# THUDM/GCC

Hardware: AMD Instinct MI355X
Metric: sampled-subgraphs/sec (higher is better)
Workload: dtype f32

## Files before the change

gcc_amd/_cabi.py:

```python
from __future__ import annotations

import ctypes
import os

_HERE = os.path.dirname(os.path.abspath(__file__))
LIB_PATH = os.path.join(_HERE, "csrc", "libgcc_amd.so")
HEADER_PATH = os.path.join(os.path.dirname(_HERE), "include", "gcc_amd.h")

c_i32p = ctypes.POINTER(ctypes.c_int32)
c_f32p = ctypes.POINTER(ctypes.c_float)
c_f64p = ctypes.POINTER(ctypes.c_double)

STATUS_SCRATCH_OVERFLOW = 1
STATUS_NODE_OVERFLOW = 2
STATUS_EDGE_OVERFLOW = 4


class GccGraph(ctypes.Structure):
    _fields_ = [
        ("row_ptr", ctypes.c_void_p),
        ("col_idx", ctypes.c_void_p),
        ("seed_cdf", ctypes.c_void_p),
        ("ltab", ctypes.c_void_p),
        ("num_nodes", ctypes.c_int64),
# ... 150 lines not shown


CLS_HEAD_MAX_CLASSES = 64
CLS_HEAD_MAX_DIM = 256

ABI_VERSION = 3
GRAPH_CONTRACT_CHECKED = 1

GAT_MAX_LAYERS = 8
GAT_MAX_S2S_LAYERS = 8


class GccGatWeights(ctypes.Structure):
    _fields_ = [
        ("num_layers", ctypes.c_int32), ("hidden", ctypes.c_int32), ("heads", ctypes.c_int32), ("out_dim", ctypes.c_int32),
        ("pos_dim", ctypes.c_int32), ("deg_emb_dim", ctypes.c_int32), ("max_degree", ctypes.c_int32),
        ("s2s_iters", ctypes.c_int32), ("s2s_layers", ctypes.c_int32), ("normalize", ctypes.c_int32),
        ("norm_eps", ctypes.c_float),
        ("degree_embedding", _VP),
        ("fc", _VP * GAT_MAX_LAYERS), ("attn_l", _VP * GAT_MAX_LAYERS), ("attn_r", _VP * GAT_MAX_LAYERS),
        ("w_ih", _VP * GAT_MAX_S2S_LAYERS), ("w_hh", _VP * GAT_MAX_S2S_LAYERS),
        ("b_ih", _VP * GAT_MAX_S2S_LAYERS), ("b_hh", _VP * GAT_MAX_S2S_LAYERS),
        ("ro0_w", _VP), ("ro0_b", _VP), ("ro2_w", _VP), ("ro2_b", _VP),
    ]


class GccGatGrads(ctypes.Structure):
    _fields_ = [
        ("degree_embedding", _VP),
        ("fc", _VP * GAT_MAX_LAYERS), ("attn_l", _VP * GAT_MAX_LAYERS), ("attn_r", _VP * GAT_MAX_LAYERS),
        ("w_ih", _VP * GAT_MAX_S2S_LAYERS), ("w_hh", _VP * GAT_MAX_S2S_LAYERS),
        ("b_ih", _VP * GAT_MAX_S2S_LAYERS), ("b_hh", _VP * GAT_MAX_S2S_LAYERS),
        ("ro0_w", _VP), ("ro0_b", _VP), ("ro2_w", _VP), ("ro2_b", _VP),
    ]


class GccGatPass(ctypes.Structure):
    _fields_ = [
        ("node_off", _VP), ("row_ptr", _VP), ("col_idx", _VP), ("seed_local", _VP), ("pos", _VP),
        ("batch_size", ctypes.c_int32), ("node_cap", ctypes.c_int32), ("edge_multiplicity", ctypes.c_int32),
        ("reserved_", ctypes.c_int32),
        ("saved", _VP), ("out", _VP),
    ]


SIGNATURES = {
    "gcc_abi_version": (ctypes.c_int32, []),
    "gcc_last_error": (ctypes.c_char_p, []),
    "gcc_stream_create_cu_mask": (ctypes.c_int32, [ctypes.c_void_p, ctypes.c_int32, ctypes.POINTER(ctypes.c_void_p)]),
    "gcc_stream_destroy": (ctypes.c_int32, [ctypes.c_void_p]),
    "gcc_prof_create": (ctypes.c_void_p, [ctypes.c_int32]),
    "gcc_prof_destroy": (None, [ctypes.c_void_p]),
    "gcc_prof_elapsed_ms": (ctypes.c_int32, [ctypes.c_void_p, ctypes.c_int32, ctypes.c_int32, c_f32p]),
    "gcc_sampler_workspace_bytes": (ctypes.c_int64, [ctypes.POINTER(GccGraph), ctypes.c_int32, ctypes.c_int64]),
    "gcc_sampler_workspace_bytes_multi": (ctypes.c_int64, [ctypes.POINTER(GccGraph), ctypes.c_int32, ctypes.c_int32, ctypes.c_int64]),
    "gcc_sample_multi": (ctypes.c_int32, [
        ctypes.POINTER(GccGraph), ctypes.POINTER(GccSampleParams), ctypes.c_int32, ctypes.c_int64, ctypes.POINTER(GccBatchOut),
        ctypes.c_void_p, ctypes.c_int64, ctypes.c_int64, ctypes.c_void_p, ctypes.c_void_p]),
    "gcc_sample_batch": (ctypes.c_int32, [
        ctypes.POINTER(GccGraph), ctypes.POINTER(GccSampleParams), ctypes.POINTER(GccBatchOut),
        ctypes.POINTER(GccBatchOut), ctypes.c_void_p, ctypes.c_int64, ctypes.c_int64, ctypes.c_void_p,
        ctypes.c_void_p]),
    "gcc_posemb_workspace_bytes": (ctypes.c_int64, [ctypes.c_int32, ctypes.c_int64, ctypes.c_int32]),
    "gcc_posemb_debug_ticks": (None, [ctypes.c_void_p]),
    "gcc_posemb_set_fork": (None, [ctypes.c_int32]),
    "gcc_sampler_debug_ticks": (None, [ctypes.c_void_p]),
    "gcc_sampler_debug_grids": (None, [ctypes.c_int32, ctypes.c_int32, ctypes.c_int32]),
    "gcc_debug_load": (ctypes.c_int32, [ctypes.c_int32, ctypes.c_int32, ctypes.c_int32, ctypes.c_int32, ctypes.c_int64, ctypes.c_int32,
                                        ctypes.c_void_p, ctypes.c_int64, ctypes.c_void_p, ctypes.c_void_p]),
    "gcc_gin_debug_ticks": (None, [ctypes.c_void_p]),
    "gcc_ginw_debug_ticks": (None, [ctypes.c_void_p]),
    "gcc_posemb_multi_workspace_bytes": (ctypes.c_int64, [ctypes.c_int32, ctypes.c_int32, ctypes.c_int64, ctypes.c_int32]),
    "gcc_posemb_multi": (ctypes.c_int32, [ctypes.POINTER(GccPosembView), ctypes.c_int32, ctypes.c_int32, ctypes.c_int64,
                                          ctypes.c_int32, ctypes.c_uint64, ctypes.c_void_p, ctypes.c_int64, ctypes.c_void_p,
                                          ctypes.c_void_p, ctypes.c_void_p]),
    "gcc_posemb_multi_gated": (ctypes.c_int32, [ctypes.POINTER(GccPosembView), ctypes.c_int32, ctypes.c_int32, ctypes.c_int64,
                                          ctypes.c_int32, ctypes.c_uint64, ctypes.c_void_p, ctypes.c_int64, ctypes.c_void_p,
                                          ctypes.c_void_p, ctypes.c_void_p, ctypes.c_void_p, ctypes.c_void_p]),
    "gcc_posemb": (ctypes.c_int32, [ctypes.POINTER(GccBatchOut), ctypes.c_int32, ctypes.c_int32, ctypes.c_void_p,
                                    ctypes.c_void_p, ctypes.c_void_p, ctypes.c_uint64, ctypes.c_void_p, ctypes.c_int64, ctypes.c_void_p,
                                    ctypes.c_void_p, ctypes.c_void_p]),
    "gcc_gin_forward": (ctypes.c_int32, [ctypes.POINTER(GccGinPass), ctypes.c_int32, ctypes.c_void_p,
                                         ctypes.c_void_p]),
    "gcc_gin_backward_workspace_bytes": (ctypes.c_int64, [ctypes.c_int64, ctypes.c_int32, ctypes.c_int32]),
    "gcc_gin_backward": (ctypes.c_int32, [ctypes.POINTER(GccGinPass), ctypes.c_void_p, ctypes.POINTER(GccGinGrads),
                                          ctypes.c_int32, ctypes.c_void_p, ctypes.c_int64, ctypes.c_int64,
                                          ctypes.c_void_p, ctypes.c_void_p]),
    "gcc_ginx_workspace_bytes": (ctypes.c_int64, [ctypes.c_int64, ctypes.c_int32, ctypes.c_int32, ctypes.c_int32, ctypes.c_int32, ctypes.c_int32]),
    "gcc_ginx_forward": (ctypes.c_int32, [ctypes.POINTER(GccGinxPass), ctypes.c_void_p]),
    "gcc_ginx_backward": (ctypes.c_int32, [ctypes.POINTER(GccGinxPass), ctypes.c_void_p, ctypes.POINTER(GccGinGrads), ctypes.c_void_p]),
    "gcc_ncex_forward": (ctypes.c_int32, [ctypes.c_void_p, ctypes.c_void_p, ctypes.c_void_p, ctypes.c_int32, ctypes.c_int32, ctypes.c_int32,
                                          ctypes.c_float, ctypes.c_int32] + [ctypes.c_void_p] * 8),
    "gcc_queue_enqueue_x": (ctypes.c_int32, [ctypes.c_void_p, ctypes.c_int32, ctypes.c_int32, ctypes.c_void_p, ctypes.c_int32, ctypes.c_int32,
                                             ctypes.c_void_p]),
    "gcc_ginw_forward": (ctypes.c_int32, [ctypes.POINTER(GccGinwArgs), ctypes.c_void_p, ctypes.c_void_p, ctypes.c_void_p]),
    "gcc_ginw_pack_weights": (ctypes.c_int32, [ctypes.c_void_p, ctypes.c_void_p, ctypes.c_int32, ctypes.c_void_p]),
    "gcc_nce_workspace_bytes": (ctypes.c_int64, [ctypes.c_int32, ctypes.c_int32]),
    "gcc_nce_forward": (ctypes.c_int32, [ctypes.POINTER(GccNceArgs), ctypes.c_void_p, ctypes.c_int64,
                                         ctypes.c_void_p, ctypes.c_void_p]),
    "gcc_nce_backward": (ctypes.c_int32, [ctypes.POINTER(GccNceArgs), ctypes.c_void_p, ctypes.c_int32,
                                          ctypes.c_void_p, ctypes.c_void_p, ctypes.c_int64, ctypes.c_void_p,
                                          ctypes.c_void_p]),
    "gcc_queue_enqueue": (ctypes.c_int32, [ctypes.c_void_p, ctypes.c_int32, ctypes.c_void_p, ctypes.c_int32,
                                           ctypes.c_int32, ctypes.c_void_p, ctypes.c_void_p]),
    "gcc_adam_step": (ctypes.c_int32, [ctypes.c_void_p, ctypes.c_void_p, ctypes.c_void_p, ctypes.c_void_p,
                                       ctypes.c_int64, ctypes.c_float, ctypes.c_float, ctypes.c_float, ctypes.c_float,
                                       ctypes.c_float, ctypes.c_int32, ctypes.c_float, ctypes.c_float, ctypes.c_void_p,
                                       ctypes.c_void_p, ctypes.c_void_p]),
    "gcc_adam_ema_step": (ctypes.c_int32, [ctypes.c_void_p, ctypes.c_void_p, ctypes.c_void_p, ctypes.c_void_p,
                                           ctypes.c_int64, ctypes.c_float, ctypes.c_float, ctypes.c_float, ctypes.c_float,
                                           ctypes.c_float, ctypes.c_int32, ctypes.c_float, ctypes.c_float, ctypes.c_void_p,
                                           ctypes.c_void_p, ctypes.c_void_p, ctypes.c_int64, ctypes.c_float,
                                           ctypes.POINTER(GccStepMetersArgs), ctypes.c_void_p]),
    "gcc_adam_ema_step_scalars": (ctypes.c_int32, [ctypes.c_void_p, ctypes.c_void_p, ctypes.c_void_p, ctypes.c_void_p,
                                                   ctypes.c_int64, ctypes.c_float, ctypes.c_float, ctypes.c_float,
                                                   ctypes.c_float, ctypes.c_float, ctypes.c_float, ctypes.c_void_p,
                                                   ctypes.c_void_p, ctypes.c_void_p, ctypes.c_int64, ctypes.c_float,
                                                   ctypes.POINTER(GccStepMetersArgs), ctypes.c_void_p, ctypes.c_void_p]),
    "gcc_queue_enqueue_scalars": (ctypes.c_int32, [ctypes.c_void_p, ctypes.c_int32, ctypes.c_void_p, ctypes.c_int32,
                                                   ctypes.c_void_p, ctypes.c_void_p]),
    "gcc_ginw_scratch_bytes": (ctypes.c_int64, [ctypes.c_int64, ctypes.c_int32]),
    "gcc_gin_eval_debug_ticks": (None, [ctypes.c_void_p]),
    "gcc_gin_eval_fused": (ctypes.c_int32, [ctypes.POINTER(GccGinPass), ctypes.c_int32, ctypes.c_void_p, ctypes.c_void_p]),
    "gcc_step_scalars_fill": (None, [ctypes.c_void_p, ctypes.c_float, ctypes.c_float, ctypes.c_float, ctypes.c_int32,
                                      ctypes.c_int32, ctypes.c_uint64]),
    "gcc_step_scalars_fetch": (ctypes.c_int32, [ctypes.c_void_p, ctypes.c_void_p, ctypes.c_int32, ctypes.c_void_p, ctypes.c_void_p]),
    "gcc_step_scalars_set": (ctypes.c_int32, [ctypes.c_void_p, ctypes.c_float, ctypes.c_float, ctypes.c_float, ctypes.c_int32,
                                              ctypes.c_int32, ctypes.c_uint64, ctypes.c_void_p]),
    "gcc_step_meters": (ctypes.c_int32, [ctypes.c_void_p] * 8 + [ctypes.c_int32, ctypes.c_void_p]),
    "gcc_ema_update": (ctypes.c_int32, [ctypes.c_void_p, ctypes.c_void_p, ctypes.c_int64, ctypes.c_float,
                                        ctypes.c_void_p]),
    "gcc_gat_saved_floats": (ctypes.c_int64, [ctypes.POINTER(GccGatWeights), ctypes.c_int32, ctypes.c_int32]),
    "gcc_gat_forward": (ctypes.c_int32, [ctypes.POINTER(GccGatPass), ctypes.POINTER(GccGatWeights), ctypes.c_void_p]),
    "gcc_gat_backward_workspace_bytes": (ctypes.c_int64, [ctypes.POINTER(GccGatWeights), ctypes.c_int32, ctypes.c_int32]),
    "gcc_gat_backward": (ctypes.c_int32, [ctypes.POINTER(GccGatPass), ctypes.POINTER(GccGatWeights), ctypes.c_void_p,
                                          ctypes.POINTER(GccGatGrads), ctypes.c_int32, ctypes.c_void_p, ctypes.c_int64,
                                          ctypes.c_void_p]),
    "gcc_cls_head_train": (ctypes.c_int32, [ctypes.POINTER(GccClsHeadArgs), ctypes.c_void_p]),
    "gcc_cls_head_eval": (ctypes.c_int32, [ctypes.POINTER(GccClsHeadArgs), ctypes.c_void_p]),
    "gcc_adam_clipvalue_step": (ctypes.c_int32, [ctypes.c_void_p, ctypes.c_void_p, ctypes.c_void_p, ctypes.c_void_p,
                                                 ctypes.c_int64, ctypes.c_float, ctypes.c_float, ctypes.c_float, ctypes.c_float,
                                                 ctypes.c_float, ctypes.c_int32, ctypes.c_float, ctypes.c_float, ctypes.c_void_p]),
}
PENDING = set()


def declare(lib: ctypes.CDLL) -> ctypes.CDLL:
    for name, (res, args) in SIGNATURES.items():
        fn = getattr(lib, name)
        fn.restype = res
        fn.argtypes = args
    return lib


_lib = None


def load() -> ctypes.CDLL:
    global _lib
    if _lib is None:
        if not os.path.exists(LIB_PATH):
            raise RuntimeError(
                f"{LIB_PATH} is missing: build it with `python -c 'import __graft_entry__ as g; g.build()'` "
                "(hipcc --offload-arch=gfx950).  gcc_amd has no CPU fallback.")
        import torch

        lib = declare(ctypes.CDLL(LIB_PATH))
        got = lib.gcc_abi_version()
        if got != ABI_VERSION:
            raise RuntimeError(f"{LIB_PATH} reports C-ABI version {got}, this binding was written for {ABI_VERSION}: "
                               "rebuild the library (python -c 'import __graft_entry__ as g; g.build()')")
        _lib = lib
    return _lib


def check(rc: int, what: str) -> None:
    if rc != 0:
        raise RuntimeError(f"{what} failed ({rc}): {load().gcc_last_error().decode()}")


def dev_ptr(t, dtype=None) -> int:
    import torch

    if t is None:
        return 0
    if not isinstance(t, torch.Tensor) or not t.is_cuda:
        raise RuntimeError("gcc_amd kernels take device (HIP) tensors only; there is no CPU path")
    if dtype is not None and t.dtype != dtype:
        raise TypeError(f"expected {dtype}, got {t.dtype}")
    if not t.is_contiguous():
        raise ValueError("tensor must be contiguous")
    return t.data_ptr()
```

gcc_amd/contrast.py:

```python
from __future__ import annotations

import ctypes
import math

import torch
from torch import nn

from . import _cabi

D = 64


class NceEngine:

    def __init__(self, lib=None, ptr=None, dtype="f32"):
        self.lib = lib if lib is not None else _cabi.load()
        self.ptr = ptr if ptr is not None else _cabi.dev_ptr
        self._ws = {}
        self.dtype = dtype

    def _workspace(self, B, K, device):
        nbytes = self.lib.gcc_nce_workspace_bytes(B, K)
        key = (nbytes, str(device))
        if key not in self._ws:
            self._ws[key] = torch.empty(nbytes, dtype=torch.uint8, device=device)
        return self._ws[key], nbytes

    def _args(self, q, k, mem, inv_T, pos_mode, patch, patch_index, outs, dense):
        ptr = self.ptr
        a = _cabi.GccNceArgs()
        a.q, a.k, a.mem = ptr(q), ptr(k) if k is not None else None, ptr(mem)
        a.patch = ptr(patch) if patch is not None else None
        a.patch_index = int(patch_index)
        a.patch_rows = int(patch.shape[0]) if patch is not None else 0
        a.B, a.K, a.pos_mode, a.inv_T = q.shape[0], mem.shape[0], pos_mode, inv_T
        a.lse, a.pos, a.loss, a.prob = ptr(outs["lse"]), ptr(outs["pos"]), ptr(outs["loss"]), ptr(outs["prob"])
        a.out_dense = ptr(dense) if dense is not None else None
        a.dtype = {"f32": 0, "bf16": 1}[self.dtype]
        return a

    def forward(self, q, k, mem, T, pos_mode, dense=False, lse_rows=None, patch=None, patch_index=0, stream=None,
                prof=None):
        B, K = q.shape[0], mem.shape[0]
        f32 = dict(dtype=torch.float32, device=q.device)
        outs = dict(lse=torch.empty(lse_rows or B, **f32), pos=torch.empty(B, **f32), loss=torch.empty(1, **f32),
                    prob=torch.empty(1, **f32))
        out = torch.empty(B, K + (1 if pos_mode == 0 else 0), **f32) if dense else None
        ws, nbytes = self._workspace(B, K, q.device)
        a = self._args(q, k, mem, 1.0 / T, pos_mode, patch, patch_index, outs, out)
        rc = self.lib.gcc_nce_forward(ctypes.byref(a), self.ptr(ws), nbytes, prof.handle if prof else None, stream)
        if rc != 0:
            raise RuntimeError(f"gcc_nce_forward failed ({rc}): {self.lib.gcc_last_error().decode()}")
        outs["out"] = out
        return outs

    def backward(self, q, k, mem, T, pos_mode, outs, dloss, patch=None, patch_index=0, by_mem_row=False,
                 stream=None, prof=None):
        B, K = q.shape[0], mem.shape[0]
        dq = torch.empty_like(q)
        ws, nbytes = self._workspace(B, K, q.device)
        a = self._args(q, k, mem, 1.0 / T, pos_mode, patch, patch_index, outs, None)
        dloss = dloss.reshape(1).to(torch.float32).contiguous()
        rc = self.lib.gcc_nce_backward(ctypes.byref(a), self.ptr(dloss), int(by_mem_row), self.ptr(dq), self.ptr(ws),
                                       nbytes, prof.handle if prof else None, stream)
        if rc != 0:
            raise RuntimeError(f"gcc_nce_backward failed ({rc}): {self.lib.gcc_last_error().decode()}")
        return dq

    def set_scalars(self, scalars, lr, betas, adam_step, enqueue_index, dropout_seed, stream=None):
        rc = self.lib.gcc_step_scalars_set(self.ptr(scalars), float(lr), float(betas[0]), float(betas[1]), int(adam_step),
                                           int(enqueue_index), int(dropout_seed) & 0xFFFFFFFFFFFFFFFF, stream)
        if rc != 0:
            raise RuntimeError(f"gcc_step_scalars_set failed ({rc}): {self.lib.gcc_last_error().decode()}")

    def fill_scalars(self, ring, slot, lr, betas, adam_step, enqueue_index, dropout_seed):
        self.lib.gcc_step_scalars_fill(ring.data_ptr() + 24 * int(slot), float(lr), float(betas[0]), float(betas[1]),
                                       int(adam_step), int(enqueue_index), int(dropout_seed) & 0xFFFFFFFFFFFFFFFF)

    def fetch_scalars(self, scalars, ring, ring_len, counter, stream=None):
        rc = self.lib.gcc_step_scalars_fetch(self.ptr(scalars), ring.data_ptr(), int(ring_len), self.ptr(counter), stream)
        if rc != 0:
            raise RuntimeError(f"gcc_step_scalars_fetch failed ({rc}): {self.lib.gcc_last_error().decode()}")

    def enqueue(self, mem, keys, index, save=True, stream=None, scalars=None):
        if scalars is not None:
            rc = self.lib.gcc_queue_enqueue_scalars(self.ptr(mem), mem.shape[0], self.ptr(keys), keys.shape[0],
                                                    self.ptr(scalars), stream)
            if rc != 0:
                raise RuntimeError(f"gcc_queue_enqueue_scalars failed ({rc}): {self.lib.gcc_last_error().decode()}")
            return None
        saved = torch.empty_like(keys) if save else None
        rc = self.lib.gcc_queue_enqueue(self.ptr(mem), mem.shape[0], self.ptr(keys), keys.shape[0], int(index),
                                        self.ptr(saved) if saved is not None else None, stream)
        if rc != 0:
            raise RuntimeError(f"gcc_queue_enqueue failed ({rc}): {self.lib.gcc_last_error().decode()}")
        return saved

    def adam(self, param, grad, exp_avg, exp_avg_sq, lr, betas, eps, weight_decay, step, max_norm, grad_norm,
             scratch, stream=None, grad_scale=1.0):
        rc = self.lib.gcc_adam_step(self.ptr(param), self.ptr(grad), self.ptr(exp_avg), self.ptr(exp_avg_sq),
                                    param.numel(), float(lr), float(betas[0]), float(betas[1]), float(eps),
                                    float(weight_decay), int(step), float(max_norm), float(grad_scale), self.ptr(grad_norm),
                                    self.ptr(scratch), stream)
        if rc != 0:
            raise RuntimeError(f"gcc_adam_step failed ({rc}): {self.lib.gcc_last_error().decode()}")

    def adam_ema(self, param, grad, exp_avg, exp_avg_sq, lr, betas, eps, weight_decay, step, max_norm, grad_norm,
                 scratch, stream=None, grad_scale=1.0, ema=None, ema_src=None, ema_m=0.0, meters=None, scalars=None):
        ma = None
        if meters is not None:
            acc, mx, loss, prob, q, k = meters
            ma = _cabi.GccStepMetersArgs(self.ptr(acc), self.ptr(mx), self.ptr(loss), self.ptr(prob), self.ptr(q.node_off),
                                         self.ptr(q.edge_off), self.ptr(k.node_off), int(q.batch_size))
        if ema is not None and (ema_src is None or ema_src.data_ptr() != param.data_ptr() or ema.numel() != ema_src.numel()):
            raise ValueError("adam_ema: param must be a prefix of ema_src, and ema the same size as ema_src")
        if scalars is not None:
            rc = self.lib.gcc_adam_ema_step_scalars(
                self.ptr(param), self.ptr(grad), self.ptr(exp_avg), self.ptr(exp_avg_sq), param.numel(), float(betas[0]),
                float(betas[1]), float(eps), float(weight_decay), float(max_norm), float(grad_scale), self.ptr(grad_norm),
                self.ptr(scratch), self.ptr(ema) if ema is not None else None, ema.numel() if ema is not None else 0,
                float(ema_m), ctypes.byref(ma) if ma is not None else None, self.ptr(scalars), stream)
            if rc != 0:
                raise RuntimeError(f"gcc_adam_ema_step_scalars failed ({rc}): {self.lib.gcc_last_error().decode()}")
            return
        rc = self.lib.gcc_adam_ema_step(self.ptr(param), self.ptr(grad), self.ptr(exp_avg), self.ptr(exp_avg_sq),
                                        param.numel(), float(lr), float(betas[0]), float(betas[1]), float(eps),
                                        float(weight_decay), int(step), float(max_norm), float(grad_scale),
                                        self.ptr(grad_norm), self.ptr(scratch),
                                        self.ptr(ema) if ema is not None else None, ema.numel() if ema is not None else 0,
                                        float(ema_m), ctypes.byref(ma) if ma is not None else None, stream)
        if rc != 0:
            raise RuntimeError(f"gcc_adam_ema_step failed ({rc}): {self.lib.gcc_last_error().decode()}")

    def meters(self, acc, mx, loss, prob, grad_norm, q, k, stream=None):
        rc = self.lib.gcc_step_meters(self.ptr(acc), self.ptr(mx), self.ptr(loss), self.ptr(prob), self.ptr(grad_norm),
                                      self.ptr(q.node_off), self.ptr(q.edge_off), self.ptr(k.node_off),
                                      int(q.batch_size), stream)
        if rc != 0:
            raise RuntimeError(f"gcc_step_meters failed ({rc}): {self.lib.gcc_last_error().decode()}")

    def ema(self, ema, p, m, stream=None):
        rc = self.lib.gcc_ema_update(self.ptr(ema), self.ptr(p), ema.numel(), float(m), stream)
        if rc != 0:
            raise RuntimeError(f"gcc_ema_update failed ({rc}): {self.lib.gcc_last_error().decode()}")


def _stream(t):
    return torch.cuda.current_stream(t.device).cuda_stream if t.is_cuda else None


class _MoCoLoss(torch.autograd.Function):

    @staticmethod
    def forward(ctx, q, k, module, outs, patch, patch_index):
        ctx.module, ctx.outs, ctx.patch, ctx.patch_index = module, outs, patch, patch_index
        ctx.save_for_backward(q, k)
        return outs["loss"].reshape(())

    @staticmethod
    def backward(ctx, dloss):
        q, k = ctx.saved_tensors
        m = ctx.module
        dq = m.engine().backward(q, k, m.kernel_memory(), m.T, 0, ctx.outs, dloss, patch=ctx.patch,
                                 patch_index=ctx.patch_index, stream=_stream(q))
        return dq, None, None, None, None, None


class _NSLoss(torch.autograd.Function):

    @staticmethod
    def forward(ctx, feat_q, feat_k, T, eng):
        fq, fk = feat_q.contiguous(), feat_k.contiguous()
        outs = eng.forward(fk, None, fq, T, 1, stream=_stream(fq))
        ctx.eng, ctx.T, ctx.outs = eng, T, outs
        ctx.save_for_backward(fq, fk)
        ctx.mark_non_differentiable(outs["prob"])
        return outs["loss"].reshape(()), outs["prob"].reshape(())

    @staticmethod
    def backward(ctx, dloss, _dprob):
        fq, fk = ctx.saved_tensors
        eng, T, outs = ctx.eng, ctx.T, ctx.outs
        dk = eng.backward(fk, None, fq, T, 1, outs, dloss, stream=_stream(fq))
        dq = eng.backward(fq, None, fk, T, 1, outs, dloss, by_mem_row=True, stream=_stream(fq))
        return dq, dk, None, None


class WideNceEngine:

    def __init__(self, lib=None, ptr=None):
        self.lib = lib if lib is not None else _cabi.load()
        self.ptr = ptr if ptr is not None else _cabi.dev_ptr

    def forward(self, rows, k, mem, T, mode, stream=None):
        B, D = rows.shape
        K = mem.shape[0]
        f32 = dict(dtype=torch.float32, device=rows.device)
        ncols = K + 1 if mode == 0 else K
# ... 173 lines not shown
```

gcc_amd/csrc/encoder.hip:

```cpp
#include "encoder_common.h"

namespace {

struct FeatArgs {
    const int32_t *node_off, *row_ptr, *graph_id, *seed_local;
    const float *pos, *emb;
    float *x0;
    float4 *zero_a, *zero_b;
    int64_t zero_a16, zero_b16;
    int32_t B, pos_dim, emb_dim, max_degree, mult;
    int32_t cap;
};
struct FeatLaunch { FeatArgs p[kMaxPass]; };

__global__ __launch_bounds__(kThreads) void gin_feat_kernel(FeatLaunch L)
{
    TRAIN_STEP_WAVE_PRIORITY();
    const FeatArgs &a = L.p[blockIdx.y];
    const int tid = (int)threadIdx.x, t = tid & 15, gi = tid >> 4;
    constexpr int kR = kTile / 16;
    int vv[kR], r0[kR], r1[kR], gv[kR];
    float pv[kR][4];
    auto request = [&](int tile0) {
#pragma unroll
        for (int i = 0; i < kR; ++i) {
            vv[i] = cap_row(tile0 + gi + 16 * i, a.cap);
            r0[i] = a.row_ptr[vv[i]];
            r1[i] = a.row_ptr[vv[i] + 1];
            gv[i] = a.graph_id[vv[i]];
#pragma unroll
            for (int e = 0; e < 4; ++e)
                pv[i][e] = a.pos_dim > 0 ? a.pos[(int64_t)vv[i] * a.pos_dim + min(4 * t + e, a.pos_dim - 1)] : 0.f;
        }
    };
    const int tf = first_tile();
    request(tf * kTile);
    const int N = a.node_off[a.B];
    SCHED_FENCE();
    {
        const float4 z4 = make_float4(0.f, 0.f, 0.f, 0.f);
        const int64_t stride = (int64_t)gridDim.x * kThreads;
        for (int64_t i = (int64_t)blockIdx.x * kThreads + tid; i < a.zero_a16; i += stride) a.zero_a[i] = z4;
        for (int64_t i = (int64_t)blockIdx.x * kThreads + tid; i < a.zero_b16; i += stride) a.zero_b[i] = z4;
    }
    for (TileWalk tw(N); tw.ti < tw.tend; tw.ti += tw.step) {
        const int tile0 = tw.ti * kTile;
        const int nrows = min(kTile, N - tile0);
        if (tw.ti != tf) request(tile0);
        int first[kR], sl[kR];
        float ev[kR][4];
        const int dtot = a.pos_dim + a.emb_dim;
#pragma unroll
        for (int i = 0; i < kR; ++i) {
            const int deg = (r1[i] - r0[i]) * a.mult;
            const int dcl = max(0, deg < a.max_degree ? deg : a.max_degree);
            const int g = min(max(gv[i], 0), a.B - 1);
            first[i] = a.node_off[g];
            sl[i] = a.seed_local ? a.seed_local[g] : 0;
#pragma unroll
            for (int e = 0; e < 4; ++e) {
                const int c = 4 * t + e;
                ev[i][e] = a.emb[(int64_t)dcl * a.emb_dim + (c >= a.pos_dim && c < dtot ? c - a.pos_dim : 0)];
            }
        }
#pragma unroll
        for (int i = 0; i < kR; ++i) {
            if (gi + 16 * i >= nrows) continue;
            const bool is_seed = vv[i] == first[i] + sl[i];
            F4 x;
#pragma unroll
            for (int e = 0; e < 4; ++e) {
                const int c = 4 * t + e;
                at(x, e) = c < a.pos_dim ? pv[i][e] : c < dtot ? ev[i][e] : (c == dtot && is_seed ? 1.f : 0.f);
            }
            st4(a.x0 + (int64_t)vv[i] * H + 4 * t, x);
        }
    }
}

struct InArgs {
    const int32_t *node_off, *row_ptr, *col_idx, *graph_id;
    const float *src;
    BnDev bnb, bnc;
    const float *w0, *b0;
    float *agg;
    float *z1;
    double *stats_a;
    double *pooled;
    int32_t B, first, kdim, training;
    float eps, nbr_weight;
    int32_t cap;
};
struct InLaunch { InArgs p[kMaxPass]; long long *ticks; };
#ifndef GIN_IN_LDS_W
#define GIN_IN_LDS_W 1
#endif
#ifndef GIN_DBG_SKIP
#define GIN_DBG_SKIP 0
#endif
static long long *g_gin_ticks = nullptr;
constexpr int kTickWgs = 2048, kTickPhases = 16;
#define TICK_ADD(kind, ph, v) atomicAdd((unsigned long long *)&L.ticks[((kind) * kTickPhases + (ph)) * kTickWgs + (int)blockIdx.y * 1024 + (int)blockIdx.x], (unsigned long long)(v))
#define GIN_TICK(ph) do { if (L.ticks && tid == 0) { const long long now_ = device_ticks(); TICK_ADD(a.first ? 0 : 1, ph, now_ - tick_); tick_ = now_; } } while (0)

#ifndef GIN_IN_PER_CU
#define GIN_IN_PER_CU 3
#endif
#ifndef GIN_GATHER_J
#define GIN_GATHER_J 8
#endif
__global__ __launch_bounds__(kThreads, GIN_IN_PER_CU) void gin_in_kernel(InLaunch L)
{
    TRAIN_STEP_WAVE_PRIORITY();
    __shared__ float T[kTile * kLdt];
    __shared__ __attribute__((aligned(16))) float part[32 * H];
    __shared__ float red[4 * 2 * H];
    __shared__ int prow[32];
    __shared__ int rpl[kTile + 1], gidl[kTile];
    const InArgs &a = L.p[blockIdx.y];
    const int tid = (int)threadIdx.x, t = tid & 15, gi = tid >> 4, lane = lane_id(), wv = tid >> 6;
    int N;
    __shared__ float tabb[2 * H], tabc[2 * H];
#if GIN_IN_LDS_W
    __shared__ float Wl[H * kLdt];
    __shared__ __attribute__((aligned(16))) float bl[H];
#endif
    Aff4 ab, ac;
    long long tick_ = L.ticks ? device_ticks() : 0;
    const float *src = a.src;
    auto load = [&](int u) -> F4 { return ld4(src + (int64_t)u * H + 4 * t); };
    const int tf = first_tile();
    int rp_own, gid_own;
    F4 own[kTile / 16];
    auto request = [&](int tile0) {
        rp_own = a.row_ptr[min(tile0 + min(tid, kTile), a.cap)];
        gid_own = a.graph_id[cap_row(tile0 + (tid & (kTile - 1)), a.cap)];
#pragma unroll
        for (int i = 0; i < kTile / 16; ++i) own[i] = load(cap_row(tile0 + gi + 16 * i, a.cap));
    };
    {
#if GIN_IN_LDS_W
        const WStage wst = stage_weights_request(a.w0, a.kdim);
        const float b_own = a.b0 ? a.b0[tid & (H - 1)] : 0.f;
#endif
        if (!a.first) {
            const BnReq rb = bn_request(a.bnb), rc = bn_request(a.bnc);
            request(tf * kTile);
            N = a.node_off[a.B];
            SCHED_FENCE();
            if (no_tiles(N)) return;
            bn_table_finish(tabb, rb, (double)N, a.eps, a.training, (double *)part);
            bn_table_finish(tabc, rc, (double)N, a.eps, a.training, (double *)part);
        } else {
            request(tf * kTile);
            N = ((const volatile int32_t *)a.node_off)[a.B];
            if (no_tiles(N)) return;
        }
#if GIN_IN_LDS_W
        stage_weights_store(Wl, wst, a.kdim);
// ... 295 lines not shown
            for (int e = 0; e < 4; ++e) pd[c][e] = prow[16 * c + e];
        SCHED_FENCE();
#pragma unroll
        for (int c = 0; c < 4; ++c) {
            const F4 x = {(float)pd[c][0], (float)pd[c][1], (float)pd[c][2], (float)pd[c][3]}, z = {0.f, 0.f, 0.f, 0.f};
            xb[c] = valid ? x : z;
        }
        f32x4 acc[4];
        mfma_rows16(xb, wf, acc);
#pragma unroll
        for (int cb = 0; cb < 4; ++cb) {
            const int ch = 16 * cb + 4 * q;
            const F4 bias = bias4[cb];
            const F4 m = valid ? drop_mul4(drop, i, b, ch) : bias;
            score[cb].x += (acc[cb][0] + bias.x) * m.x;
            score[cb].y += (acc[cb][1] + bias.y) * m.y;
            score[cb].z += (acc[cb][2] + bias.z) * m.z;
            score[cb].w += (acc[cb][3] + bias.w) * m.w;
        }
    }
#pragma unroll
    for (int cb = 0; cb < 4; ++cb) st4(&part[wv][j][16 * cb + 4 * q], score[cb]);
    __syncthreads();
    if (wv == 0) {
        float ss = 0.f;
#pragma unroll
        for (int cb = 0; cb < 4; ++cb) {
            F4 t = ld4(&part[0][j][16 * cb + 4 * q]);
            for (int w2 = 1; w2 < 4; ++w2) t = add4(t, ld4(&part[w2][j][16 * cb + 4 * q]));
            score[cb] = t;
            ss += t.x * t.x + t.y * t.y + t.z * t.z + t.w * t.w;
        }
        ss += wave_shfl_xor(ss, 16);
        ss += wave_shfl_xor(ss, 32);
        const float inv = a.normalize ? 1.0f / fmaxf(sqrtf(ss), a.norm_eps) : 1.0f;
        if (valid) {
#pragma unroll
            for (int cb = 0; cb < 4; ++cb) {
                const int ch = 16 * cb + 4 * q;
                st4(a.score + (int64_t)b * H + ch, score[cb]);
                F4 o = {score[cb].x * inv, score[cb].y * inv, score[cb].z * inv, score[cb].w * inv};
                st4(a.feat + (int64_t)b * H + ch, o);
            }
        }
    }
    if (bn_work) {
        const int n_nodes = a.node_off[a.B];
        double *scratch = (double *)&part[0][0][0];
        for (int k = (int)blockIdx.x; k < 3 * a.nlayers; k += (int)gridDim.x) {
            __syncthreads();
            const BnDev &bn = a.bn[k];
            float rm = rm0, rv = rv0;
            if (k == (int)blockIdx.x) {
                scratch[tid] = rep_sum(rq);
                __syncthreads();
            } else {
                replica_sums128(bn.stats, 2 * H, scratch);
                rm = bn.running_mean[tid & (H - 1)];
                rv = bn.running_var[tid & (H - 1)];
            }
            if (tid < H) {
                const int c = tid;
                const double n = (double)n_nodes;
                const double s1 = scratch[c] + scratch[128 + c], s2 = scratch[H + c] + scratch[128 + H + c];
                if (a.totals) { a.totals[(int64_t)k * 2 * H + c] = s1; a.totals[(int64_t)k * 2 * H + H + c] = s2; }
                if (a.update_running) {
                    const double mean = s1 / n;
                    double var = s2 / n - mean * mean;
                    if (var < 0.0) var = 0.0;
                    const double unb = n > 1.0 ? var * n / (n - 1.0) : var;
                    bn.running_mean[c] = (float)((1.0 - a.momentum) * (double)rm + a.momentum * mean);
                    bn.running_var[c] = (float)((1.0 - a.momentum) * (double)rv + a.momentum * unb);
                    if (c == 0 && bn.nbt) bn.nbt[0] += 1;
                }
            }
        }
    }
}

}

extern "C" void gcc_gin_debug_ticks(long long *device_ticks64) { g_gin_ticks = device_ticks64; }

extern "C" int32_t gcc_gin_forward(const gcc_gin_pass *passes, int32_t npass, gcc_prof *prof, void *stream)
{
    if (!passes || npass < 1 || npass > kMaxPass) {
        snprintf(g_err, kErrLen, "gcc_gin_forward: npass must be 1..%d", kMaxPass);
        return -1;
    }
    const int Lg = passes[0].w.num_gin_layers;
    int maxB = 0;
    for (int i = 0; i < npass; ++i) {
        const gcc_gin_pass &p = passes[i];
        const int din = p.w.pos_dim + p.w.deg_emb_dim + 1;
        if (p.w.num_gin_layers != Lg || Lg < 1 || Lg > GCC_GIN_MAX_LAYERS || din > H || p.batch_size < 1) {
            snprintf(g_err, kErrLen, "gcc_gin_forward: unsupported shape (layers=%d d_in=%d B=%d)",
                     p.w.num_gin_layers, din, p.batch_size);
            return -2;
        }
        if (p.node_cap < 1 || p.node_cap > 0x7fffffff) {
            snprintf(g_err, kErrLen, "gcc_gin_forward: gcc_gin_pass.node_cap = %lld (the row capacity of the pass's buffers is required)",
                     (long long)p.node_cap);
            return -2;
        }
        maxB = p.batch_size > maxB ? p.batch_size : maxB;
    }
    hipStream_t s = (hipStream_t)stream;
    prof_mark(prof, 0, s);
    int64_t rows_max = 0;
    for (int i = 0; i < npass; ++i) {
        const gcc_gin_pass &p = passes[i];
        const int64_t r = p.rows_hint > 0 && p.rows_hint < p.node_cap ? p.rows_hint : p.node_cap;
        rows_max = r > rows_max ? r : rows_max;
    }
    const dim3 grid(tile_grid(rows_max), npass), block(kThreads);
    {
        FeatLaunch L;
        for (int i = 0; i < npass; ++i) {
            const gcc_gin_pass &p = passes[i];
            L.p[i] = {p.node_off, p.row_ptr, p.graph_id, p.seed_local, p.pos, p.w.degree_embedding, p.x0,
                      (float4 *)p.stats, (float4 *)p.pooled, (int64_t)Lg * 3 * kRep * 2 * H * (int64_t)sizeof(double) / 16,
                      (int64_t)(Lg + 1) * p.batch_size * H * (int64_t)sizeof(double) / 16,
                      p.batch_size, p.w.pos_dim, p.w.deg_emb_dim, p.w.max_degree, p.edge_multiplicity > 1 ? p.edge_multiplicity : 1,
                      (int32_t)p.node_cap};
        }
        hipLaunchKernelGGL(gin_feat_kernel, grid, block, 0, s, L);
    }
    for (int l = 0; l < Lg; ++l) {
        {
            InLaunch L;
            for (int i = 0; i < npass; ++i) {
                const gcc_gin_pass &p = passes[i];
                InArgs a;
                a.node_off = p.node_off; a.row_ptr = p.row_ptr; a.col_idx = p.col_idx; a.graph_id = p.graph_id;
                a.src = l == 0 ? p.x0 : p.z2[l - 1];
                a.bnb = l == 0 ? BnDev() : bn_of(p, p.w.bn_b[l - 1], l - 1, 1, false);
                a.bnc = l == 0 ? BnDev() : bn_of(p, p.w.bn_c[l - 1], l - 1, 2, false);
                a.w0 = p.w.lin0_w[l]; a.b0 = p.w.lin0_b[l];
                a.agg = p.agg[l]; a.z1 = p.z1[l];
                a.stats_a = stats_of(p, l, 0);
                a.pooled = p.pooled + (int64_t)l * p.batch_size * H;
                a.B = p.batch_size; a.first = l == 0;
                a.kdim = l == 0 ? p.w.pos_dim + p.w.deg_emb_dim + 1 : hidden_of(p.w);
                a.training = p.training; a.eps = p.w.bn_eps;
                a.nbr_weight = p.edge_multiplicity > 1 ? (float)p.edge_multiplicity : 1.0f;
                a.cap = (int32_t)p.node_cap;
                L.p[i] = a;
            }
            L.ticks = g_gin_ticks;
            hipLaunchKernelGGL(gin_in_kernel, grid, block, 0, s, L);
        }
        {
            MidLaunch L;
            for (int i = 0; i < npass; ++i) {
                const gcc_gin_pass &p = passes[i];
                L.p[i] = {p.node_off, p.z1[l], bn_of(p, p.w.bn_a[l], l, 0, false), p.w.lin1_w[l], p.w.lin1_b[l],
                          p.z2[l], stats_of(p, l, 1), p.batch_size, p.training,
                          p.w.bn_eps, hidden_of(p.w), (int32_t)p.node_cap};
            }
            L.ticks = g_gin_ticks;
            hipLaunchKernelGGL(gin_mid_kernel, grid, block, 0, s, L);
        }
        {
            StatLaunch L;
            bool need = false;
            for (int i = 0; i < npass; ++i) {
                const gcc_gin_pass &p = passes[i];
                L.p[i] = {p.node_off, p.z2[l], bn_of(p, p.w.bn_b[l], l, 1, false), stats_of(p, l, 2), p.batch_size, p.training, p.w.bn_eps,
                          (int32_t)p.node_cap};
                need = need || p.training;
            }
            if (need) hipLaunchKernelGGL(gin_stat_kernel, grid, block, 0, s, L);
        }
    }
    {
        PoolLaunch L;
        for (int i = 0; i < npass; ++i) {
            const gcc_gin_pass &p = passes[i];
            L.p[i] = {p.node_off, p.graph_id, p.z2[Lg - 1], bn_of(p, p.w.bn_b[Lg - 1], Lg - 1, 1, false),
                      bn_of(p, p.w.bn_c[Lg - 1], Lg - 1, 2, false), p.pooled + (int64_t)Lg * p.batch_size * H,
                      p.batch_size, p.training, p.w.bn_eps, (int32_t)p.node_cap};
        }
        hipLaunchKernelGGL(gin_pool_kernel, grid, block, 0, s, L);
    }
    {
        ReadLaunch L;
        for (int i = 0; i < npass; ++i) {
            const gcc_gin_pass &p = passes[i];
            ReadArgs a;
            a.node_off = p.node_off; a.pooled = p.pooled;
            for (int k = 0; k <= Lg; ++k) { a.pred_w[k] = p.w.pred_w[k]; a.pred_b[k] = p.w.pred_b[k]; }
            a.drop = drop_cfg(p); a.score = p.score; a.feat = p.feat;
            for (int l = 0; l < Lg; ++l) {
                a.bn[3 * l + 0] = bn_of(p, p.w.bn_a[l], l, 0, false);
                a.bn[3 * l + 1] = bn_of(p, p.w.bn_b[l], l, 1, false);
                a.bn[3 * l + 2] = bn_of(p, p.w.bn_c[l], l, 2, false);
            }
            a.totals = p.training ? p.bn_totals : nullptr;
            a.B = p.batch_size; a.nlayers = Lg; a.kdim0 = p.w.pos_dim + p.w.deg_emb_dim + 1; a.hid = hidden_of(p.w);
            a.normalize = p.normalize; a.update_running = p.training && p.update_running_stats;
            a.norm_eps = p.w.norm_eps; a.momentum = p.w.bn_momentum;
            L.p[i] = a;
        }
        hipLaunchKernelGGL(gin_readout_kernel, dim3((maxB + 15) / 16, npass), block, 0, s, L);
    }
    prof_mark(prof, 1, s);
    hipError_t e = hipGetLastError();
    if (e != hipSuccess) {
        snprintf(g_err, kErrLen, "gcc_gin_forward: launch failed: %s", hipGetErrorString(e));
        return -10;
    }
    return 0;
}
```

gcc_amd/csrc/encoder_bwd.hip:

```cpp
#include "encoder_common.h"

namespace {

constexpr int kWgChunks = 64;

struct BnCol { float mean, rstd, gamma, beta; };
__device__ __forceinline__ BnCol bn_col(const BnDev &bn, int c, double s1, double s2, double n, float eps)
{
    const double mean = s1 / n;
    double var = s2 / n - mean * mean;
    if (var < 0.0) var = 0.0;
    BnCol r;
    r.mean = (float)mean;
    r.rstd = (float)(1.0 / sqrt(var + (double)eps));
    r.gamma = bn.weight[c];
    r.beta = bn.bias[c];
    return r;
}

enum { RS = 0, RM = 1, PS = 2, PH = 3, K1 = 4, K2 = 5, K3 = 6, kCoefRows = 7 };

__device__ __forceinline__ void fill_coefs(float *C , const BnDev &bn, const double *bst, double n,
                                           float eps, double *scratch)
{
// ... 641 lines not shown
    SCHED_FENCE();
    const int N = jb.rows_fixed > 0 ? jb.rows_fixed : Nn;
    TileWalk tw(N);
    if (tid < H) {
        float sc = 1.f, sh = 0.f;
        if (fast) {
            const double mean = cr.s1 / (double)Nn;
            double var = cr.s2 / (double)Nn - mean * mean;
            if (var < 0.0) var = 0.0;
            const double rstd = 1.0 / sqrt(var + (double)a.eps);
            sc = (float)((double)cr.gamma * rstd);
            sh = (float)((double)cr.beta - mean * (double)cr.gamma * rstd);
        } else if (act) {
            bn_scale_shift(jb.bn, tid, (double)Nn, a.eps, 1, sc, sh);
        }
        Cx[tid] = sc;
        Cx[H + tid] = sh;
    }
    __syncthreads();
    float xs[4], xh[4];
#pragma unroll
    for (int kb = 0; kb < 4; ++kb) { xs[kb] = Cx[16 * kb + j]; xh[kb] = Cx[H + 16 * kb + j]; }
    for (; tw.ti < tw.tend; tw.ti += tw.step) {
        const int tile0 = tw.ti * kTile;
        float an[4][4], xn[4][4];
        const bool more = tw.ti + tw.step < tw.tend;
        if (more) fetch((tw.ti + tw.step) * kTile, an, xn);
        mask_tile(tile0, N, av, xv);
#pragma unroll
        for (int s = 0; s < 4; ++s) {
            const int row = tile0 + 16 * wv + 4 * s + q;
            float bv[4];
#pragma unroll
            for (int k = 0; k < 4; ++k) {
                bsum[k] += av[s][k];
                bv[k] = act ? (row < N ? fmaxf(fmaf(xv[s][k], xs[k], xh[k]), 0.f) : 0.f) : xv[s][k];
            }
#pragma unroll
            for (int ob = 0; ob < 4; ++ob)
#pragma unroll
                for (int kb = 0; kb < 4; ++kb) acc[ob][kb] = mfma_16x16x4_f32(av[s][ob], bv[kb], acc[ob][kb]);
        }
        if (more) {
#pragma unroll
            for (int s = 0; s < 4; ++s)
#pragma unroll
                for (int k = 0; k < 4; ++k) { av[s][k] = an[s][k]; xv[s][k] = xn[s][k]; }
        }
    }
    for (int w = 0; w < 4; ++w) {
        if (wv == w) {
#pragma unroll
            for (int ob = 0; ob < 4; ++ob)
#pragma unroll
                for (int kb = 0; kb < 4; ++kb)
#pragma unroll
                    for (int r = 0; r < 4; ++r) {
                        const int o = 16 * ob + 4 * q + r, k = 16 * kb + j;
                        S[o * H + k] = (w == 0 ? 0.f : S[o * H + k]) + acc[ob][kb][r];
                    }
        }
        __syncthreads();
    }
    float *slab = a.slabs + ((int64_t)jid * kWgChunks + blockIdx.x) * H * H;
    for (int i = tid; i < H * H; i += kThreads) slab[i] = S[i];
#pragma unroll
    for (int k = 0; k < 4; ++k) {
        bsum[k] += wave_shfl_xor(bsum[k], 16);
        bsum[k] += wave_shfl_xor(bsum[k], 32);
        if (q == 0) Sb[wv * H + 16 * k + j] = bsum[k];
    }
    __syncthreads();
    if (tid < H)
        a.bias_slabs[((int64_t)jid * kWgChunks + blockIdx.x) * H + tid] =
            (Sb[tid] + Sb[H + tid]) + (Sb[2 * H + tid] + Sb[3 * H + tid]);
}

struct FinalArgs {
    const float *slabs, *bias_slabs;
    const double *bst;
    const float *demb_parts;
    gcc_gin_grads g;
    int32_t B, L, kdim0, emb_rows, emb_dim, accumulate, hid;
};

__device__ __forceinline__ void put(float *dst, float v, int acc)
{
    if (dst) *dst = acc ? *dst + v : v;
}

__global__ __launch_bounds__(kThreads) void gin_grad_final_kernel(FinalArgs a)
{
    TRAIN_STEP_WAVE_PRIORITY();
    const int64_t gid = (int64_t)blockIdx.x * kThreads + threadIdx.x;
    const int L = a.L;
    int64_t base = 0;
    const int njobs = 3 * L + 1;
    const int64_t n1 = (int64_t)njobs * H * H;
    if (gid < n1) {
        const int y = (int)(gid / (H * H)), idx = (int)(gid % (H * H));
        const int o = idx / H, k = idx % H;
        float s = 0.f;
        for (int c = 0; c < kWgChunks; ++c) s += a.slabs[((int64_t)y * kWgChunks + c) * H * H + idx];
        int kd = H;
        float *dst;
        if (y < 2 * L) {
            const int l = y >> 1, which = y & 1;
            kd = (which == 0 && l == 0) ? a.kdim0 : a.hid;
            dst = which ? a.g.lin1_w[l] : a.g.lin0_w[l];
        } else {
            const int i = y - 2 * L;
            kd = i == 0 ? a.kdim0 : a.hid;
            dst = a.g.pred_w[i];
        }
        if (k < kd && dst) put(dst + (int64_t)o * kd + k, s, a.accumulate);
        return;
    }
    base += n1;
    const int64_t n3 = (int64_t)(L + 1) * H;
    if (gid < base + n3) {
        const int64_t r = gid - base;
        const int i = (int)(r / H), o = (int)(r % H);
        float s = 0.f;
        for (int c = 0; c < kWgChunks; ++c) s += a.bias_slabs[((int64_t)(2 * L + i) * kWgChunks + c) * H + o];
        if (a.g.pred_b[i]) put(a.g.pred_b[i] + o, s, a.accumulate);
        return;
    }
    base += n3;
    const int64_t n4 = (int64_t)L * 3 * 3 * H;
    if (gid < base + n4) {
        const int64_t r = gid - base;
        const int c = (int)(r % H), slot = (int)((r / H) % 3), which = (int)((r / (3 * H)) % 3), l = (int)(r / (9 * H));
        double acc = 0.0;
        const double *src = a.bst + ((int64_t)l * 3 + which) * kRep * 3 * H + slot * H + c;
#pragma unroll
        for (int rep = 0; rep < kRep; rep += 8) {
            double v8[8];
#pragma unroll
            for (int u = 0; u < 8; ++u) v8[u] = src[(int64_t)(rep + u) * 3 * H];
            acc += ((v8[0] + v8[1]) + (v8[2] + v8[3])) + ((v8[4] + v8[5]) + (v8[6] + v8[7]));
        }
        const float v = (float)acc;
        float *dst = nullptr;
        if (which == 0) dst = slot == 0 ? a.g.bn_a_b[l] : slot == 1 ? a.g.bn_a_w[l] : a.g.lin0_b[l];
        else if (which == 1) dst = slot == 0 ? a.g.bn_b_b[l] : slot == 1 ? a.g.bn_b_w[l] : a.g.lin1_b[l];
        else dst = slot == 0 ? a.g.bn_c_b[l] : slot == 1 ? a.g.bn_c_w[l] : nullptr;
        if (dst) put(dst + c, v, a.accumulate);
        return;
    }
    base += n4;
    base = (base + 63) & ~(int64_t)63;
    const int64_t n5 = (int64_t)a.emb_rows * a.emb_dim;
    if (gid >= base) {
        static_assert(kEmbBlocks % 64 == 0, "8 threads x batches of 8 partials");
        const int64_t q = gid - base, r = q >> 3;
        const int part = (int)(q & 7);
        float s = 0.f;
        if (r < n5) {
            const float *src = a.demb_parts + (int64_t)part * (kEmbBlocks / 8) * n5 + r;
            for (int k = 0; k < kEmbBlocks / 8; k += 8) {
                float v[8];
#pragma unroll
                for (int u = 0; u < 8; ++u) v[u] = src[(int64_t)(k + u) * n5];
                s += ((v[0] + v[1]) + (v[2] + v[3])) + ((v[4] + v[5]) + (v[6] + v[7]));
            }
        }
        s += wave_shfl_xor(s, 1);
        s += wave_shfl_xor(s, 2);
        s += wave_shfl_xor(s, 4);
        if (part == 0 && r < n5 && a.g.degree_embedding) put(a.g.degree_embedding + r, s, a.accumulate);
    }
}

struct BwdWork {
    float *U, *V, *Wt, *D;
    float *dz1[GCC_GIN_MAX_LAYERS], *dz2[GCC_GIN_MAX_LAYERS];
    float *G, *dpooled, *slabs, *bias_slabs;
    double *bst;
    float *demb_parts;
    int64_t off_zero, zero_bytes, total;
};

inline BwdWork bwd_layout(char *base, int64_t node_cap, int32_t B, int32_t L, int32_t emb_elems)
{
    BwdWork w;
    auto al = [](int64_t x) { return (x + 255) & ~(int64_t)255; };
    int64_t o = 0;
    auto take = [&](int64_t bytes) { int64_t at = o; o = al(o + bytes); return base ? base + at : (char *)nullptr; };
    const int64_t act = node_cap * H * (int64_t)sizeof(float);
    w.U = (float *)take(act); w.V = (float *)take(act); w.Wt = (float *)take(act); w.D = (float *)take(act);
    for (int l = 0; l < GCC_GIN_MAX_LAYERS; ++l) {
        w.dz1[l] = l < L ? (float *)take(act) : nullptr;
        w.dz2[l] = l < L ? (float *)take(act) : nullptr;
    }
    w.G = (float *)take((int64_t)(L + 1) * B * H * sizeof(float));
    w.dpooled = (float *)take((int64_t)(L + 1) * B * H * sizeof(float));
    w.slabs = (float *)take((int64_t)(3 * L + 1) * kWgChunks * H * H * sizeof(float));
    w.bias_slabs = (float *)take((int64_t)(3 * L + 1) * kWgChunks * H * sizeof(float));
    w.demb_parts = (float *)take((int64_t)kEmbBlocks * emb_elems * sizeof(float));
    w.off_zero = o;
    w.bst = (double *)take((int64_t)L * 9 * kRep * H * sizeof(double));
    w.zero_bytes = o - w.off_zero;
    w.total = o;
    return w;
}

}

extern "C" int64_t gcc_gin_backward_workspace_bytes(int64_t node_cap, int32_t batch_size, int32_t num_gin_layers)
{
    if (node_cap <= 0 || batch_size <= 0 || num_gin_layers < 1 || num_gin_layers > GCC_GIN_MAX_LAYERS) {
        snprintf(g_err, kErrLen, "gcc_gin_backward_workspace_bytes: bad argument");
        return -1;
    }
    return bwd_layout(nullptr, node_cap, batch_size, num_gin_layers, kEmbMaxElems).total;
}

extern "C" int32_t gcc_gin_backward(const gcc_gin_pass *pass, const float *dfeat, const gcc_gin_grads *grads,
                                    int32_t accumulate, void *workspace, int64_t workspace_bytes,
                                    int64_t node_cap, gcc_prof *prof, void *stream)
{
    if (!pass || !dfeat || !grads || !workspace) {
        snprintf(g_err, kErrLen, "gcc_gin_backward: null argument");
        return -1;
    }
    const gcc_gin_pass &p = *pass;
    if (p.edge_multiplicity > 1) {
        snprintf(g_err, kErrLen, "gcc_gin_backward: edge_multiplicity %d (inference-only feature)", p.edge_multiplicity);
        return -2;
    }
    const int L = p.w.num_gin_layers, B = p.batch_size;
    const int kdim0 = p.w.pos_dim + p.w.deg_emb_dim + 1;
    const int emb_elems = (p.w.max_degree + 1) * p.w.deg_emb_dim;
    if (!p.training || L < 1 || L > GCC_GIN_MAX_LAYERS || emb_elems > kEmbMaxElems) {
        snprintf(g_err, kErrLen, "gcc_gin_backward: needs a training-mode pass (layers=%d)", L);
        return -2;
    }
    for (int l = 0; l < L; ++l)
        if (!p.agg[l]) { snprintf(g_err, kErrLen, "gcc_gin_backward: agg[%d] was not saved", l); return -2; }
    const BwdWork w = bwd_layout((char *)workspace, node_cap, B, L, kEmbMaxElems);
    if (workspace_bytes < w.total) {
        snprintf(g_err, kErrLen, "gcc_gin_backward: workspace %lld < %lld bytes", (long long)workspace_bytes,
                 (long long)w.total);
        return -3;
    }
    if (node_cap < 1 || node_cap > 0x7fffffff || (p.node_cap > 0 && p.node_cap != node_cap)) {
        snprintf(g_err, kErrLen, "gcc_gin_backward: node_cap %lld (the pass says %lld)", (long long)node_cap, (long long)p.node_cap);
        return -2;
    }
    const int32_t cap = (int32_t)node_cap;
    hipStream_t s = (hipStream_t)stream;
    prof_mark(prof, 0, s);
    const dim3 grid(tile_grid(p.rows_hint > 0 && p.rows_hint < node_cap ? p.rows_hint : node_cap)), block(kThreads);
    auto bst = [&](int l, int which) { return w.bst + ((int64_t)l * 3 + which) * kRep * 3 * H; };
    {
        ReadBwdArgs a;
        a.dfeat = dfeat; a.score = p.score; a.feat = p.feat; a.drop = drop_cfg(p);
        for (int i = 0; i <= L; ++i) a.pred_w[i] = p.w.pred_w[i];
        a.G = w.G; a.dpooled = w.dpooled; a.B = B; a.nlayers = L; a.kdim0 = kdim0; a.normalize = p.normalize; a.hid = hidden_of(p.w);
        a.norm_eps = p.w.norm_eps;
        a.zero = (float4 *)((char *)workspace + w.off_zero); a.zero16 = w.zero_bytes / 16; a.nread = ((B + 15) / 16 * (L + 1) + 3) / 4;
        hipLaunchKernelGGL(gin_bwd_readout_kernel, dim3(a.nread + 64), block, 0, s, a);
    }
    for (int l = L - 1; l >= 0; --l) {
        const BnDev bna = bn_of(p, p.w.bn_a[l], l, 0);
        const BnDev bnb = bn_of(p, p.w.bn_b[l], l, 1);
        const BnDev bnc = bn_of(p, p.w.bn_c[l], l, 2);
        {
            BwdCArgs a = {p.node_off, p.row_ptr, p.col_idx, p.graph_id, l == L - 1 ? nullptr : w.D,
                          w.dpooled + (int64_t)(l + 1) * B * H, p.z2[l], bnb, bnc, w.U, bst(l, 2), B, p.w.bn_eps, cap};
            hipLaunchKernelGGL(gin_bwd_c_kernel, grid, block, 0, s, a);
        }
        {
            BwdBArgs a = {p.node_off, w.U, p.z2[l], bnb, bnc, bst(l, 2), w.V, bst(l, 1), B, p.w.bn_eps, cap};
            hipLaunchKernelGGL(gin_bwd_b_kernel, grid, block, 0, s, a);
        }
        {
            BwdLinArgs a = {p.node_off, w.V, p.z2[l], bnb, bst(l, 1), bst(l, 1) + 2 * H, p.w.lin1_w[l], hidden_of(p.w),
                            w.dz2[l], w.Wt, p.z1[l], bna, bst(l, 0), B, p.w.bn_eps, cap};
            hipLaunchKernelGGL((gin_bwd_lin_kernel<true>), grid, block, 0, s, a);
        }
        {
            BwdLinArgs a = {p.node_off, w.Wt, p.z1[l], bna, bst(l, 0), bst(l, 0) + 2 * H, p.w.lin0_w[l],
                            l == 0 ? kdim0 : hidden_of(p.w), w.dz1[l], w.D, nullptr, BnDev(), nullptr, B, p.w.bn_eps, cap};
            hipLaunchKernelGGL((gin_bwd_lin_kernel<false>), grid, block, 0, s, a);
        }
    }
    {
        EmbArgs a = {p.node_off, p.row_ptr, p.col_idx, p.graph_id, w.D, w.dpooled, w.demb_parts, B, p.w.pos_dim,
                     p.w.deg_emb_dim, p.w.max_degree, cap};
        hipLaunchKernelGGL(gin_bwd_emb_kernel, dim3(kEmbBlocks), block, 0, s, a);
    }
    {
        WgradArgs a;
        a.node_off = p.node_off; a.slabs = w.slabs; a.bias_slabs = w.bias_slabs; a.B = B; a.eps = p.w.bn_eps; a.cap = cap;
        for (int l = 0; l < L; ++l) {
            a.job[2 * l + 0] = {w.dz1[l], p.agg[l], nullptr, BnDev(), 0};
            a.job[2 * l + 1] = {w.dz2[l], p.z1[l], nullptr, bn_of(p, p.w.bn_a[l], l, 0), 0};
        }
        for (int i = 0; i <= L; ++i)
            a.job[2 * L + i] = {w.G + (int64_t)i * B * H, nullptr, p.pooled + (int64_t)i * B * H, BnDev(), B};
        hipLaunchKernelGGL(gin_wgrad_kernel, dim3(kWgChunks, 3 * L + 1), block, 0, s, a);
    }
    {
        FinalArgs a;
        a.slabs = w.slabs; a.bias_slabs = w.bias_slabs; a.bst = w.bst; a.demb_parts = w.demb_parts; a.g = *grads;
        a.B = B; a.L = L; a.kdim0 = kdim0; a.emb_rows = p.w.max_degree + 1; a.emb_dim = p.w.deg_emb_dim; a.hid = hidden_of(p.w);
        a.accumulate = accumulate;
        const int64_t upto4 = (int64_t)(3 * L + 1) * H * H + (int64_t)(L + 1) * H + (int64_t)L * 9 * H;
        const int64_t total = ((upto4 + 63) & ~(int64_t)63) + (((int64_t)a.emb_rows * a.emb_dim * 8 + 63) & ~(int64_t)63);
        hipLaunchKernelGGL(gin_grad_final_kernel, dim3((unsigned)((total + kThreads - 1) / kThreads)), block, 0, s, a);
    }
    prof_mark(prof, 1, s);
    hipError_t e = hipGetLastError();
    if (e != hipSuccess) {
        snprintf(g_err, kErrLen, "gcc_gin_backward: launch failed: %s", hipGetErrorString(e));
        return -10;
    }
    return 0;
}
```

gcc_amd/csrc/nce.hip:

```cpp
#include "host_common.h"

#include <math.h>

namespace {

constexpr int D = GCC_NCE_DIM;
constexpr int kLd = 72;
constexpr int kChunk = 64;
constexpr int kThreads = 256;
constexpr int kQPerBlock = 64;

struct F4 { float x, y, z, w; };
__device__ __forceinline__ F4 ld4(const float *p)
{
    const float4 v = *reinterpret_cast<const float4 *>(p);
    F4 r = {v.x, v.y, v.z, v.w};
    return r;
}
__device__ __forceinline__ void st4(float *p, F4 v) { *reinterpret_cast<float4 *>(p) = make_float4(v.x, v.y, v.z, v.w); }

struct NceDev {
    const float *q, *k, *mem, *patch;
    int32_t patch_index, patch_rows, B, K, pos_mode;
    int32_t bf16;
// ... 112 lines not shown
    for (int c0 = row_beg; c0 < row_end; c0 += kChunk) {
#pragma unroll
        for (int i = 0; i < 4; ++i) {
            const int idx = tid + kThreads * i, row = idx >> 4, c4 = (idx & 15) * 4;
            st4(&Ms[row * kLd + c4], finish_mem4(a, nxt[i], c0 + row));
        }
        __syncthreads();
        if (c0 + kChunk < row_end) request(c0 + kChunk);
        for (int t = 0; t < 4; ++t) {
            if (c0 + 16 * t >= row_end) break;
            f32x4 acc = {0.f, 0.f, 0.f, 0.f};
            if (kBf16 && !kBwd) {
#pragma unroll
                for (int sl = 0; sl < 2; ++sl) {
                    const F4 lo = ld4(&Ms[(16 * t + j) * kLd + 32 * sl + 8 * q]), hi = ld4(&Ms[(16 * t + j) * kLd + 32 * sl + 8 * q + 4]);
                    u32x4 mb;
                    mb[0] = pack_bf16(lo.x, lo.y); mb[1] = pack_bf16(lo.z, lo.w);
                    mb[2] = pack_bf16(hi.x, hi.y); mb[3] = pack_bf16(hi.z, hi.w);
                    acc = mfma_16x16x32_bf16(mb, qb[sl], acc);
                }
            } else {
#pragma unroll
                for (int c = 0; c < 4; ++c) {
                    const F4 mf = ld4(&Ms[(16 * t + j) * kLd + 16 * c + 4 * q]);
                    acc = mfma_16x16x4_f32(mf.x, qf[c].x, acc);
                    acc = mfma_16x16x4_f32(mf.y, qf[c].y, acc);
                    acc = mfma_16x16x4_f32(mf.z, qf[c].z, acc);
                    acc = mfma_16x16x4_f32(mf.w, qf[c].w, acc);
                }
            }
            const int row0 = c0 + 16 * t + 4 * q;
            float lv[4];
#pragma unroll
            for (int r = 0; r < 4; ++r) {
                const float l = acc[r] * a.inv_T;
                const bool valid = row0 + r < row_end;
                if (!kBwd && a.out_dense && qvalid && valid) a.out_dense[(int64_t)qj * ld_out + off_out + row0 + r] = l;
                lv[r] = valid ? l : -INFINITY;
            }
            if (!kBwd) {
                const float tmax = fmaxf(fmaxf(lv[0], lv[1]), fmaxf(lv[2], lv[3]));
                if (tmax > -INFINITY) {
                    const float mn = fmaxf(m, tmax);
                    ssum = ssum * expf(m - mn) + expf(lv[0] - mn) + expf(lv[1] - mn) + expf(lv[2] - mn) + expf(lv[3] - mn);
                    m = mn;
                }
            } else {
                float lse_r[4] = {my_lse, my_lse, my_lse, my_lse};
                if (a.by_mem_row) {
#pragma unroll
                    for (int r = 0; r < 4; ++r) lse_r[r] = a.lse[min(row0 + r, a.K - 1)];
                }
#pragma unroll
                for (int r = 0; r < 4; ++r) {
                    float p = 0.f;
                    if (qvalid && lv[r] > -INFINITY) p = expf(lv[r] - lse_r[r]);
#pragma unroll
                    for (int db = 0; db < 4; ++db)
                        acc2[db] = mfma_16x16x4_f32(Ms[(16 * t + 4 * q + r) * kLd + 16 * db + j], p, acc2[db]);
                }
            }
        }
        __syncthreads();
    }
    if (!kBwd) {
#pragma unroll
        for (int d = 16; d <= 32; d <<= 1) {
            const float m2 = wave_shfl_xor(m, d), s2 = wave_shfl_xor(ssum, d);
            const float mn = fmaxf(m, m2);
            ssum = mn > -INFINITY ? ssum * expf(m - mn) + s2 * expf(m2 - mn) : 0.f;
            m = mn;
        }
        if (q == 0 && qvalid) {
            a.pm[(int64_t)s * a.B + qj] = m;
            a.ps[(int64_t)s * a.B + qj] = ssum;
        }
    } else if (qvalid) {
#pragma unroll
        for (int db = 0; db < 4; ++db) {
            F4 o = {acc2[db][0], acc2[db][1], acc2[db][2], acc2[db][3]};
            st4(a.slabs + ((int64_t)s * a.B + qj) * D + 16 * db + 4 * q, o);
        }
    }
}

__global__ __launch_bounds__(kThreads) void nce_combine_kernel(NceDev a)
{
    TRAIN_STEP_WAVE_PRIORITY();
    __shared__ double red[8];
    __shared__ int last;
    const int tid = (int)threadIdx.x, lane = lane_id(), wv = tid >> 6;
    const int ld_out = a.K + (a.pos_mode == 0 ? 1 : 0);
    const int b = (int)blockIdx.x * (kThreads >> 6) + wv;
    if (b < a.B) {
        const float *other = a.pos_mode == 0 ? a.k : a.mem;
        float qv = a.q[(int64_t)b * D + lane], ov = other[(int64_t)b * D + lane];
        const int s0 = min(lane, a.S - 1);
        const float pm0r = a.pm[(int64_t)s0 * a.B + b], ps0r = a.ps[(int64_t)s0 * a.B + b];
        const float pm0 = lane < a.S ? pm0r : -INFINITY;
        if (a.bf16) { qv = rnd_bf16(qv); ov = rnd_bf16(ov); }
        const float pos = wave_sum(qv * ov) * a.inv_T;
        float m = pm0;
        for (int s = lane + 64; s < a.S; s += 64) m = fmaxf(m, a.pm[(int64_t)s * a.B + b]);
        m = wave_max(m);
        if (a.pos_mode == 0) m = fmaxf(m, pos);
        float sum = pm0 > -INFINITY ? ps0r * expf(pm0 - m) : 0.f;
        for (int s = lane + 64; s < a.S; s += 64) {
            const float pmv = a.pm[(int64_t)s * a.B + b], psv = a.ps[(int64_t)s * a.B + b];
            if (pmv > -INFINITY) sum += psv * expf(pmv - m);
        }
        sum = wave_sum(sum);
        if (a.pos_mode == 0) sum += expf(pos - m);
        const float lse = m + logf(sum);
        if (lane == 0) {
            a.lse[b] = lse;
            a.pos[b] = pos;
            if (a.pos_mode == 0 && a.out_dense) a.out_dense[(int64_t)b * ld_out] = pos;
        }
    }
    device_fence();
    __syncthreads();
    if (tid == 0) last = atomicAdd(a.ticket, 1) == (int)gridDim.x - 1;
    __syncthreads();
    if (!last) return;
    device_fence();
    double lsum = 0.0, psum = 0.0;
    for (int i = tid; i < a.B; i += kThreads) {
        const float lse = load_fresh(a.lse + i), pos = load_fresh(a.pos + i);
        lsum += (double)(lse - pos);
        psum += (double)pos;
    }
    lsum = wave_sum(lsum);
    psum = wave_sum(psum);
    if (lane == 0) { red[wv] = lsum; red[4 + wv] = psum; }
    __syncthreads();
    if (tid == 0) {
        a.loss[0] = (float)((red[0] + red[1] + red[2] + red[3]) / (double)a.B);
        a.prob[0] = (float)((red[4] + red[5] + red[6] + red[7]) / (double)a.B);
        *a.ticket = 0;
    }
}

#ifndef NCE_DQ_BATCH
#define NCE_DQ_BATCH 16
#endif
__global__ __launch_bounds__(kThreads) void nce_dq_kernel(NceDev a)
{
    TRAIN_STEP_WAVE_PRIORITY();
    const int gid = (int)blockIdx.x * kThreads + (int)threadIdx.x;
    const int b = gid >> 4, c4 = (gid & 15) * 4;
    if (b >= a.B) return;
    const float dl = a.dloss[0];
    const float posb = a.pos_mode == 0 ? a.pos[b] : 0.f, lseb = a.pos_mode == 0 ? a.lse[b] : 0.f;
    const F4 other = rnd4(ld4((a.pos_mode == 0 ? a.k : a.mem) + (int64_t)b * D + c4), a.bf16 != 0);
    F4 s = {0.f, 0.f, 0.f, 0.f};
    const float *sp = a.slabs + (int64_t)b * D + c4;
    const int64_t st = (int64_t)a.B * D;
    for (int sl = 0; sl < a.S; sl += NCE_DQ_BATCH) {
        F4 v[NCE_DQ_BATCH];
#pragma unroll
        for (int u = 0; u < NCE_DQ_BATCH; ++u) v[u] = ld4(sp + (int64_t)min(sl + u, a.S - 1) * st);
#pragma unroll
        for (int u = 0; u < NCE_DQ_BATCH; ++u)
            if (sl + u < a.S) { s.x += v[u].x; s.y += v[u].y; s.z += v[u].z; s.w += v[u].w; }
    }
    const int nrows = a.by_mem_row ? a.K : a.B;
    const float coef = dl * a.inv_T / (float)nrows;
    F4 o;
    if (a.pos_mode == 0) {
        const float pp = expf(posb - lseb) - 1.f;
        o.x = coef * (s.x + pp * other.x); o.y = coef * (s.y + pp * other.y);
        o.z = coef * (s.z + pp * other.z); o.w = coef * (s.w + pp * other.w);
    } else {
        o.x = coef * (s.x - other.x); o.y = coef * (s.y - other.y); o.z = coef * (s.z - other.z); o.w = coef * (s.w - other.w);
    }
    st4(a.dq + (int64_t)b * D + c4, o);
}

__global__ __launch_bounds__(kThreads) void queue_enqueue_kernel(float *mem, int K, const float *keys, int nkeys,
                                                                 int index, float *saved, const gcc_step_scalars *sc)
{
    TRAIN_STEP_WAVE_PRIORITY();
    if (sc) index = sc->enqueue_index % K;
    const int gid = (int)blockIdx.x * kThreads + (int)threadIdx.x;
    const int i = gid >> 4, c4 = (gid & 15) * 4;
    if (i >= nkeys) return;
    const int row = (index + i) % K;
    if (saved) st4(saved + (int64_t)i * D + c4, ld4(mem + (int64_t)row * D + c4));
    st4(mem + (int64_t)row * D + c4, ld4(keys + (int64_t)i * D + c4));
}

__global__ __launch_bounds__(kThreads) void ema_kernel(float *ema, const float *p, int64_t n, float m)
{
    TRAIN_STEP_WAVE_PRIORITY();
    const int64_t stride = (int64_t)gridDim.x * kThreads;
    for (int64_t i = (int64_t)blockIdx.x * kThreads + threadIdx.x; i < n; i += stride)
        ema[i] = ema[i] * m + (1.f - m) * p[i];
}

constexpr int kNormBlocks = 32;
__global__ __launch_bounds__(kThreads) void gradnorm_kernel(const float *g, int64_t n, double *scratch)
{
    TRAIN_STEP_WAVE_PRIORITY();
    static_assert(kNormBlocks <= 64, "the last workgroup adds the partials up with one wave");
    __shared__ double red[kThreads / 64];
    __shared__ int last;
    const int tid = (int)threadIdx.x;
    double s = 0.0;
    const int64_t stride = (int64_t)gridDim.x * kThreads;
    for (int64_t base = (int64_t)blockIdx.x * kThreads + tid; base < n; base += 8 * stride) {
        float x[8];
#pragma unroll
        for (int u = 0; u < 8; ++u) { const int64_t i = base + u * stride; x[u] = g[i < n ? i : n - 1]; }
#pragma unroll
        for (int u = 0; u < 8; ++u) if (base + u * stride < n) s += (double)x[u] * (double)x[u];
    }
    s = wave_sum(s);
    if ((tid & 63) == 0) red[tid >> 6] = s;
    __syncthreads();
    if (tid == 0) {
        double t = 0.0;
        for (int i = 0; i < kThreads / 64; ++i) t += red[i];
        scratch[2 + blockIdx.x] = t;
        device_fence();
        last = atomicAdd((int *)(scratch + 1), 1) == (int)gridDim.x - 1;
    }
    __syncthreads();
    if (last && tid < 64) {
        device_fence();
        const double v = tid < (int)gridDim.x ? load_fresh_f64(scratch + 2 + tid) : 0.0;
        const double tot = wave_sum(v);
        if (tid == 0) {
            scratch[0] = tot;
            *(int *)(scratch + 1) = 0;
        }
    }
}

struct AdamExtras {
    float *ema; int64_t n_ema; float ema_m;
    const gcc_step_scalars *sc;
    double *acc; int32_t *mx; const float *loss, *prob; const int32_t *node_off_q, *edge_off_q, *node_off_k; int32_t B;
};

__global__ __launch_bounds__(kThreads) void adam_kernel(float *p, float *g, float *m, float *v, int64_t n, float lr,
                                                        float b1, float b2, float eps, float wd, float bc1,
                                                        float bc2_sqrt, float max_norm, float grad_scale,
                                                        const double *sumsq, float *grad_norm, AdamExtras x)
{
    TRAIN_STEP_WAVE_PRIORITY();
    const double ss = sumsq[0];
    if (x.sc) { lr = x.sc->lr; bc1 = x.sc->bias_corr1; bc2_sqrt = x.sc->bias_corr2_sqrt; }
    const int64_t stride = (int64_t)gridDim.x * kThreads, i0 = (int64_t)blockIdx.x * kThreads + threadIdx.x;
    const int64_t ic = i0 < n ? i0 : n - 1;
    float g0 = g[ic], p0 = p[ic], m0 = m[ic], v0 = v[ic];
    const float e0 = x.ema ? x.ema[i0 < x.n_ema ? i0 : x.n_ema - 1] : 0.f;
    const float norm = grad_scale * (float)sqrt(ss);
    float coef = 1.f;
    if (max_norm > 0.f) {
        coef = max_norm / (norm + 1e-6f);
        coef = coef > 1.f ? 1.f : coef;
    }
    if (blockIdx.x == 0 && threadIdx.x == 0) {
        grad_norm[0] = norm;
        if (x.acc) {
            const int32_t nq = x.node_off_q[x.B], nk = x.node_off_k[x.B], eq = x.edge_off_q[x.B];
            x.acc[0] += (double)x.loss[0];
            x.acc[1] += (double)x.prob[0];
            x.acc[2] += (double)norm;
            x.acc[3] += (double)nq + (double)nk;
            x.acc[4] += 1.0;
            x.mx[0] = nq > x.mx[0] ? nq : x.mx[0];
            x.mx[1] = eq > x.mx[1] ? eq : x.mx[1];
        }
    }
    coef *= grad_scale;
    const int64_t nmax = x.ema && x.n_ema > n ? x.n_ema : n;
    for (int64_t i = i0; i < nmax; i += stride) {
        float pi, ei = 0.f;
        if (i != i0) {
            const int64_t j = i < n ? i : n - 1;
            g0 = g[j]; p0 = p[j]; m0 = m[j]; v0 = v[j];
            if (x.ema) ei = x.ema[i < x.n_ema ? i : x.n_ema - 1];
        } else {
            ei = e0;
        }
        if (i < n) {
            const float gc = g0 * coef;
            g[i] = gc;
            const float gi = fmaf(wd, p0, gc);
            const float mi = fmaf(b1, m0, (1.f - b1) * gi);
            const float vi = fmaf(b2, v0, (1.f - b2) * gi * gi);
            m[i] = mi;
            v[i] = vi;
            const float denom = sqrtf(vi) / bc2_sqrt + eps;
            pi = p0 - (lr / bc1) * (mi / denom);
            p[i] = pi;
        } else {
            pi = p[i];
        }
        if (x.ema && i < x.n_ema) x.ema[i] = ei * x.ema_m + (1.f - x.ema_m) * pi;
    }
}

__global__ void step_meters_kernel(double *acc, int32_t *mx, const float *loss, const float *prob, const float *gnorm,
                                   const int32_t *node_off_q, const int32_t *edge_off_q, const int32_t *node_off_k,
                                   int32_t B)
{
    TRAIN_STEP_WAVE_PRIORITY();
    if (threadIdx.x != 0 || blockIdx.x != 0) return;
    const int32_t nq = node_off_q[B], nk = node_off_k[B], eq = edge_off_q[B];
    acc[0] += (double)loss[0];
    acc[1] += (double)prob[0];
    acc[2] += (double)gnorm[0];
    acc[3] += (double)nq + (double)nk;
    acc[4] += 1.0;
    mx[0] = nq > mx[0] ? nq : mx[0];
    mx[1] = eq > mx[1] ? eq : mx[1];
}

inline int fill_dev(const gcc_nce_args *a, void *workspace, int64_t workspace_bytes, NceDev &d, Plan &pl)
{
    if (!a || !a->q || !a->mem || a->B < 1 || a->K < 1 || (a->pos_mode == 0 && !a->k) ||
        (a->pos_mode == 1 && a->K < a->B) || !a->lse || !a->pos) {
        snprintf(g_err, kErrLen, "gcc_nce: bad argument");
        return -1;
    }
    pl = make_plan(a->B, a->K);
    if (!workspace || workspace_bytes < pl.total) {
        snprintf(g_err, kErrLen, "gcc_nce: workspace %lld < %lld bytes", (long long)workspace_bytes, (long long)pl.total);
        return -3;
    }
    d.q = a->q; d.k = a->k; d.mem = a->mem; d.patch = a->patch;
    d.patch_index = a->patch_index; d.patch_rows = a->patch ? a->patch_rows : 0;
    d.B = a->B; d.K = a->K; d.pos_mode = a->pos_mode; d.inv_T = a->inv_T;
    d.bf16 = a->dtype == GCC_NCE_BF16 ? 1 : 0;
    d.lse = a->lse; d.pos = a->pos; d.loss = a->loss; d.prob = a->prob; d.out_dense = a->out_dense;
    d.S = pl.S; d.R = pl.R;
    char *base = (char *)workspace;
    d.pm = (float *)(base + pl.off_pm); d.ps = (float *)(base + pl.off_ps); d.slabs = (float *)(base + pl.off_slabs);
    d.ticket = (int32_t *)(base + pl.off_ticket);
    d.dloss = nullptr; d.by_mem_row = 0; d.dq = nullptr;
    return 0;
}

}

extern "C" {

int64_t gcc_nce_workspace_bytes(int32_t B, int32_t K)
{
    if (B < 1 || K < 1) { snprintf(g_err, kErrLen, "gcc_nce_workspace_bytes: bad argument"); return -1; }
    return make_plan(B, K).total;
}

int32_t gcc_nce_forward(const gcc_nce_args *a, void *workspace, int64_t workspace_bytes, gcc_prof *prof, void *stream)
{
    NceDev d;
    Plan pl;
    int rc = fill_dev(a, workspace, workspace_bytes, d, pl);
    if (rc) return rc;
    if (!a->loss || !a->prob) { snprintf(g_err, kErrLen, "gcc_nce_forward: loss/prob are required"); return -1; }
    hipStream_t s = (hipStream_t)stream;
    prof_mark(prof, 0, s);
    if (d.bf16) hipLaunchKernelGGL((nce_slice_kernel<false, true>), dim3(pl.S, pl.QB), dim3(kThreads), 0, s, d);
    else hipLaunchKernelGGL((nce_slice_kernel<false, false>), dim3(pl.S, pl.QB), dim3(kThreads), 0, s, d);
    hipLaunchKernelGGL(nce_combine_kernel, dim3((d.B + (kThreads >> 6) - 1) / (kThreads >> 6)), dim3(kThreads), 0, s, d);
    prof_mark(prof, 1, s);
    hipError_t e = hipGetLastError();
    if (e != hipSuccess) { snprintf(g_err, kErrLen, "gcc_nce_forward: %s", hipGetErrorString(e)); return -10; }
    return 0;
}

int32_t gcc_nce_backward(const gcc_nce_args *a, const float *dloss, int32_t by_mem_row, float *dq, void *workspace,
                         int64_t workspace_bytes, gcc_prof *prof, void *stream)
{
    NceDev d;
    Plan pl;
    int rc = fill_dev(a, workspace, workspace_bytes, d, pl);
    if (rc) return rc;
    if (!dloss || !dq || (by_mem_row && a->pos_mode != 1)) {
        snprintf(g_err, kErrLen, "gcc_nce_backward: bad argument");
        return -1;
    }
    d.dloss = dloss; d.by_mem_row = by_mem_row; d.dq = dq;
    hipStream_t s = (hipStream_t)stream;
    prof_mark(prof, 0, s);
    if (d.bf16) hipLaunchKernelGGL((nce_slice_kernel<true, true>), dim3(pl.S, pl.QB), dim3(kThreads), 0, s, d);
    else hipLaunchKernelGGL((nce_slice_kernel<true, false>), dim3(pl.S, pl.QB), dim3(kThreads), 0, s, d);
    hipLaunchKernelGGL(nce_dq_kernel, dim3((a->B * 16 + kThreads - 1) / kThreads), dim3(kThreads), 0, s, d);
    prof_mark(prof, 1, s);
    hipError_t e = hipGetLastError();
    if (e != hipSuccess) { snprintf(g_err, kErrLen, "gcc_nce_backward: %s", hipGetErrorString(e)); return -10; }
    return 0;
}

int32_t gcc_queue_enqueue(float *mem, int32_t K, const float *keys, int32_t nkeys, int32_t index, float *saved,
                          void *stream)
{
    if (!mem || !keys || K < 1 || nkeys < 1 || nkeys > K || index < 0 || index >= K) {
        snprintf(g_err, kErrLen, "gcc_queue_enqueue: bad argument (K=%d n=%d index=%d)", K, nkeys, index);
        return -1;
    }
    hipLaunchKernelGGL(queue_enqueue_kernel, dim3((nkeys * 16 + kThreads - 1) / kThreads), dim3(kThreads), 0,
                       (hipStream_t)stream, mem, K, keys, nkeys, index, saved, (const gcc_step_scalars *)nullptr);
    return hipGetLastError() == hipSuccess ? 0 : -10;
}

int32_t gcc_queue_enqueue_scalars(float *mem, int32_t K, const float *keys, int32_t nkeys, const gcc_step_scalars *scalars,
                                  void *stream)
{
    if (!mem || !keys || !scalars || K < 1 || nkeys < 1 || nkeys > K) {
        snprintf(g_err, kErrLen, "gcc_queue_enqueue_scalars: bad argument (K=%d n=%d)", K, nkeys);
        return -1;
    }
    hipLaunchKernelGGL(queue_enqueue_kernel, dim3((nkeys * 16 + kThreads - 1) / kThreads), dim3(kThreads), 0,
                       (hipStream_t)stream, mem, K, keys, nkeys, 0, (float *)nullptr, scalars);
    return hipGetLastError() == hipSuccess ? 0 : -10;
}

__global__ void step_scalars_kernel(gcc_step_scalars *dev, gcc_step_scalars v) { *dev = v; }

__global__ void step_scalars_fetch_kernel(gcc_step_scalars *dev, const gcc_step_scalars *ring, int ring_len,
                                          unsigned long long *counter)
{
    const unsigned long long n = *counter;
    const uint32_t *src = (const uint32_t *)(ring + (n % (unsigned long long)ring_len));
    uint32_t *dst = (uint32_t *)dev;
#pragma unroll
    for (int i = 0; i < (int)(sizeof(gcc_step_scalars) / 4); ++i) dst[i] = load_system_u32(src + i);
    *counter = n + 1;
}

static void fill_scalars(gcc_step_scalars &v, float lr, float beta1, float beta2, int32_t adam_step, int32_t enqueue_index,
                         uint64_t dropout_seed)
{
    v.lr = lr;
    v.bias_corr1 = 1.0f - powf(beta1, (float)adam_step);
    v.bias_corr2_sqrt = sqrtf(1.0f - powf(beta2, (float)adam_step));
    v.enqueue_index = enqueue_index;
    v.dropout_seed = dropout_seed;
}

void gcc_step_scalars_fill(gcc_step_scalars *host_entry, float lr, float beta1, float beta2, int32_t adam_step,
                           int32_t enqueue_index, uint64_t dropout_seed)
{
    gcc_step_scalars v;
    fill_scalars(v, lr, beta1, beta2, adam_step, enqueue_index, dropout_seed);
    memcpy(host_entry, &v, sizeof(v));
    __atomic_thread_fence(__ATOMIC_RELEASE);
}

int32_t gcc_step_scalars_fetch(gcc_step_scalars *dev, const gcc_step_scalars *ring, int32_t ring_len,
                               unsigned long long *counter, void *stream)
{
    if (!dev || !ring || !counter || ring_len < 1) {
        snprintf(g_err, kErrLen, "gcc_step_scalars_fetch: bad argument");
        return -1;
    }
    hipLaunchKernelGGL(step_scalars_fetch_kernel, dim3(1), dim3(1), 0, (hipStream_t)stream, dev, ring, (int)ring_len, counter);
    return hipGetLastError() == hipSuccess ? 0 : -10;
}

int32_t gcc_step_scalars_set(gcc_step_scalars *dev, float lr, float beta1, float beta2, int32_t adam_step,
                             int32_t enqueue_index, uint64_t dropout_seed, void *stream)
{
    if (!dev || adam_step < 1 || enqueue_index < 0) {
        snprintf(g_err, kErrLen, "gcc_step_scalars_set: bad argument");
        return -1;
    }
    gcc_step_scalars v;
    fill_scalars(v, lr, beta1, beta2, adam_step, enqueue_index, dropout_seed);
    hipLaunchKernelGGL(step_scalars_kernel, dim3(1), dim3(1), 0, (hipStream_t)stream, dev, v);
    return hipGetLastError() == hipSuccess ? 0 : -10;
}

int32_t gcc_adam_step(float *param, float *grad, float *exp_avg, float *exp_avg_sq, int64_t n, float lr,
                      float beta1, float beta2, float eps, float weight_decay, int32_t step, float max_norm,
                      float grad_scale, float *grad_norm, double *scratch, void *stream)
{
    if (!param || !grad || !exp_avg || !exp_avg_sq || !grad_norm || !scratch || n < 1 || step < 1 || !(grad_scale > 0.f)) {
        snprintf(g_err, kErrLen, "gcc_adam_step: bad argument");
        return -1;
    }
    hipStream_t s = (hipStream_t)stream;
    const float bc1 = 1.0f - powf(beta1, (float)step);
    const float bc2_sqrt = sqrtf(1.0f - powf(beta2, (float)step));
    hipLaunchKernelGGL(gradnorm_kernel, dim3(kNormBlocks), dim3(kThreads), 0, s, (const float *)grad, n, scratch);
    int blocks = (int)((n + kThreads - 1) / kThreads);
    if (blocks > 512) blocks = 512;
    const AdamExtras none = {};
    hipLaunchKernelGGL(adam_kernel, dim3(blocks), dim3(kThreads), 0, s, param, grad, exp_avg, exp_avg_sq, n, lr, beta1,
                       beta2, eps, weight_decay, bc1, bc2_sqrt, max_norm, grad_scale, (const double *)scratch, grad_norm, none);
    return hipGetLastError() == hipSuccess ? 0 : -10;
}

static int32_t adam_ema_launch(const char *who, float *param, float *grad, float *exp_avg, float *exp_avg_sq, int64_t n, float lr,
                               float beta1, float beta2, float eps, float weight_decay, int32_t step, float max_norm,
                               float grad_scale, float *grad_norm, double *scratch, float *ema, int64_t n_ema, float ema_m,
                               const gcc_step_meters_args *meters, const gcc_step_scalars *scalars, void *stream)
{
    if (!param || !grad || !exp_avg || !exp_avg_sq || !grad_norm || !scratch || n < 1 || (!scalars && step < 1) || !(grad_scale > 0.f) ||
        (ema && n_ema < n) ||
        (meters && (!meters->acc || !meters->mx || !meters->loss || !meters->prob || !meters->node_off_q ||
                    !meters->edge_off_q || !meters->node_off_k || meters->batch_size < 1))) {
        snprintf(g_err, kErrLen, "%s: bad argument", who);
        return -1;
    }
    hipStream_t s = (hipStream_t)stream;
    const float bc1 = scalars ? 1.f : 1.0f - powf(beta1, (float)step);
    const float bc2_sqrt = scalars ? 1.f : sqrtf(1.0f - powf(beta2, (float)step));
    hipLaunchKernelGGL(gradnorm_kernel, dim3(kNormBlocks), dim3(kThreads), 0, s, (const float *)grad, n, scratch);
    AdamExtras x = {};
    x.sc = scalars;
    if (ema) { x.ema = ema; x.n_ema = n_ema; x.ema_m = ema_m; }
    if (meters) {
        x.acc = meters->acc; x.mx = meters->mx; x.loss = meters->loss; x.prob = meters->prob;
        x.node_off_q = meters->node_off_q; x.edge_off_q = meters->edge_off_q; x.node_off_k = meters->node_off_k;
        x.B = meters->batch_size;
    }
    const int64_t nmax = ema ? n_ema : n;
    int blocks = (int)((nmax + kThreads - 1) / kThreads);
    if (blocks > 512) blocks = 512;
    hipLaunchKernelGGL(adam_kernel, dim3(blocks), dim3(kThreads), 0, s, param, grad, exp_avg, exp_avg_sq, n, lr, beta1,
                       beta2, eps, weight_decay, bc1, bc2_sqrt, max_norm, grad_scale, (const double *)scratch, grad_norm, x);
    return hipGetLastError() == hipSuccess ? 0 : -10;
}

int32_t gcc_adam_ema_step(float *param, float *grad, float *exp_avg, float *exp_avg_sq, int64_t n, float lr,
                          float beta1, float beta2, float eps, float weight_decay, int32_t step, float max_norm,
                          float grad_scale, float *grad_norm, double *scratch, float *ema, int64_t n_ema, float ema_m,
                          const gcc_step_meters_args *meters, void *stream)
{
    return adam_ema_launch("gcc_adam_ema_step", param, grad, exp_avg, exp_avg_sq, n, lr, beta1, beta2, eps, weight_decay, step,
                           max_norm, grad_scale, grad_norm, scratch, ema, n_ema, ema_m, meters, nullptr, stream);
}

int32_t gcc_adam_ema_step_scalars(float *param, float *grad, float *exp_avg, float *exp_avg_sq, int64_t n,
                                  float beta1, float beta2, float eps, float weight_decay, float max_norm,
                                  float grad_scale, float *grad_norm, double *scratch, float *ema, int64_t n_ema, float ema_m,
                                  const gcc_step_meters_args *meters, const gcc_step_scalars *scalars, void *stream)
{
    if (!scalars) { snprintf(g_err, kErrLen, "gcc_adam_ema_step_scalars: scalars is NULL"); return -1; }
    return adam_ema_launch("gcc_adam_ema_step_scalars", param, grad, exp_avg, exp_avg_sq, n, 0.f, beta1, beta2, eps, weight_decay,
                           0, max_norm, grad_scale, grad_norm, scratch, ema, n_ema, ema_m, meters, scalars, stream);
}

int32_t gcc_step_meters(double *acc, int32_t *mx, const float *loss, const float *prob, const float *grad_norm,
                        const int32_t *node_off_q, const int32_t *edge_off_q, const int32_t *node_off_k,
                        int32_t batch_size, void *stream)
{
    if (!acc || !mx || !loss || !prob || !grad_norm || !node_off_q || !edge_off_q || !node_off_k || batch_size < 1) {
        snprintf(g_err, kErrLen, "gcc_step_meters: bad argument");
        return -1;
    }
    hipLaunchKernelGGL(step_meters_kernel, dim3(1), dim3(64), 0, (hipStream_t)stream, acc, mx, loss, prob, grad_norm,
                       node_off_q, edge_off_q, node_off_k, batch_size);
    return hipGetLastError() == hipSuccess ? 0 : -10;
}

int32_t gcc_ema_update(float *ema, const float *p, int64_t n, float m, void *stream)
{
    if (!ema || !p || n < 1) { snprintf(g_err, kErrLen, "gcc_ema_update: bad argument"); return -1; }
    int blocks = (int)((n + kThreads - 1) / kThreads);
    if (blocks > 1024) blocks = 1024;
    hipLaunchKernelGGL(ema_kernel, dim3(blocks), dim3(kThreads), 0, (hipStream_t)stream, ema, p, n, m);
    return hipGetLastError() == hipSuccess ? 0 : -10;
}

}
```

gcc_amd/encoder.py:

```python
from __future__ import annotations

import ctypes

import torch
import torch.nn as nn

from . import _cabi

H = _cabi.GIN_HIDDEN
STATS_REPLICAS = 16
STALE_SLOT_MSG = ("backward of a GraphEncoder forward whose activations were overwritten: at most two forward passes that need "
                  "a backward (grad enabled, training mode) may be pending per encoder -- run backward before a third one; passes "
                  "under torch.no_grad() or in eval mode keep a workspace of their own and may run at any time")


class _MLP(nn.Module):
    def __init__(self, d_in, d_hid, d_out):
        super().__init__()
        self.linears = nn.ModuleList([nn.Linear(d_in, d_hid), nn.Linear(d_hid, d_out)])
        self.batch_norms = nn.ModuleList([nn.BatchNorm1d(d_hid)])


class _ApplyNodeFunc(nn.Module):
    def __init__(self, mlp, d):
# ... 181 lines not shown
            raise RuntimeError(f"gcc_gat_backward_workspace_bytes failed ({nbytes}): {self.lib.gcc_last_error().decode()}")
        ws = torch.empty(nbytes, dtype=torch.uint8, device=dout.device)
        grads = _fill_struct(_cabi.GccGatGrads(), [(n, i, t) for (n, i, _), t in zip(gat_params(enc), targets)], self.ptr)
        dout = dout.contiguous()
        rc = self.lib.gcc_gat_backward(ctypes.byref(p), ctypes.byref(w), self.ptr(dout), ctypes.byref(grads), int(accumulate),
                                       self.ptr(ws), nbytes, stream)
        if rc != 0:
            raise RuntimeError(f"gcc_gat_backward failed ({rc}): {self.lib.gcc_last_error().decode()}")
        return targets


class GinEngine:

    def __init__(self, lib=None, ptr=None):
        self.lib = lib if lib is not None else _cabi.load()
        self.ptr = ptr if ptr is not None else _cabi.dev_ptr
        self._bufs = {}
        self._gen = {}
        self.rows_hint = None

    def hint_rows(self, n, margin=1.10):
        want = int(n * margin) + 64
        if self.rows_hint is None or want > self.rows_hint:
            self.rows_hint = want

    def _buffers(self, key, node_cap, B, L, device):
        k = (key, node_cap, B, L, str(device))
        if k not in self._bufs:
            f32 = dict(dtype=torch.float32, device=device)
            self._bufs[k] = dict(
                x0=torch.zeros(node_cap, H, **f32),
                agg=[torch.zeros(node_cap, H, **f32) for _ in range(L)],
                z1=[torch.zeros(node_cap, H, **f32) for _ in range(L)],
                z2=[torch.zeros(node_cap, H, **f32) for _ in range(L)],
                stats=torch.zeros(L, 3, STATS_REPLICAS, 2, H, dtype=torch.float64, device=device),
                bn_totals=torch.zeros(L * 3 * 2 * H, dtype=torch.float64, device=device),
                pooled=torch.zeros(L + 1, B, H, dtype=torch.float64, device=device),
                score=torch.zeros(B, H, **f32), feat=torch.zeros(B, H, **f32))
        return self._bufs[k]

    def make_pass(self, enc, g, training, keep=None, slot=0, dropout_seed=None, scalars=None, backward=True):
        ptr = self.ptr
        L = len(enc.gnn.ginlayers)
        enc.ensure_padded()
        node_cap = g.parent_nid.numel() if hasattr(g, "parent_nid") else g.graph_id.numel()
        buf = self._buffers(slot, node_cap, g.batch_size, L, g.node_off.device)
        p = _cabi.GccGinPass()
        p.node_off, p.row_ptr, p.col_idx, p.graph_id = ptr(g.node_off), ptr(g.row_ptr), ptr(g.col_idx), ptr(g.graph_id)
        if g.pos_undirected is None:
            raise RuntimeError("the batch has no pos_undirected (run the positional embedding first)")
        p.pos = ptr(g.pos_undirected)
        p.batch_size = g.batch_size
        p.training = int(training)
        p.update_running_stats = int(training)
        p.normalize = int(enc.norm)
        p.dropout_keep = ptr(keep) if keep is not None else None
        p.dropout_philox = int(keep is None and dropout_seed is not None)
        p.dropout_seed = int(dropout_seed or 0) & 0xFFFFFFFFFFFFFFFF
        p.w = fill_weights(enc, ptr)
        p.x0 = ptr(buf["x0"])
        for i in range(L):
            p.agg[i], p.z1[i], p.z2[i] = (ptr(buf["agg"][i]) if backward else None), ptr(buf["z1"][i]), ptr(buf["z2"][i])
        p.stats, p.pooled, p.score, p.feat = ptr(buf["stats"]), ptr(buf["pooled"]), ptr(buf["score"]), ptr(buf["feat"])
        p.edge_multiplicity = int(getattr(g, "edge_multiplicity", 1))
        p.bn_totals = ptr(buf["bn_totals"]) if training else None
        seed_local = getattr(g, "seed_local", None)
        p.seed_local = ptr(seed_local) if seed_local is not None else None
        p.scalars = ptr(scalars) if scalars is not None else None
        p.node_cap = node_cap
        if self.rows_hint is None:
            self.hint_rows(int(g.node_off[g.batch_size].item()))
        p.rows_hint = int(self.rows_hint or 0)
        key = (slot, node_cap, g.batch_size, L, str(g.node_off.device))
        self._gen[key] = self._gen.get(key, 0) + 1
        buf = dict(buf)
        buf["_keepalive"] = (g, keep, enc)
        buf["_slot"] = (key, self._gen[key])
        return p, buf

    def slot_is_current(self, buf):
        key, gen = buf["_slot"]
        return self._gen.get(key) == gen

    def forward(self, passes, stream=None, prof=None):
        arr = (_cabi.GccGinPass * len(passes))(*passes)
        rc = self.lib.gcc_gin_forward(arr, len(passes), prof.handle if prof is not None else None, stream)
        if rc != 0:
            raise RuntimeError(f"gcc_gin_forward failed ({rc}): {self.lib.gcc_last_error().decode()}")


    def eval_fused(self, passes, mean_out=None, stream=None):
        arr = (_cabi.GccGinPass * len(passes))(*passes)
        rc = self.lib.gcc_gin_eval_fused(arr, len(passes), self.ptr(mean_out) if mean_out is not None else None, stream)
        if rc != 0:
            raise RuntimeError(f"gcc_gin_eval_fused failed ({rc}): {self.lib.gcc_last_error().decode()}")

    def backward(self, enc, p, buf, dfeat, targets=None, accumulate=False, stream=None, prof=None):
        ptr = self.ptr
        L = len(enc.gnn.ginlayers)
        g = buf["_keepalive"][0]
        node_cap = g.parent_nid.numel() if hasattr(g, "parent_nid") else g.graph_id.numel()
        nbytes = self.lib.gcc_gin_backward_workspace_bytes(node_cap, p.batch_size, L)
        key = ("bwd", nbytes, str(dfeat.device))
        if key not in self._bufs:
            self._bufs[key] = torch.empty(nbytes, dtype=torch.uint8, device=dfeat.device)
        ws = self._bufs[key]
        grads = _cabi.GccGinGrads()
        plist = grad_params(enc)
        if targets is None:
            targets = []
            for _, _, param in plist:
                if param.grad is None or (enc.is_padded() and not getattr(param.grad, "_gcc_padded", False)):
                    param.grad = enc.padded_zeros_like(param)
                targets.append(param.grad)
        for (name, idx, _), tgt in zip(plist, targets):
            if idx is None:
                setattr(grads, name, ptr(tgt))
            else:
                getattr(grads, name)[idx] = ptr(tgt)
        dfeat = dfeat.contiguous()
        rc = self.lib.gcc_gin_backward(ctypes.byref(p), ptr(dfeat), ctypes.byref(grads), int(accumulate),
                                       ptr(ws), nbytes, node_cap, prof.handle if prof is not None else None, stream)
        if rc != 0:
            raise RuntimeError(f"gcc_gin_backward failed ({rc}): {self.lib.gcc_last_error().decode()}")
        return targets


class GraphEncoder(nn.Module):

    def __init__(self, positional_embedding_size=32, max_node_freq=8, max_edge_freq=8, max_degree=128,
                 freq_embedding_size=32, degree_embedding_size=32, output_dim=32, node_hidden_dim=32,
                 edge_hidden_dim=32, num_layers=6, num_heads=4, num_step_set2set=6, num_layer_set2set=3,
                 norm=False, gnn_model="mpnn", degree_input=False, lstm_as_gate=False):
        super().__init__()
        if gnn_model not in ("gin", "gat"):
            raise NotImplementedError(f"gnn_model={gnn_model!r}: gcc_amd runs the \"gin\" (train.py:77 default) and \"gat\" "
                                      "backbones (\"mpnn\" does not run in the reference: graph_encoder.py:188 feeds "
                                      "e_feat=None to NNConv)")
        if not degree_input:
            raise NotImplementedError("train.py:617 always passes degree_input=True")
        if node_hidden_dim < 1 or output_dim < 1:
            raise ValueError(f"hidden / output size must be positive (got {node_hidden_dim} / {output_dim})")
        node_input_dim = positional_embedding_size + degree_embedding_size + 1
        if gnn_model == "gat":
            self._init_gat(positional_embedding_size, max_node_freq, max_edge_freq, max_degree, degree_embedding_size,
                           output_dim, node_hidden_dim, num_layers, num_heads, num_step_set2set, num_layer_set2set, norm)
            return
        self.wide = node_hidden_dim > H or output_dim > H or node_input_dim > H
        if num_layers - 1 > _cabi.GIN_MAX_LAYERS:
            raise NotImplementedError("too many GIN layers")
        self.gnn = _UnsupervisedGIN(num_layers, node_input_dim, node_hidden_dim, output_dim, final_dropout=0.5)
        self.gnn_model = gnn_model
        self.max_node_freq, self.max_edge_freq = max_node_freq, max_edge_freq
        self.max_degree = max_degree
        self.degree_input = degree_input
        self.positional_embedding_size = positional_embedding_size
        self.degree_embedding_size = degree_embedding_size
        self.degree_embedding = nn.Embedding(max_degree + 1, degree_embedding_size)
        self.set2set = _Set2Set(node_hidden_dim, num_layer_set2set)
        self.lin_readout = nn.Sequential(nn.Linear(2 * node_hidden_dim, node_hidden_dim), nn.ReLU(),
                                         nn.Linear(node_hidden_dim, output_dim))
        self.norm = norm
        self.hidden, self.output_dim = int(node_hidden_dim), int(output_dim)
        self._pad_ptrs = {}
        self.fused_eval = True
        self._engine = None
        self._wide_engine = None
        self._slot = id(self)
        self._calls = 0

    def _init_gat(self, pos, max_node_freq, max_edge_freq, max_degree, deg_emb, output_dim, hidden, num_layers, num_heads,
                  num_step_set2set, num_layer_set2set, norm):
        node_input_dim = pos + deg_emb + 1
        if hidden > H or output_dim > H or hidden % num_heads != 0:
            raise NotImplementedError(f"the GAT kernels serve hidden and output sizes up to {H} with hidden % num_heads == 0 "
                                      f"(got hidden {hidden}, output {output_dim}, {num_heads} heads)")
        if node_input_dim > H:
            raise NotImplementedError(f"the GAT kernels take input features up to {H} columns (positional + degree "
                                      f"embedding + 1 = {node_input_dim})")
        if not 1 <= num_layers <= _cabi.GAT_MAX_LAYERS or not 1 <= num_layer_set2set <= _cabi.GAT_MAX_S2S_LAYERS \
                or num_step_set2set < 1:
            raise NotImplementedError(f"the GAT kernels serve 1..{_cabi.GAT_MAX_LAYERS} GAT layers, 1.."
                                      f"{_cabi.GAT_MAX_S2S_LAYERS} LSTM layers and at least one Set2Set step")
        self.wide = False
        self.gnn = _UnsupervisedGAT(node_input_dim, hidden, num_layers, num_heads)
        self.gnn_model = "gat"
        self.max_node_freq, self.max_edge_freq = max_node_freq, max_edge_freq
        self.max_degree = max_degree
        self.degree_input = True
        self.positional_embedding_size = pos
        self.degree_embedding_size = deg_emb
        self.degree_embedding = nn.Embedding(max_degree + 1, deg_emb)
        self.set2set = _Set2Set(hidden, num_layer_set2set)
        self.set2set.lstm.reset_parameters()
        self.lin_readout = nn.Sequential(nn.Linear(2 * hidden, hidden), nn.ReLU(), nn.Linear(hidden, output_dim))
        self.norm = norm
        self.hidden, self.output_dim = int(hidden), int(output_dim)
        self.num_heads, self.num_step_set2set = int(num_heads), int(num_step_set2set)
        self._pad_ptrs = {}
        self.fused_eval = False
        self._engine = None
        self._wide_engine = None
        self._slot = id(self)
# ... 134 lines not shown
```

gcc_amd/train_step.py:

```python
from __future__ import annotations

import os
import time

import torch

from .contrast import MemoryMoCo, NceEngine
from .encoder import GraphEncoder, H, grad_params


def flatten_parameters(enc: GraphEncoder):
    if getattr(enc, "_flat", None) is not None:
        return enc._flat, enc._n_live
    live = [p for _, _, p in grad_params(enc)]
    live_ids = {id(p) for p in live}
    dead = [p for p in enc.parameters() if id(p) not in live_ids]
    pn = getattr(enc, "padded_numel", lambda t: t.numel())
    n_live = sum(pn(p) for p in live)
    total = n_live + sum(p.numel() for p in dead)
    dev = live[0].device
    flat = torch.zeros(total, dtype=torch.float32, device=dev)
    off = 0
    with torch.no_grad():
        for p in live + dead:
# ... 155 lines not shown
            if ev is not None:
                if not ev.query():
                    t_wait = time.perf_counter()
                    ev.synchronize()
                    self.late_chunks += 1
                    self.late_wait_s += time.perf_counter() - t_wait
            elif hasattr(sampler, "snapshot_sync"):
                sampler.snapshot_sync()
            bits = sampler.read_snapshot(self.snap[c][0])
            if not bits:
                self.snap.pop(c)
                break
            if attempts == 4:
                raise RuntimeError(f"sampler overflow persists after growing {attempts} times (chunk {c})")
            self._reproduce(c, bits)
            attempts += 1
        pairs, ev = self.ready[c]
        if ev is not None:
            torch.cuda.current_stream(self.dev).wait_event(ev)
            self.ready[c] = (pairs, None)
        return pairs[step - c * self.chunk]

    def release(self, step):
        c = step // self.chunk
        if step == (c + 1) * self.chunk - 1:
            self.ready.pop(c, None)
            if self.cuda:
                ev = torch.cuda.Event()
                ev.record(torch.cuda.current_stream(self.dev))
                self.released[c] = ev


_CAPTURE_ERROR_MARKS = ("capture", "hipErrorStreamCapture", "cudaErrorStreamCapture", "operation not permitted when stream is capturing",
                        "operation failed due to a previous error during capture")


def _is_capture_error(e):
    msg = str(e)
    return any(m in msg for m in _CAPTURE_ERROR_MARKS)


def _hint_rows_once(engine, q, k):
    if not hasattr(engine, "hint_rows"):
        return
    _hint_rows_once_(engine, q, k)


def _hint_rows_once_(engine, q, k):
    if engine.rows_hint is None:
        B = q.batch_size
        engine.hint_rows(max(int(q.node_off[B].item()), int(k.node_off[B].item())))


def _meter_buffers(dev):
    return torch.zeros(5, dtype=torch.float64, device=dev), torch.zeros(2, dtype=torch.int32, device=dev)


def read_meters(trainer):
    if hasattr(trainer, "join"):
        trainer.join()
    a, m = trainer.meter_acc.tolist(), trainer.meter_max.tolist()
    trainer.meter_acc.zero_()
    trainer.meter_max.zero_()
    if hasattr(getattr(trainer, "gin", None), "hint_rows") and m[0] > 0:
        before = trainer.gin.rows_hint
        trainer.gin.hint_rows(m[0], margin=1.04)
        if before is not None and trainer.gin.rows_hint > before and getattr(trainer, "graphs", None):
            trainer._retired_graphs = list(trainer.graphs.values())
            trainer.graphs = {}
    return a, m


class FlatAdam:

    def __init__(self, param, grad, lr, betas, weight_decay, clip_norm, engine, eps=1e-8):
        self.param, self.grad, self.engine = param, grad, engine
        self.param_groups = [dict(lr=lr, betas=tuple(betas), eps=eps, weight_decay=weight_decay)]
        self.clip_norm = clip_norm
        self.exp_avg = torch.zeros_like(param)
        self.exp_avg_sq = torch.zeros_like(param)
        self.steps = 0
        self.grad_norm = torch.zeros(1, dtype=torch.float32, device=param.device)
        self._scratch = torch.zeros(64, dtype=torch.float64, device=param.device)

    def step(self, grad_scale=1.0, ema=None, ema_src=None, ema_m=0.0, meters=None, scalars=None):
        g = self.param_groups[0]
        self.steps += 1
        st = torch.cuda.current_stream(self.param.device).cuda_stream if self.param.is_cuda else None
        if ema is None and meters is None and scalars is None:
            self.engine.adam(self.param, self.grad, self.exp_avg, self.exp_avg_sq, g["lr"], g["betas"], g["eps"],
                             g["weight_decay"], self.steps, self.clip_norm, self.grad_norm, self._scratch, stream=st,
                             grad_scale=grad_scale)
        else:
            self.engine.adam_ema(self.param, self.grad, self.exp_avg, self.exp_avg_sq, g["lr"], g["betas"], g["eps"],
                                 g["weight_decay"], self.steps, self.clip_norm, self.grad_norm, self._scratch, stream=st,
                                 grad_scale=grad_scale, ema=ema, ema_src=ema_src, ema_m=ema_m, meters=meters, scalars=scalars)
        return self.grad_norm

    def zero_grad(self):
        pass

    def state_dict(self):
        return dict(state=dict(step=self.steps, exp_avg=self.exp_avg, exp_avg_sq=self.exp_avg_sq),
                    param_groups=self.param_groups)


class _GraphedStep:

    RING_LEN = 2048

    def _graph_init(self, graph):
        self.relaxed_streams = False
        self._joined_caller = False
        self.use_scalars = False
        self.use_graph = bool(self.prefetch) if graph is None else bool(graph)
        if self.use_graph and self.collectives and self._staged_possible():
            if graph:
                raise ValueError("graph replay with collectives needs RCCL on device buffers (not the gloo staging path)")
            self.use_graph = False
        if self.use_graph and self.dev.type != "cuda":
            raise ValueError("graph replay needs a device")
        if self.use_graph and self.main is None:
            self.main = torch.cuda.Stream(self.dev, priority=-1)
        self.scalars = torch.zeros(24, dtype=torch.uint8, device=self.dev)
        self.ring_len = int(self.RING_LEN)
        self.ring = torch.zeros(24 * self.ring_len, dtype=torch.uint8)
        if self.dev.type == "cuda":
            self.ring = self.ring.pin_memory()
        self.ring_count = 0
        self.ring_counter = torch.zeros(1, dtype=torch.int64, device=self.dev)
        self._ring_events = []
        self._ring_dirty = False
        self.graphs = {}
        self._graphs_regrown = 0
        self._retired_graphs = []
        self.graph_replays = 0

    def _staged_possible(self):
        return bool(torch.distributed.is_available() and torch.distributed.is_initialized()
                    and torch.distributed.get_backend() == "gloo")

    def _slot_key(self, q, k):
        return tuple(t.data_ptr() for g in (q, k) for t in (g.node_off, g.edge_off, g.row_ptr, g.col_idx, g.graph_id,
                                                            g.pos_undirected))

    def _ring_guard(self):
        if self.dev.type != "cuda":
            return
        n = self.ring_count
        every = max(1, self.ring_len // 8)
        if n % every == 0:
            ev = torch.cuda.Event()
            ev.record(torch.cuda.current_stream(self.dev))
            self._ring_events.append((n, ev))
        while self._ring_events and self._ring_events[0][0] <= n - (self.ring_len * 3) // 4:
            self._ring_events.pop(0)[1].synchronize()

    @staticmethod
    def _run_segments(body_out):
        segments, result = body_out
        for _, fn in segments:
            fn()
        return result()

    def _run_step(self, q, k, lr, seed, enqueue_index, explicit_masks, pr, st, body):
        step_marks = any(n in pr for n in ("gin_fwd", "nce_fwd", "nce_bwd", "gin_bwd"))
        graphed = self.use_graph and not explicit_masks and not step_marks
        scalars = self.scalars if (graphed or self.use_scalars) and not explicit_masks else None
        if self._ring_dirty:
            torch.cuda.synchronize(self.dev)
            self.ring_counter.fill_(self.ring_count)
            self._ring_dirty = False
        regrown = getattr(getattr(self, "producer", None), "regrown", 0)
        if regrown != self._graphs_regrown:
            self._retired_graphs = list(self.graphs.values())
            self.graphs = {}
            self._graphs_regrown = regrown
        try:
            if scalars is not None:
# ... 20 lines not shown
            self._capture(key, body)
            if first_ever:
                self._precapture_ready(st)
            return out
        except Exception:
            self._ring_dirty = scalars is not None
            raise

    def _capture(self, key, body):
        steps0 = self.optimizer.steps
        self._drain_collectives()
        try:
            segments, result = body(self.scalars, {})
            items, pool = [], None
            for capturable, fn in segments:
                if not capturable:
                    items.append(fn)
                    continue
                gobj = torch.cuda.CUDAGraph()
                mode = os.environ.get("GCC_CAPTURE_MODE") or "thread_local"
                gobj.capture_begin(capture_error_mode=mode, **({} if pool is None else dict(pool=pool)))
                try:
                    fn()
                finally:
                    gobj.capture_end()
                pool = pool or gobj.pool()
                items.append(gobj)
            cap = result()
        except RuntimeError as e:
            if not _is_capture_error(e):
                raise
            self.graph_capture_failures = getattr(self, "graph_capture_failures", 0) + 1
            import warnings
            if self.graph_capture_failures > 4:
                self.use_graph = False
                warnings.warn(f"step graph capture failed {self.graph_capture_failures} times ({e}); graph replay is switched off")
            else:
                warnings.warn(f"step graph capture failed ({e}); the slot stays eager")
            try:
                torch.cuda.synchronize(self.dev)
            except RuntimeError:
                pass
            return False
        finally:
            self.optimizer.steps = steps0
        self.graphs[key] = (items, dict(loss=cap["loss"], prob=cap["prob"], grad_norm=cap["grad_norm"]))
        return True

    def _drain_collectives(self):
        if not self.collectives or self.dev.type != "cuda":
            return
        dist = torch.distributed
        if not (dist.is_available() and dist.is_initialized()) or dist.get_backend() != "nccl":
            return
        torch.cuda.synchronize(self.dev)
        wait = getattr(dist.group.WORLD, "_wait_for_pending_works", None)
        if wait is not None:
            wait()
        else:
            import time
            time.sleep(0.25)

    def _precapture_ready(self, st):
        prod = getattr(self, "producer", None)
        if prod is None or not hasattr(self, "_capture_body"):
            return
        self.graphs_precaptured = 0
        for c in sorted(prod.ready):
            pairs, _ev = prod.ready[c]
            for q, k in pairs:
                key = self._slot_key(q, k)
                if key not in self.graphs and self._capture(key, self._capture_body(q, k, st)):
                    self.graphs_precaptured += 1

    def _fetch_scalars(self, scalars, st):
        if scalars is not None:
            self.nce.fetch_scalars(scalars, self.ring, self.ring_len, self.ring_counter, stream=st)


class MoCoTrainStep(_GraphedStep):
    def __init__(self, model: GraphEncoder, model_ema: GraphEncoder, contrast: MemoryMoCo, sampler, posemb,
                 learning_rate=0.005, betas=(0.9, 0.999), weight_decay=1e-5, clip_norm=1.0, alpha=0.999,
                 world_size=1, rank=0, prefetch=True, extra_lanes=(), depth=2, lanes=None, chunk=1, reserved_cus=0, cu_layout="interleaved",
                 collectives=None, ahead=None, graph=None, flat_engine=None):
        self.model, self.ema, self.contrast = model, model_ema, contrast
        self.sampler, self.posemb = sampler, posemb
        self.clip_norm, self.alpha = clip_norm, alpha
        self.world, self.rank = world_size, rank
        self.collectives = world_size > 1 if collectives is None else bool(collectives)
        self.dev = next(model.parameters()).device
        self.flat, self.n_live = flatten_parameters(model)
        self.flat_ema, n2 = flatten_parameters(model_ema)
        assert n2 == self.n_live and self.flat.numel() == self.flat_ema.numel()
        self.flat_grad = torch.zeros(self.n_live, dtype=torch.float32, device=self.dev)
        self.grad_views, off = [], 0
        for _, _, p in grad_params(model):
            self.grad_views.append(self.flat_grad[off:off + p.numel()].view_as(p))
            off += model.padded_numel(p)
        self.live = self.flat[: self.n_live]
        self.wide = bool(model.wide or contrast.wide)
        if self.wide and not (model.wide and contrast.wide and model_ema.wide):
            raise ValueError("a wide step needs a wide encoder pair AND a wide head (hidden-size and MemoryMoCo's feature size above 64)")
        self.gin = model.wide_engine() if self.wide else model.engine()
        self.nce = contrast.engine()
        self.optimizer = FlatAdam(self.live, self.flat_grad, learning_rate, betas, weight_decay, clip_norm,
                                  (flat_engine or NceEngine()) if self.wide else self.nce)
        self.mask_fn = None
        self.dropout_seed = 0x5EED0000
        self.B = sampler.batch_size
        if contrast.queueSize < self.B * world_size:
            raise ValueError(f"nce_k = {contrast.queueSize} is smaller than the {self.B * world_size} keys enqueued per step "
                             f"(batch_size {self.B} x world {world_size}): raise --nce-k")
        self.L = len(model.gnn.ginlayers)
        self.keys_all = torch.empty(self.B * world_size, contrast.inputSize if self.wide else H, device=self.dev) if self.collectives else None
        self.one = torch.ones(1, device=self.dev)
        self.meter_acc, self.meter_max = _meter_buffers(self.dev)
        self.prefetch = prefetch and self.dev.type == "cuda"
        self.main = torch.cuda.Stream(self.dev, priority=-1) if self.prefetch else None
        lanes = list(lanes) if lanes is not None else [(sampler, posemb)] + list(extra_lanes)
        self.producer = BatchProducer(lanes if self.prefetch else lanes[:1], self._first_id,
                                      self.dev if self.prefetch else "cpu", depth=depth if self.prefetch else 1,
                                      chunk=chunk if self.prefetch else 1, reserved_cus=reserved_cus, cu_layout=cu_layout,
                                      ahead=ahead)
        if not self.prefetch:
            self.producer.cuda = False
        if self.wide and graph:
            raise ValueError("graph replay is the 64-channel step's (device-resident scalars); the wide step is issued launch by launch")
        self._graph_init(False if self.wide else graph)
        model.train()
        model_ema.eval()
        for mod in model_ema.modules():
            if isinstance(mod, torch.nn.BatchNorm1d):
                mod.train()

    def _first_id(self, step):
        return (step * self.world + self.rank) * self.B

    def check_status(self, strict_posemb=False):
        flags, err = 0, None
        for lane in self.producer.lanes:
            smp, pe = lane[0], lane[1]
            try:
                if hasattr(smp, "check_status"):
                    smp.check_status()
                if hasattr(pe, "check_status"):
                    flags |= int(pe.check_status(strict=strict_posemb) or 0)
            except RuntimeError as e:
                err = err or e
        if self.collectives and torch.distributed.is_initialized():
            t = torch.tensor([1 if err is not None else 0, flags], dtype=torch.int64,
                             device="cpu" if self._staged() or self.dev.type != "cuda" else self.dev)
            every = [torch.zeros_like(t) for _ in range(torch.distributed.get_world_size())]
            torch.distributed.all_gather(every, t)
            any_err, flags = 0, 0
            for e in every:
                e = e.tolist()
                any_err |= int(e[0])
                flags |= int(e[1])
            if err is None and any_err:
                err = RuntimeError("another rank reported a sampler / positional-embedding overflow (see its log)")
        if err is not None:
            raise err
        return flags

    def _staged(self):
        return self.dev.type == "cuda" and torch.distributed.get_backend() == "gloo"

    def _all_gather_begin(self, out, x):
# ... 33 lines not shown

    def join(self):
        if self.main is not None:
            torch.cuda.current_stream(self.dev).wait_stream(self.main)
            self._joined_caller = False

    def _step(self, step, lr, prof=None):
        pr = prof or {}
        self._release_pending()
        q, k = self.producer.get(step, prof=prof)
        _hint_rows_once(self.gin, q, k)
        st = torch.cuda.current_stream(self.dev).cuda_stream if self.dev.type == "cuda" else None
        p_drop = self.model.gnn.drop.p
        keep = self.mask_fn() if self.mask_fn is not None else None
        seed = (self.dropout_seed + step * 0x9E3779B97F4A7C15) & 0xFFFFFFFFFFFFFFFF if p_drop > 0 else None
        c = self.contrast
        for grp in self.optimizer.param_groups:
            grp["lr"] = lr
        out = self._run_step(q, k, lr, seed, c.index, keep is not None, pr, st,
                             lambda scalars, marks: self._body(q, k, keep, seed, scalars, marks, st))
        c.index = (c.index + self.B * (self.world if self.collectives else 1)) % c.queueSize
        self._pending_release = step
        return dict(out, graph_q=q, graph_k=k)

    def _release_pending(self):
        step = getattr(self, "_pending_release", None)
        if step is not None:
            self._pending_release = None
            self.producer.release(step)

    def _body_wide(self, q, k, keep, S, st):
        c, enc = self.contrast, self.model
        p_drop = enc.gnn.drop.p

        def fwd():
            kq = keep
            if kq is None and p_drop > 0:
                kq = (torch.rand(len(enc.gnn.ginlayers) + 1, self.B, enc.output_dim, device=self.dev) >= p_drop).float()
            S["pq"], S["bufq"] = self.gin.make_pass(enc, q, training=True, keep=kq, slot=("step", 0))
            S["pk"], S["bufk"] = self.gin.make_pass(self.ema, k, training=True, keep=None, slot=("step", 1))
            self.gin.forward(S["pq"], stream=st)
            self.gin.forward(S["pk"], stream=st)
            self.last_bufs = (S["bufq"], S["bufk"])

        def gather_begin():
            S["gathering"] = self._all_gather_begin(self.keys_all, S["bufk"]["feat"])

        def head_and_backward():
            S["outs"] = self.nce.forward(S["bufq"]["feat"], S["bufk"]["feat"], c.memory, c.T, 0, stream=st)
            self.gin.backward(enc, S["pq"], S["outs"]["grad_rows"], self.grad_views, stream=st)

        def reduce_and_join():
            self._all_reduce(self.flat_grad)
            self._all_gather_end(S["gathering"])

        def update():
            outs = S["outs"]
            S["gnorm"] = self.optimizer.step(grad_scale=1.0 / self.world if self.collectives else 1.0,
                                             ema=self.flat_ema, ema_src=self.flat, ema_m=self.alpha,
                                             meters=(self.meter_acc, self.meter_max, outs["loss"], outs["prob"], q, k), scalars=None)
            keys = self.keys_all if self.collectives else S["bufk"]["feat"]
            self.nce.enqueue(c.memory, keys, c.index, stream=st)

        def result():
            return dict(loss=S["outs"]["loss"], prob=S["outs"]["prob"], grad_norm=S["gnorm"])

        if self.collectives:
            segments = [(False, fwd), (False, gather_begin), (False, head_and_backward), (False, reduce_and_join), (False, update)]
        else:
            segments = [(False, lambda: (fwd(), head_and_backward(), update()))]
        return segments, result

    def _capture_body(self, q, k, st):
        seed = 0 if self.model.gnn.drop.p > 0 else None
        return lambda scalars, marks: self._body(q, k, None, seed, scalars, marks, st)

    def _body(self, q, k, keep, seed, scalars, pr, st):
        S = {}
        c = self.contrast
        if self.wide:
            return self._body_wide(q, k, keep, S, st)

        def fwd():
            self._fetch_scalars(scalars, st)
            S["pq"], S["bufq"] = self.gin.make_pass(self.model, q, training=True, keep=keep, slot=("step", 0),
                                                    dropout_seed=(0 if seed is not None else None) if scalars is not None else seed,
                                                    scalars=scalars)
            S["pk"], S["bufk"] = self.gin.make_pass(self.ema, k, training=True, keep=None, slot=("step", 1), backward=False)
            self.gin.forward([S["pq"], S["pk"]], stream=st, prof=pr.get("gin_fwd"))

        def gather_begin():
            S["gathering"] = self._all_gather_begin(self.keys_all, S["bufk"]["feat"])

        def head_and_backward():
            feat_q, feat_k = S["bufq"]["feat"], S["bufk"]["feat"]
            S["outs"] = self.nce.forward(feat_q, feat_k, c.kernel_memory(), c.T, 0, stream=st, prof=pr.get("nce_fwd"))
            dq = self.nce.backward(feat_q, feat_k, c.kernel_memory(), c.T, 0, S["outs"], self.one, stream=st,
                                   prof=pr.get("nce_bwd"))
            self.gin.backward(self.model, S["pq"], S["bufq"], dq, targets=self.grad_views, stream=st, prof=pr.get("gin_bwd"))

        def reduce_and_join():
            self._all_reduce(self.flat_grad)
            self._all_gather_end(S["gathering"])

        def update():
            outs = S["outs"]
            S["gnorm"] = self.optimizer.step(grad_scale=1.0 / self.world if self.collectives else 1.0,
                                             ema=self.flat_ema, ema_src=self.flat, ema_m=self.alpha,
                                             meters=(self.meter_acc, self.meter_max, outs["loss"], outs["prob"], q, k),
                                             scalars=scalars)
            keys = self.keys_all if self.collectives else S["bufk"]["feat"]
            self.nce.enqueue(c.kernel_memory(), keys, c.index, save=False, stream=st, scalars=scalars)

        def result():
            return dict(loss=S["outs"]["loss"], prob=S["outs"]["prob"], grad_norm=S["gnorm"])

        if self.collectives:
            segments = [(True, fwd), (False, gather_begin), (True, head_and_backward), (False, reduce_and_join), (True, update)]
        else:
            segments = [(True, lambda: (fwd(), head_and_backward(), update()))]
        return segments, result


class E2ETrainStep(_GraphedStep):

    def __init__(self, model: GraphEncoder, sampler, posemb, nce_t=0.07, learning_rate=0.005, betas=(0.9, 0.999),
                 weight_decay=1e-5, clip_norm=1.0, prefetch=True, depth=2, lanes=None, chunk=1, ahead=None, engine=None,
                 graph=None):
        self.model = model
        self.sampler, self.posemb = sampler, posemb
        self.T, self.clip_norm = nce_t, clip_norm
        self.world, self.rank, self.collectives = 1, 0, False
        self.dev = next(model.parameters()).device
        self.flat, self.n_live = flatten_parameters(model)
        self.flat_grad = torch.zeros(self.n_live, dtype=torch.float32, device=self.dev)
        self.grad_views, off = [], 0
        for _, _, p in grad_params(model):
            self.grad_views.append(self.flat_grad[off:off + p.numel()].view_as(p))
            off += model.padded_numel(p)
        self.live = self.flat[: self.n_live]
        self.gin = model.engine()
        self.nce = engine if engine is not None else NceEngine()
        self.optimizer = FlatAdam(self.live, self.flat_grad, learning_rate, betas, weight_decay, clip_norm, self.nce)
        self.mask_fn = None
        self.dropout_seed = 0x5EED0000
        self.B = sampler.batch_size
        self.one = torch.ones(1, device=self.dev)
        self.meter_acc, self.meter_max = _meter_buffers(self.dev)
        self.prefetch = prefetch and self.dev.type == "cuda"
        self.main = torch.cuda.Stream(self.dev, priority=-1) if self.prefetch else None
        lanes = list(lanes) if lanes is not None else [(sampler, posemb)]
        self.producer = BatchProducer(lanes if self.prefetch else lanes[:1], self._first_id,
                                      self.dev if self.prefetch else "cpu", depth=depth if self.prefetch else 1,
                                      chunk=chunk if self.prefetch else 1, ahead=ahead)
        if not self.prefetch:
            self.producer.cuda = False
        self._graph_init(False if graph is None else graph)
        model.train()

    def _first_id(self, step):
        return step * self.B

    _staged = MoCoTrainStep._staged
    check_status = MoCoTrainStep.check_status
    step = MoCoTrainStep.step
    join = MoCoTrainStep.join

    def _step(self, step, lr, prof=None):
        pr = prof or {}
        self._release_pending()
        q, k = self.producer.get(step, prof=prof)
        _hint_rows_once(self.gin, q, k)
        st = torch.cuda.current_stream(self.dev).cuda_stream if self.dev.type == "cuda" else None
        p_drop = self.model.gnn.drop.p
        keep_q, keep_k = self.mask_fn() if self.mask_fn is not None else (None, None)
        s0 = (self.dropout_seed + 2 * step * 0x9E3779B97F4A7C15) & 0xFFFFFFFFFFFFFFFF if p_drop > 0 else None
        for grp in self.optimizer.param_groups:
            grp["lr"] = lr
        out = self._run_step(q, k, lr, s0, 0, keep_q is not None, pr, st,
                             lambda scalars, marks: self._body(q, k, keep_q, keep_k, s0, scalars, marks, st))
        self._pending_release = step
        return dict(out, graph_q=q, graph_k=k)

    _release_pending = MoCoTrainStep._release_pending

    def _capture_body(self, q, k, st):
        s0 = 0 if self.model.gnn.drop.p > 0 else None
        return lambda scalars, marks: self._body(q, k, None, None, s0, scalars, marks, st)

# ... 27 lines not shown
```

include/gcc_amd.h:

```cpp
#ifndef GCC_AMD_H
#define GCC_AMD_H

#include <stdint.h>

#ifdef __cplusplus
extern "C" {
#endif

#define GCC_AMD_ABI_VERSION 3

#define GCC_STATUS_SCRATCH_OVERFLOW 1
#define GCC_STATUS_NODE_OVERFLOW    2
#define GCC_STATUS_EDGE_OVERFLOW    4

int32_t gcc_abi_version(void);
const char *gcc_last_error(void);

typedef struct gcc_prof gcc_prof;
gcc_prof *gcc_prof_create(int32_t num_marks);
void gcc_prof_destroy(gcc_prof *p);
int32_t gcc_prof_elapsed_ms(gcc_prof *p, int32_t from_mark, int32_t to_mark, float *ms);

int32_t gcc_stream_create_cu_mask(const uint32_t *cu_mask, int32_t words, void **stream);
int32_t gcc_debug_load(int32_t kind, int32_t workgroups, int32_t threads, int32_t lds_bytes, int64_t ticks, int32_t max_iters,
// ... 74 lines not shown
int64_t gcc_posemb_multi_workspace_bytes(int32_t num_views, int32_t batch_size, int64_t node_cap, int32_t hidden);
int32_t gcc_posemb_multi(const gcc_posemb_view *views, int32_t num_views, int32_t batch_size, int64_t node_cap,
                         int32_t hidden, uint64_t seed, void *workspace, int64_t workspace_bytes, int32_t *status,
                         gcc_prof *prof, void *stream);
int32_t gcc_posemb_multi_gated(const gcc_posemb_view *views, int32_t num_views, int32_t batch_size, int64_t node_cap,
                               int32_t hidden, uint64_t seed, void *workspace, int64_t workspace_bytes, int32_t *status,
                               gcc_prof *prof, void *heavy_wait, void *heavy_record, void *stream);

void gcc_posemb_set_fork(int32_t mode);

#define GCC_POSEMB_TICK_CLASSES 8
void gcc_posemb_debug_ticks(long long *device_ticks64);
void gcc_gin_debug_ticks(long long *device_ticks64);

#define GCC_GIN_MAX_LAYERS 8
#define GCC_GIN_HIDDEN 64
#define GCC_GIN_STAT_REPLICAS 16

typedef struct gcc_bn {
    const float *weight, *bias;
    float *running_mean, *running_var;
    int64_t *num_batches_tracked;
} gcc_bn;

typedef struct gcc_gin_weights {
    int32_t num_gin_layers;
    int32_t pos_dim, deg_emb_dim, max_degree;
    const float *degree_embedding;
    const float *lin0_w[GCC_GIN_MAX_LAYERS];
    const float *lin0_b[GCC_GIN_MAX_LAYERS];
    const float *lin1_w[GCC_GIN_MAX_LAYERS];
    const float *lin1_b[GCC_GIN_MAX_LAYERS];
    gcc_bn bn_a[GCC_GIN_MAX_LAYERS];
    gcc_bn bn_b[GCC_GIN_MAX_LAYERS];
    gcc_bn bn_c[GCC_GIN_MAX_LAYERS];
    const float *pred_w[GCC_GIN_MAX_LAYERS + 1];
    const float *pred_b[GCC_GIN_MAX_LAYERS + 1];
    float bn_eps, bn_momentum;
    float dropout_p;
    float norm_eps;
    int32_t hidden;
} gcc_gin_weights;

typedef struct gcc_step_scalars {
    float lr, bias_corr1, bias_corr2_sqrt;
    int32_t enqueue_index;
    uint64_t dropout_seed;
} gcc_step_scalars;
int32_t gcc_step_scalars_set(gcc_step_scalars *dev, float lr, float beta1, float beta2, int32_t adam_step,
                             int32_t enqueue_index, uint64_t dropout_seed, void *stream);
void gcc_step_scalars_fill(gcc_step_scalars *host_entry, float lr, float beta1, float beta2, int32_t adam_step,
                           int32_t enqueue_index, uint64_t dropout_seed);
int32_t gcc_step_scalars_fetch(gcc_step_scalars *dev, const gcc_step_scalars *ring, int32_t ring_len,
                               unsigned long long *counter, void *stream);

typedef struct gcc_gin_pass {
    const int32_t *node_off, *row_ptr, *col_idx, *graph_id;
    const float *pos;
    int32_t batch_size;
    int32_t training;
    int32_t update_running_stats;
    int32_t normalize;
    const float *dropout_keep;
    uint64_t dropout_seed;
    int32_t dropout_philox;
    gcc_gin_weights w;
    float *x0;
    float *agg[GCC_GIN_MAX_LAYERS];
    float *z1[GCC_GIN_MAX_LAYERS];
    float *z2[GCC_GIN_MAX_LAYERS];
    double *stats;
    double *pooled;
    float *score;
    float *feat;
    int32_t edge_multiplicity;
    double *bn_totals;
    const int32_t *seed_local;
    const gcc_step_scalars *scalars;
    int64_t node_cap;
    int64_t rows_hint;
} gcc_gin_pass;

int32_t gcc_gin_forward(const gcc_gin_pass *passes, int32_t npass, gcc_prof *prof, void *stream);

int32_t gcc_gin_eval_fused(const gcc_gin_pass *passes, int32_t npass, float *mean_out, void *stream);
void gcc_gin_eval_debug_ticks(long long *device_ticks64);

typedef struct gcc_gin_grads {
    float *degree_embedding;
    float *lin0_w[GCC_GIN_MAX_LAYERS], *lin0_b[GCC_GIN_MAX_LAYERS];
    float *lin1_w[GCC_GIN_MAX_LAYERS], *lin1_b[GCC_GIN_MAX_LAYERS];
    float *bn_a_w[GCC_GIN_MAX_LAYERS], *bn_a_b[GCC_GIN_MAX_LAYERS];
    float *bn_b_w[GCC_GIN_MAX_LAYERS], *bn_b_b[GCC_GIN_MAX_LAYERS];
    float *bn_c_w[GCC_GIN_MAX_LAYERS], *bn_c_b[GCC_GIN_MAX_LAYERS];
    float *pred_w[GCC_GIN_MAX_LAYERS + 1], *pred_b[GCC_GIN_MAX_LAYERS + 1];
} gcc_gin_grads;

int64_t gcc_gin_backward_workspace_bytes(int64_t node_cap, int32_t batch_size, int32_t num_gin_layers);

int32_t gcc_gin_backward(const gcc_gin_pass *pass, const float *dfeat, const gcc_gin_grads *grads,
                         int32_t accumulate, void *workspace, int64_t workspace_bytes, int64_t node_cap,
                         gcc_prof *prof, void *stream);

typedef struct gcc_ginx_pass {
    const int32_t *node_off, *row_ptr, *col_idx, *graph_id;
    const float *pos;
    const int32_t *seed_local;
    int32_t batch_size;
    int32_t training;
    int32_t update_running_stats;
    int32_t normalize;
    const float *dropout_keep;
    int32_t hidden, out_dim;
    int32_t edge_multiplicity;
    int32_t reserved_;
    int64_t node_cap;
    gcc_gin_weights w;
    void *workspace;
    int64_t workspace_bytes;
    float *feat;
    float *pooled_out;
} gcc_ginx_pass;
int64_t gcc_ginx_workspace_bytes(int64_t node_cap, int32_t batch_size, int32_t num_gin_layers, int32_t d_in, int32_t hidden,
                                 int32_t out_dim);
int32_t gcc_ginx_forward(const gcc_ginx_pass *p, void *stream);
int32_t gcc_ginx_backward(const gcc_ginx_pass *p, const float *dfeat, const gcc_gin_grads *grads, void *stream);

int32_t gcc_ncex_forward(const float *q, const float *k, const float *mem, int32_t B, int32_t K, int32_t D, float inv_T, int32_t mode,
                         float *out, float *dlog, float *grad_rows, float *grad_mem, float *loss, float *prob, double *acc, void *stream);
int32_t gcc_queue_enqueue_x(float *mem, int32_t K, int32_t D, const float *keys, int32_t nkeys, int32_t index, void *stream);

#define GCC_GINW_HIDDEN 256
#define GCC_GINW_MAX_NODES 128
#define GCC_STATUS_GINW_TOO_LARGE 32
#define GCC_STATUS_GINW_BAD_EDGE 64
typedef struct gcc_ginw_layer {
    const uint16_t *w0, *w1;
    const float *s0, *t0, *s1, *t1, *s2, *t2;
    const uint16_t *w0_frag, *w1_frag;
} gcc_ginw_layer;
typedef struct gcc_ginw_args {
    const int32_t *node_off;
    const int32_t *row_ptr, *col_idx;
    const uint16_t *x_in;
    uint16_t *x_out;
    float *pooled;
    int32_t batch_size, num_layers;
    gcc_ginw_layer layers[GCC_GIN_MAX_LAYERS];
    void *scratch;
    int64_t scratch_bytes;
    int64_t num_nodes;
} gcc_ginw_args;
int64_t gcc_ginw_scratch_bytes(int64_t num_nodes, int32_t batch_size);
int32_t gcc_ginw_forward(const gcc_ginw_args *a, int32_t *status, gcc_prof *prof, void *stream);
int32_t gcc_ginw_pack_weights(const uint16_t *w, uint16_t *w_frag, int32_t which, void *stream);
void gcc_ginw_debug_ticks(long long *device_ticks64);

#define GCC_NCE_DIM 64
typedef struct gcc_nce_args {
    const float *q;
    const float *k;
    const float *mem;
    const float *patch;
    int32_t patch_index;
    int32_t patch_rows;
    int32_t B, K;
    int32_t pos_mode;
    float inv_T;
    float *lse, *pos;
    float *loss, *prob;
    float *out_dense;
    int32_t dtype;
} gcc_nce_args;
#define GCC_NCE_F32 0
#define GCC_NCE_BF16 1

int64_t gcc_nce_workspace_bytes(int32_t B, int32_t K);
int32_t gcc_nce_forward(const gcc_nce_args *a, void *workspace, int64_t workspace_bytes, gcc_prof *prof,
                        void *stream);
int32_t gcc_nce_backward(const gcc_nce_args *a, const float *dloss, int32_t by_mem_row, float *dq,
                         void *workspace, int64_t workspace_bytes, gcc_prof *prof, void *stream);

int32_t gcc_queue_enqueue(float *mem, int32_t K, const float *keys, int32_t nkeys, int32_t index, float *saved,
                          void *stream);

int32_t gcc_adam_step(float *param, float *grad, float *exp_avg, float *exp_avg_sq, int64_t n, float lr,
                      float beta1, float beta2, float eps, float weight_decay, int32_t step, float max_norm,
                      float grad_scale, float *grad_norm, double *scratch, void *stream);

int32_t gcc_step_meters(double *acc, int32_t *mx, const float *loss, const float *prob, const float *grad_norm,
                        const int32_t *node_off_q, const int32_t *edge_off_q, const int32_t *node_off_k,
                        int32_t batch_size, void *stream);

int32_t gcc_ema_update(float *ema, const float *p, int64_t n, float m, void *stream);

typedef struct {
    double *acc;
    int32_t *mx;
    const float *loss, *prob;
    const int32_t *node_off_q, *edge_off_q, *node_off_k;
    int32_t batch_size;
} gcc_step_meters_args;
int32_t gcc_adam_ema_step(float *param, float *grad, float *exp_avg, float *exp_avg_sq, int64_t n, float lr,
                          float beta1, float beta2, float eps, float weight_decay, int32_t step, float max_norm,
                          float grad_scale, float *grad_norm, double *scratch, float *ema, int64_t n_ema, float ema_m,
                          const gcc_step_meters_args *meters, void *stream);
int32_t gcc_adam_ema_step_scalars(float *param, float *grad, float *exp_avg, float *exp_avg_sq, int64_t n,
                                  float beta1, float beta2, float eps, float weight_decay, float max_norm,
                                  float grad_scale, float *grad_norm, double *scratch, float *ema, int64_t n_ema, float ema_m,
                                  const gcc_step_meters_args *meters, const gcc_step_scalars *scalars, void *stream);
int32_t gcc_queue_enqueue_scalars(float *mem, int32_t K, const float *keys, int32_t nkeys,
                                  const gcc_step_scalars *scalars, void *stream);

typedef struct gcc_cls_head_args {
    const float *feat;
    const float *W;
    const float *b;
    const int32_t *labels;
    int32_t B, D, C, ld_feat, ld_dfeat;
    float *logits;
    float *dlogits;
    float *dW, *db;
    float *dfeat;
    float *loss;
    int32_t *correct;
    double *meter_acc;
    int32_t *meter_max;
    const int32_t *node_off, *edge_off;
    double *eval_loss_sum;
    int32_t *eval_counts;
} gcc_cls_head_args;
int32_t gcc_cls_head_train(const gcc_cls_head_args *args, void *stream);
int32_t gcc_cls_head_eval(const gcc_cls_head_args *args, void *stream);

int32_t gcc_adam_clipvalue_step(float *param, float *grad, float *exp_avg, float *exp_avg_sq, int64_t n, float lr,
                                float beta1, float beta2, float eps, float weight_decay, int32_t step, float clip_value,
                                float grad_scale, void *stream);

#define GCC_GAT_MAX_LAYERS 8
#define GCC_GAT_MAX_S2S_LAYERS 8

typedef struct gcc_gat_weights {
    int32_t num_layers, hidden, heads, out_dim;
    int32_t pos_dim, deg_emb_dim, max_degree;
    int32_t s2s_iters, s2s_layers;
    int32_t normalize;
    float norm_eps;
    const float *degree_embedding;
    const float *fc[GCC_GAT_MAX_LAYERS];
    const float *attn_l[GCC_GAT_MAX_LAYERS];
    const float *attn_r[GCC_GAT_MAX_LAYERS];
    const float *w_ih[GCC_GAT_MAX_S2S_LAYERS];
    const float *w_hh[GCC_GAT_MAX_S2S_LAYERS];
    const float *b_ih[GCC_GAT_MAX_S2S_LAYERS];
    const float *b_hh[GCC_GAT_MAX_S2S_LAYERS];
    const float *ro0_w, *ro0_b;
    const float *ro2_w, *ro2_b;
} gcc_gat_weights;

typedef struct gcc_gat_grads {
    float *degree_embedding;
    float *fc[GCC_GAT_MAX_LAYERS], *attn_l[GCC_GAT_MAX_LAYERS], *attn_r[GCC_GAT_MAX_LAYERS];
    float *w_ih[GCC_GAT_MAX_S2S_LAYERS], *w_hh[GCC_GAT_MAX_S2S_LAYERS];
    float *b_ih[GCC_GAT_MAX_S2S_LAYERS], *b_hh[GCC_GAT_MAX_S2S_LAYERS];
    float *ro0_w, *ro0_b, *ro2_w, *ro2_b;
} gcc_gat_grads;

typedef struct gcc_gat_pass {
    const int32_t *node_off, *row_ptr, *col_idx;
    const int32_t *seed_local;
    const float *pos;
    int32_t batch_size, node_cap, edge_multiplicity, reserved_;
    float *saved;
    float *out;
} gcc_gat_pass;

int64_t gcc_gat_saved_floats(const gcc_gat_weights *w, int32_t node_cap, int32_t batch_size);
int32_t gcc_gat_forward(const gcc_gat_pass *p, const gcc_gat_weights *w, void *stream);
int64_t gcc_gat_backward_workspace_bytes(const gcc_gat_weights *w, int32_t node_cap, int32_t batch_size);
int32_t gcc_gat_backward(const gcc_gat_pass *p, const gcc_gat_weights *w, const float *dout, const gcc_gat_grads *g,
                         int32_t accumulate, void *workspace, int64_t workspace_bytes, void *stream);

#ifdef __cplusplus
}
#endif
#endif
```

Baseline: 701,200.

## Fold scalar fetch, grad sum-of-squares and queue enqueue into neighboring kernels

Moves the per-step scalar fetch from the host-visible ring into the first GIN feature kernel. The gradient-finalization kernel now also emits per-block sum-of-squares partials, and the Adam/EMA step consumes those partials and performs the MoCo queue enqueue in the same launch. An optional one-pass NCE forward+backward entry point is added but off by default. The aim is fewer kernel launches and no separate grad-norm reduction pass per training step, at the cost of extra block reductions and more complex coupling between kernels.

```diff
diff --git a/gcc_amd/_cabi.py b/gcc_amd/_cabi.py
--- a/gcc_amd/_cabi.py
+++ b/gcc_amd/_cabi.py
@@ -256,10 +256,15 @@
                                     ctypes.c_void_p, ctypes.c_void_p]),
     "gcc_gin_forward": (ctypes.c_int32, [ctypes.POINTER(GccGinPass), ctypes.c_int32, ctypes.c_void_p,
                                          ctypes.c_void_p]),
+    "gcc_gin_forward_fetch": (ctypes.c_int32, [ctypes.POINTER(GccGinPass), ctypes.c_int32, ctypes.c_void_p, ctypes.c_void_p,
+                                               ctypes.c_int32, ctypes.c_void_p, ctypes.c_void_p, ctypes.c_void_p]),
     "gcc_gin_backward_workspace_bytes": (ctypes.c_int64, [ctypes.c_int64, ctypes.c_int32, ctypes.c_int32]),
     "gcc_gin_backward": (ctypes.c_int32, [ctypes.POINTER(GccGinPass), ctypes.c_void_p, ctypes.POINTER(GccGinGrads),
                                           ctypes.c_int32, ctypes.c_void_p, ctypes.c_int64, ctypes.c_int64,
                                           ctypes.c_void_p, ctypes.c_void_p]),
+    "gcc_gin_backward_sumsq": (ctypes.c_int32, [ctypes.POINTER(GccGinPass), ctypes.c_void_p, ctypes.POINTER(GccGinGrads),
+                                                ctypes.c_void_p, ctypes.c_int64, ctypes.c_int64, ctypes.c_void_p, ctypes.c_int32,
+                                                c_i32p, ctypes.c_void_p, ctypes.c_void_p]),
     "gcc_ginx_workspace_bytes": (ctypes.c_int64, [ctypes.c_int64, ctypes.c_int32, ctypes.c_int32, ctypes.c_int32, ctypes.c_int32, ctypes.c_int32]),
     "gcc_ginx_forward": (ctypes.c_int32, [ctypes.POINTER(GccGinxPass), ctypes.c_void_p]),
     "gcc_ginx_backward": (ctypes.c_int32, [ctypes.POINTER(GccGinxPass), ctypes.c_void_p, ctypes.POINTER(GccGinGrads), ctypes.c_void_p]),
@@ -275,6 +280,8 @@
     "gcc_nce_backward": (ctypes.c_int32, [ctypes.POINTER(GccNceArgs), ctypes.c_void_p, ctypes.c_int32,
                                           ctypes.c_void_p, ctypes.c_void_p, ctypes.c_int64, ctypes.c_void_p,
                                           ctypes.c_void_p]),
+    "gcc_nce_forward_backward": (ctypes.c_int32, [ctypes.POINTER(GccNceArgs), ctypes.c_void_p, ctypes.c_void_p, ctypes.c_void_p,
+                                                  ctypes.c_int64, ctypes.c_void_p, ctypes.c_void_p, ctypes.c_void_p]),
     "gcc_queue_enqueue": (ctypes.c_int32, [ctypes.c_void_p, ctypes.c_int32, ctypes.c_void_p, ctypes.c_int32,
                                            ctypes.c_int32, ctypes.c_void_p, ctypes.c_void_p]),
     "gcc_adam_step": (ctypes.c_int32, [ctypes.c_void_p, ctypes.c_void_p, ctypes.c_void_p, ctypes.c_void_p,
@@ -291,6 +298,13 @@
                                                    ctypes.c_float, ctypes.c_float, ctypes.c_float, ctypes.c_void_p,
                                                    ctypes.c_void_p, ctypes.c_void_p, ctypes.c_int64, ctypes.c_float,
                                                    ctypes.POINTER(GccStepMetersArgs), ctypes.c_void_p, ctypes.c_void_p]),
+    "gcc_adam_ema_enqueue_step_scalars": (ctypes.c_int32, [ctypes.c_void_p, ctypes.c_void_p, ctypes.c_void_p, ctypes.c_void_p,
+                                                           ctypes.c_int64, ctypes.c_float, ctypes.c_float, ctypes.c_float,
+                                                           ctypes.c_float, ctypes.c_float, ctypes.c_float, ctypes.c_void_p,
+                                                           ctypes.c_void_p, ctypes.c_void_p, ctypes.c_int64, ctypes.c_float,
+                                                           ctypes.POINTER(GccStepMetersArgs), ctypes.c_void_p, ctypes.c_void_p,
+                                                           ctypes.c_int32, ctypes.c_void_p, ctypes.c_int32, ctypes.c_void_p,
+                                                           ctypes.c_int32, ctypes.c_void_p]),
     "gcc_queue_enqueue_scalars": (ctypes.c_int32, [ctypes.c_void_p, ctypes.c_int32, ctypes.c_void_p, ctypes.c_int32,
                                                    ctypes.c_void_p, ctypes.c_void_p]),
     "gcc_ginw_scratch_bytes": (ctypes.c_int64, [ctypes.c_int64, ctypes.c_int32]),
diff --git a/gcc_amd/contrast.py b/gcc_amd/contrast.py
--- a/gcc_amd/contrast.py
+++ b/gcc_amd/contrast.py
@@ -67,6 +67,29 @@
             raise RuntimeError(f"gcc_nce_backward failed ({rc}): {self.lib.gcc_last_error().decode()}")
         return dq
 
+    def one_pass(self):
+        return self.dtype == "f32"
+
+    def forward_backward(self, q, k, mem, T, dloss, patch=None, patch_index=0, stream=None, prof_fwd=None, prof_bwd=None):
+        if not self.one_pass():
+            outs = self.forward(q, k, mem, T, 0, patch=patch, patch_index=patch_index, stream=stream, prof=prof_fwd)
+            return outs, self.backward(q, k, mem, T, 0, outs, dloss, patch=patch, patch_index=patch_index, stream=stream,
+                                       prof=prof_bwd)
+        B, K = q.shape[0], mem.shape[0]
+        f32 = dict(dtype=torch.float32, device=q.device)
+        outs = dict(lse=torch.empty(B, **f32), pos=torch.empty(B, **f32), loss=torch.empty(1, **f32), prob=torch.empty(1, **f32),
+                    out=None)
+        dq = torch.empty_like(q)
+        ws, nbytes = self._workspace(B, K, q.device)
+        a = self._args(q, k, mem, 1.0 / T, 0, patch, patch_index, outs, None)
+        dloss = dloss.reshape(1).to(torch.float32).contiguous()
+        rc = self.lib.gcc_nce_forward_backward(ctypes.byref(a), self.ptr(dloss), self.ptr(dq), self.ptr(ws), nbytes,
+                                               prof_fwd.handle if prof_fwd else None, prof_bwd.handle if prof_bwd else None,
+                                               stream)
+        if rc != 0:
+            raise RuntimeError(f"gcc_nce_forward_backward failed ({rc}): {self.lib.gcc_last_error().decode()}")
+        return outs, dq
+
     def set_scalars(self, scalars, lr, betas, adam_step, enqueue_index, dropout_seed, stream=None):
         rc = self.lib.gcc_step_scalars_set(self.ptr(scalars), float(lr), float(betas[0]), float(betas[1]), int(adam_step),
                                            int(enqueue_index), int(dropout_seed) & 0xFFFFFFFFFFFFFFFF, stream)
@@ -106,7 +129,8 @@
             raise RuntimeError(f"gcc_adam_step failed ({rc}): {self.lib.gcc_last_error().decode()}")
 
     def adam_ema(self, param, grad, exp_avg, exp_avg_sq, lr, betas, eps, weight_decay, step, max_norm, grad_norm,
-                 scratch, stream=None, grad_scale=1.0, ema=None, ema_src=None, ema_m=0.0, meters=None, scalars=None):
+                 scratch, stream=None, grad_scale=1.0, ema=None, ema_src=None, ema_m=0.0, meters=None, scalars=None,
+                 sumsq_parts=None, enqueue=None):
         ma = None
         if meters is not None:
             acc, mx, loss, prob, q, k = meters
@@ -114,6 +138,22 @@
                                          self.ptr(q.edge_off), self.ptr(k.node_off), int(q.batch_size))
         if ema is not None and (ema_src is None or ema_src.data_ptr() != param.data_ptr() or ema.numel() != ema_src.numel()):
             raise ValueError("adam_ema: param must be a prefix of ema_src, and ema the same size as ema_src")
+        if (sumsq_parts is not None or enqueue is not None) and scalars is None:
+            raise ValueError("adam_ema: sumsq_parts / enqueue are the device-resident-scalars step's")
+        if sumsq_parts is not None or enqueue is not None:
+            parts, nparts = sumsq_parts if sumsq_parts is not None else (None, 0)
+            queue, keys = enqueue if enqueue is not None else (None, None)
+            rc = self.lib.gcc_adam_ema_enqueue_step_scalars(
+                self.ptr(param), self.ptr(grad), self.ptr(exp_avg), self.ptr(exp_avg_sq), param.numel(), float(betas[0]),
+                float(betas[1]), float(eps), float(weight_decay), float(max_norm), float(grad_scale), self.ptr(grad_norm),
+                self.ptr(scratch), self.ptr(ema) if ema is not None else None, ema.numel() if ema is not None else 0,
+                float(ema_m), ctypes.byref(ma) if ma is not None else None, self.ptr(scalars),
+                self.ptr(parts) if parts is not None else None, int(nparts),
+                self.ptr(queue) if queue is not None else None, queue.shape[0] if queue is not None else 0,
+                self.ptr(keys) if keys is not None else None, keys.shape[0] if keys is not None else 0, stream)
+            if rc != 0:
+                raise RuntimeError(f"gcc_adam_ema_enqueue_step_scalars failed ({rc}): {self.lib.gcc_last_error().decode()}")
+            return
         if scalars is not None:
             rc = self.lib.gcc_adam_ema_step_scalars(
                 self.ptr(param), self.ptr(grad), self.ptr(exp_avg), self.ptr(exp_avg_sq), param.numel(), float(betas[0]),
diff --git a/gcc_amd/csrc/encoder.hip b/gcc_amd/csrc/encoder.hip
--- a/gcc_amd/csrc/encoder.hip
+++ b/gcc_amd/csrc/encoder.hip
@@ -11,7 +11,8 @@
     int32_t B, pos_dim, emb_dim, max_degree, mult;
     int32_t cap;
 };
-struct FeatLaunch { FeatArgs p[kMaxPass]; };
+struct FeatFetch { gcc_step_scalars *dev; const gcc_step_scalars *ring; unsigned long long *counter; int32_t ring_len; };
+struct FeatLaunch { FeatArgs p[kMaxPass]; FeatFetch f; };
 
 __global__ __launch_bounds__(kThreads) void gin_feat_kernel(FeatLaunch L)
 {
@@ -36,6 +37,16 @@
     const int tf = first_tile();
     request(tf * kTile);
     const int N = a.node_off[a.B];
+    constexpr int kScWords = (int)(sizeof(gcc_step_scalars) / 4);
+    const bool fetch = L.f.ring && blockIdx.x == 0 && blockIdx.y == 0 && tid == 0;
+    uint32_t scw[kScWords];
+    unsigned long long step_n = 0;
+    if (fetch) {
+        step_n = *L.f.counter;
+        const uint32_t *src = (const uint32_t *)(L.f.ring + (step_n % (unsigned long long)L.f.ring_len));
+#pragma unroll
+        for (int i = 0; i < kScWords; ++i) scw[i] = load_system_u32(src + i);
+    }
     SCHED_FENCE();
     {
         const float4 z4 = make_float4(0.f, 0.f, 0.f, 0.f);
@@ -75,6 +86,12 @@
             }
             st4(a.x0 + (int64_t)vv[i] * H + 4 * t, x);
         }
+    }
+    if (fetch) {
+        uint32_t *dst = (uint32_t *)L.f.dev;
+#pragma unroll
+        for (int i = 0; i < kScWords; ++i) dst[i] = scw[i];
+        *L.f.counter = step_n + 1;
     }
 }
 
@@ -536,7 +553,7 @@
 
 extern "C" void gcc_gin_debug_ticks(long long *device_ticks64) { g_gin_ticks = device_ticks64; }
 
-extern "C" int32_t gcc_gin_forward(const gcc_gin_pass *passes, int32_t npass, gcc_prof *prof, void *stream)
+static int32_t gin_forward_launches(const gcc_gin_pass *passes, int32_t npass, const FeatFetch &fetch, gcc_prof *prof, void *stream)
 {
     if (!passes || npass < 1 || npass > kMaxPass) {
         snprintf(g_err, kErrLen, "gcc_gin_forward: npass must be 1..%d", kMaxPass);
@@ -578,6 +595,7 @@
                       p.batch_size, p.w.pos_dim, p.w.deg_emb_dim, p.w.max_degree, p.edge_multiplicity > 1 ? p.edge_multiplicity : 1,
                       (int32_t)p.node_cap};
         }
+        L.f = fetch;
         hipLaunchKernelGGL(gin_feat_kernel, grid, block, 0, s, L);
     }
     for (int l = 0; l < Lg; ++l) {
@@ -666,3 +684,19 @@
     }
     return 0;
 }
+
+extern "C" int32_t gcc_gin_forward(const gcc_gin_pass *passes, int32_t npass, gcc_prof *prof, void *stream)
+{
+    return gin_forward_launches(passes, npass, FeatFetch{nullptr, nullptr, nullptr, 0}, prof, stream);
+}
+
+extern "C" int32_t gcc_gin_forward_fetch(const gcc_gin_pass *passes, int32_t npass, gcc_step_scalars *dev,
+                                         const gcc_step_scalars *ring, int32_t ring_len, unsigned long long *counter,
+                                         gcc_prof *prof, void *stream)
+{
+    if (!dev || !ring || !counter || ring_len < 1) {
+        snprintf(g_err, kErrLen, "gcc_gin_forward_fetch: bad argument");
+        return -1;
+    }
+    return gin_forward_launches(passes, npass, FeatFetch{dev, ring, counter, ring_len}, prof, stream);
+}
diff --git a/gcc_amd/csrc/encoder_bwd.hip b/gcc_amd/csrc/encoder_bwd.hip
--- a/gcc_amd/csrc/encoder_bwd.hip
+++ b/gcc_amd/csrc/encoder_bwd.hip
@@ -747,11 +747,15 @@
     const float *demb_parts;
     gcc_gin_grads g;
     int32_t B, L, kdim0, emb_rows, emb_dim, accumulate, hid;
+    double *sumsq_parts;
 };
 
-__device__ __forceinline__ void put(float *dst, float v, int acc)
-{
-    if (dst) *dst = acc ? *dst + v : v;
+__device__ __forceinline__ float put(float *dst, float v, int acc)
+{
+    if (!dst) return 0.f;
+    const float w = acc ? *dst + v : v;
+    *dst = w;
+    return w;
 }
 
 __global__ __launch_bounds__(kThreads) void gin_grad_final_kernel(FinalArgs a)
@@ -759,9 +763,12 @@
     TRAIN_STEP_WAVE_PRIORITY();
     const int64_t gid = (int64_t)blockIdx.x * kThreads + threadIdx.x;
     const int L = a.L;
-    int64_t base = 0;
+    float wrote = 0.f;
     const int njobs = 3 * L + 1;
     const int64_t n1 = (int64_t)njobs * H * H;
+    const int64_t n3 = (int64_t)(L + 1) * H;
+    const int64_t n4 = (int64_t)L * 3 * 3 * H;
+    const int64_t base5 = (n1 + n3 + n4 + 63) & ~(int64_t)63;
     if (gid < n1) {
         const int y = (int)(gid / (H * H)), idx = (int)(gid % (H * H));
         const int o = idx / H, k = idx % H;
@@ -778,23 +785,15 @@
             kd = i == 0 ? a.kdim0 : a.hid;
             dst = a.g.pred_w[i];
         }
-        if (k < kd && dst) put(dst + (int64_t)o * kd + k, s, a.accumulate);
-        return;
-    }
-    base += n1;
-    const int64_t n3 = (int64_t)(L + 1) * H;
-    if (gid < base + n3) {
-        const int64_t r = gid - base;
+        if (k < kd && dst) wrote = put(dst + (int64_t)o * kd + k, s, a.accumulate);
+    } else if (gid < n1 + n3) {
+        const int64_t r = gid - n1;
         const int i = (int)(r / H), o = (int)(r % H);
         float s = 0.f;
         for (int c = 0; c < kWgChunks; ++c) s += a.bias_slabs[((int64_t)(2 * L + i) * kWgChunks + c) * H + o];
-        if (a.g.pred_b[i]) put(a.g.pred_b[i] + o, s, a.accumulate);
-        return;
-    }
-    base += n3;
-    const int64_t n4 = (int64_t)L * 3 * 3 * H;
-    if (gid < base + n4) {
-        const int64_t r = gid - base;
+        if (a.g.pred_b[i]) wrote = put(a.g.pred_b[i] + o, s, a.accumulate);
+    } else if (gid < n1 + n3 + n4) {
+        const int64_t r = gid - (n1 + n3);
         const int c = (int)(r % H), slot = (int)((r / H) % 3), which = (int)((r / (3 * H)) % 3), l = (int)(r / (9 * H));
         double acc = 0.0;
         const double *src = a.bst + ((int64_t)l * 3 + which) * kRep * 3 * H + slot * H + c;
@@ -810,15 +809,11 @@
         if (which == 0) dst = slot == 0 ? a.g.bn_a_b[l] : slot == 1 ? a.g.bn_a_w[l] : a.g.lin0_b[l];
         else if (which == 1) dst = slot == 0 ? a.g.bn_b_b[l] : slot == 1 ? a.g.bn_b_w[l] : a.g.lin1_b[l];
         else dst = slot == 0 ? a.g.bn_c_b[l] : slot == 1 ? a.g.bn_c_w[l] : nullptr;
-        if (dst) put(dst + c, v, a.accumulate);
-        return;
-    }
-    base += n4;
-    base = (base + 63) & ~(int64_t)63;
-    const int64_t n5 = (int64_t)a.emb_rows * a.emb_dim;
-    if (gid >= base) {
+        if (dst) wrote = put(dst + c, v, a.accumulate);
+    } else if (gid >= base5) {
+        const int64_t n5 = (int64_t)a.emb_rows * a.emb_dim;
         static_assert(kEmbBlocks % 64 == 0, "8 threads x batches of 8 partials");
-        const int64_t q = gid - base, r = q >> 3;
+        const int64_t q = gid - base5, r = q >> 3;
         const int part = (int)(q & 7);
         float s = 0.f;
         if (r < n5) {
@@ -833,7 +828,14 @@
         s += wave_shfl_xor(s, 1);
         s += wave_shfl_xor(s, 2);
         s += wave_shfl_xor(s, 4);
-        if (part == 0 && r < n5 && a.g.degree_embedding) put(a.g.degree_embedding + r, s, a.accumulate);
+        if (part == 0 && r < n5 && a.g.degree_embedding) wrote = put(a.g.degree_embedding + r, s, a.accumulate);
+    }
+    if (a.sumsq_parts) {
+        __shared__ double red[kThreads / 64];
+        const double sq = wave_sum((double)wrote * (double)wrote);
+        if ((threadIdx.x & 63) == 0) red[threadIdx.x >> 6] = sq;
+        __syncthreads();
+        if (threadIdx.x == 0) a.sumsq_parts[blockIdx.x] = (red[0] + red[1]) + (red[2] + red[3]);
     }
 }
 
@@ -881,9 +883,10 @@
     return bwd_layout(nullptr, node_cap, batch_size, num_gin_layers, kEmbMaxElems).total;
 }
 
-extern "C" int32_t gcc_gin_backward(const gcc_gin_pass *pass, const float *dfeat, const gcc_gin_grads *grads,
-                                    int32_t accumulate, void *workspace, int64_t workspace_bytes,
-                                    int64_t node_cap, gcc_prof *prof, void *stream)
+static int32_t gin_backward_launches(const gcc_gin_pass *pass, const float *dfeat, const gcc_gin_grads *grads,
+                                     int32_t accumulate, void *workspace, int64_t workspace_bytes,
+                                     int64_t node_cap, double *sumsq_parts, int32_t parts_cap, int32_t *nparts,
+                                     gcc_prof *prof, void *stream)
 {
     if (!pass || !dfeat || !grads || !workspace) {
         snprintf(g_err, kErrLen, "gcc_gin_backward: null argument");
@@ -974,7 +977,16 @@
         a.accumulate = accumulate;
         const int64_t upto4 = (int64_t)(3 * L + 1) * H * H + (int64_t)(L + 1) * H + (int64_t)L * 9 * H;
         const int64_t total = ((upto4 + 63) & ~(int64_t)63) + (((int64_t)a.emb_rows * a.emb_dim * 8 + 63) & ~(int64_t)63);
-        hipLaunchKernelGGL(gin_grad_final_kernel, dim3((unsigned)((total + kThreads - 1) / kThreads)), block, 0, s, a);
+        const int64_t blocks = (total + kThreads - 1) / kThreads;
+        a.sumsq_parts = sumsq_parts;
+        if (sumsq_parts) {
+            if (blocks > parts_cap) {
+                snprintf(g_err, kErrLen, "gcc_gin_backward_sumsq: %lld partials, room for %d", (long long)blocks, parts_cap);
+                return -3;
+            }
+            *nparts = (int32_t)blocks;
+        }
+        hipLaunchKernelGGL(gin_grad_final_kernel, dim3((unsigned)blocks), block, 0, s, a);
     }
     prof_mark(prof, 1, s);
     hipError_t e = hipGetLastError();
@@ -984,3 +996,23 @@
     }
     return 0;
 }
+
+extern "C" int32_t gcc_gin_backward(const gcc_gin_pass *pass, const float *dfeat, const gcc_gin_grads *grads,
+                                    int32_t accumulate, void *workspace, int64_t workspace_bytes,
+                                    int64_t node_cap, gcc_prof *prof, void *stream)
+{
+    return gin_backward_launches(pass, dfeat, grads, accumulate, workspace, workspace_bytes, node_cap, nullptr, 0, nullptr, prof,
+                                 stream);
+}
+
+extern "C" int32_t gcc_gin_backward_sumsq(const gcc_gin_pass *pass, const float *dfeat, const gcc_gin_grads *grads,
+                                          void *workspace, int64_t workspace_bytes, int64_t node_cap, double *sumsq_parts,
+                                          int32_t parts_cap, int32_t *nparts, gcc_prof *prof, void *stream)
+{
+    if (!sumsq_parts || !nparts || parts_cap < 1) {
+        snprintf(g_err, kErrLen, "gcc_gin_backward_sumsq: bad argument");
+        return -1;
+    }
+    return gin_backward_launches(pass, dfeat, grads, 0, workspace, workspace_bytes, node_cap, sumsq_parts, parts_cap, nparts, prof,
+                                 stream);
+}
diff --git a/gcc_amd/csrc/nce.hip b/gcc_amd/csrc/nce.hip
--- a/gcc_amd/csrc/nce.hip
+++ b/gcc_amd/csrc/nce.hip
@@ -218,6 +218,184 @@
             st4(a.slabs + ((int64_t)s * a.B + qj) * D + 16 * db + 4 * q, o);
         }
     }
+}
+
+__global__ __launch_bounds__(kThreads) void nce_onepass_kernel(NceDev a)
+{
+    TRAIN_STEP_WAVE_PRIORITY();
+    __shared__ float Ms[kChunk * kLd];
+    const int tid = (int)threadIdx.x, lane = lane_id(), wv = tid >> 6, j = lane & 15, q = lane >> 4;
+    const int s = (int)blockIdx.x;
+    if (s == 0 && blockIdx.y == 0 && tid == 0) *a.ticket = 0;
+    const int qj = (int)blockIdx.y * kQPerBlock + 16 * wv + j;
+    const bool qvalid = qj < a.B;
+    F4 qf[4];
+    const float *qrow = a.q + (int64_t)(qvalid ? qj : 0) * D;
+#pragma unroll
+    for (int c = 0; c < 4; ++c) qf[c] = ld4(qrow + 16 * c + 4 * q);
+#pragma unroll
+    for (int c = 0; c < 4; ++c) {
+        qf[c].x = qvalid ? qf[c].x : 0.f; qf[c].y = qvalid ? qf[c].y : 0.f;
+        qf[c].z = qvalid ? qf[c].z : 0.f; qf[c].w = qvalid ? qf[c].w : 0.f;
+    }
+    const int row_beg = s * a.R, row_end = min(a.K, row_beg + a.R);
+    float m = -INFINITY, ssum = 0.f;
+    f32x4 acc2[4];
+#pragma unroll
+    for (int db = 0; db < 4; ++db) { f32x4 z = {0.f, 0.f, 0.f, 0.f}; acc2[db] = z; }
+    F4 nxt[4];
+    auto request = [&](int c0) {
+#pragma unroll
+        for (int i = 0; i < 4; ++i) {
+            const int idx = tid + kThreads * i, row = idx >> 4, c4 = (idx & 15) * 4;
+            nxt[i] = ld4(mem_row_ptr(a, c0 + row) + c4);
+        }
+    };
+    if (row_beg < row_end) request(row_beg);
+    for (int c0 = row_beg; c0 < row_end; c0 += kChunk) {
+#pragma unroll
+        for (int i = 0; i < 4; ++i) {
+            const int idx = tid + kThreads * i, row = idx >> 4, c4 = (idx & 15) * 4;
+            st4(&Ms[row * kLd + c4], finish_mem4(a, nxt[i], c0 + row));
+        }
+        __syncthreads();
+        if (c0 + kChunk < row_end) request(c0 + kChunk);
+        for (int t = 0; t < 4; ++t) {
+            if (c0 + 16 * t >= row_end) break;
+            f32x4 acc = {0.f, 0.f, 0.f, 0.f};
+#pragma unroll
+            for (int c = 0; c < 4; ++c) {
+                const F4 mf = ld4(&Ms[(16 * t + j) * kLd + 16 * c + 4 * q]);
+                acc = mfma_16x16x4_f32(mf.x, qf[c].x, acc);
+                acc = mfma_16x16x4_f32(mf.y, qf[c].y, acc);
+                acc = mfma_16x16x4_f32(mf.z, qf[c].z, acc);
+                acc = mfma_16x16x4_f32(mf.w, qf[c].w, acc);
+            }
+            const int row0 = c0 + 16 * t + 4 * q;
+            float lv[4];
+#pragma unroll
+            for (int r = 0; r < 4; ++r) lv[r] = row0 + r < row_end ? acc[r] * a.inv_T : -INFINITY;
+            float tmax = fmaxf(fmaxf(lv[0], lv[1]), fmaxf(lv[2], lv[3]));
+            tmax = fmaxf(tmax, wave_shfl_xor(tmax, 16));
+            tmax = fmaxf(tmax, wave_shfl_xor(tmax, 32));
+            const float mn = fmaxf(m, tmax);
+            const float sc = mn > -INFINITY ? expf(m - mn) : 1.f;
+            float p[4];
+#pragma unroll
+            for (int r = 0; r < 4; ++r) p[r] = lv[r] > -INFINITY ? expf(lv[r] - mn) : 0.f;
+            ssum = ssum * sc + ((p[0] + p[1]) + (p[2] + p[3]));
+            m = mn;
+#pragma unroll
+            for (int db = 0; db < 4; ++db) acc2[db] *= sc;
+#pragma unroll
+            for (int r = 0; r < 4; ++r)
+#pragma unroll
+                for (int db = 0; db < 4; ++db)
+                    acc2[db] = mfma_16x16x4_f32(Ms[(16 * t + 4 * q + r) * kLd + 16 * db + j], p[r], acc2[db]);
+        }
+        __syncthreads();
+    }
+    ssum += wave_shfl_xor(ssum, 16);
+    ssum += wave_shfl_xor(ssum, 32);
+    if (qvalid) {
+        if (q == 0) {
+            a.pm[(int64_t)s * a.B + qj] = m;
+            a.ps[(int64_t)s * a.B + qj] = ssum;
+        }
+#pragma unroll
+        for (int db = 0; db < 4; ++db) {
+            F4 o = {acc2[db][0], acc2[db][1], acc2[db][2], acc2[db][3]};
+            st4(a.slabs + ((int64_t)s * a.B + qj) * D + 16 * db + 4 * q, o);
+        }
+    }
+}
+
+__device__ __forceinline__ void nce_mean_by_last(const NceDev &a, double *red, int *last)
+{
+    const int tid = (int)threadIdx.x, lane = lane_id(), wv = tid >> 6;
+    device_fence();
+    __syncthreads();
+    if (tid == 0) *last = atomicAdd(a.ticket, 1) == (int)gridDim.x - 1;
+    __syncthreads();
+    if (!*last) return;
+    device_fence();
+    double lsum = 0.0, psum = 0.0;
+    for (int i = tid; i < a.B; i += kThreads) {
+        const float lse = load_fresh(a.lse + i), pos = load_fresh(a.pos + i);
+        lsum += (double)(lse - pos);
+        psum += (double)pos;
+    }
+    lsum = wave_sum(lsum);
+    psum = wave_sum(psum);
+    if (lane == 0) { red[wv] = lsum; red[4 + wv] = psum; }
+    __syncthreads();
+    if (tid == 0) {
+        a.loss[0] = (float)((red[0] + red[1] + red[2] + red[3]) / (double)a.B);
+        a.prob[0] = (float)((red[4] + red[5] + red[6] + red[7]) / (double)a.B);
+        *a.ticket = 0;
+    }
+}
+
+#ifndef NCE_MERGE_BATCH
+#define NCE_MERGE_BATCH 32
+#endif
+__global__ __launch_bounds__(kThreads) void nce_merge_kernel(NceDev a)
+{
+    TRAIN_STEP_WAVE_PRIORITY();
+    __shared__ double red[8];
+    __shared__ int last;
+    const int tid = (int)threadIdx.x, lane = lane_id(), wv = tid >> 6;
+    const int b = (int)blockIdx.x * (kThreads >> 6) + wv;
+    if (b < a.B) {
+        const float qv = a.q[(int64_t)b * D + lane], kv = a.k[(int64_t)b * D + lane];
+        const int s0 = min(lane, a.S - 1);
+        const float pm0r = a.pm[(int64_t)s0 * a.B + b], ps0r = a.ps[(int64_t)s0 * a.B + b];
+        const float dl = a.dloss[0];
+        const float *sp = a.slabs + (int64_t)b * D + lane;
+        const int64_t st = (int64_t)a.B * D;
+        float v[NCE_MERGE_BATCH];
+#pragma unroll
+        for (int u = 0; u < NCE_MERGE_BATCH; ++u) v[u] = sp[(int64_t)min(u, a.S - 1) * st];
+        const float pm0 = lane < a.S ? pm0r : -INFINITY;
+        const float pos = wave_sum(qv * kv) * a.inv_T;
+        float m = pm0;
+        for (int s = lane + 64; s < a.S; s += 64) m = fmaxf(m, a.pm[(int64_t)s * a.B + b]);
+        m = fmaxf(wave_max(m), pos);
+        float sum = pm0 > -INFINITY ? ps0r * expf(pm0 - m) : 0.f;
+        for (int s = lane + 64; s < a.S; s += 64) {
+            const float pmv = a.pm[(int64_t)s * a.B + b], psv = a.ps[(int64_t)s * a.B + b];
+            if (pmv > -INFINITY) sum += psv * expf(pmv - m);
+        }
+        sum = wave_sum(sum) + expf(pos - m);
+        const float lse = m + logf(sum);
+        if (lane == 0) {
+            a.lse[b] = lse;
+            a.pos[b] = pos;
+        }
+        float acc = 0.f;
+        for (int base = 0; base < a.S; base += 64) {
+            float pmv = pm0;
+            if (base > 0) pmv = base + lane < a.S ? a.pm[(int64_t)(base + lane) * a.B + b] : -INFINITY;
+            const float w = pmv > -INFINITY ? expf(pmv - lse) : 0.f;
+            const int send = min(a.S, base + 64);
+            for (int sl = base; sl < send; sl += NCE_MERGE_BATCH) {
+                if (sl > 0) {
+#pragma unroll
+                    for (int u = 0; u < NCE_MERGE_BATCH; ++u) v[u] = sp[(int64_t)min(sl + u, a.S - 1) * st];
+                }
+#pragma unroll
+                for (int u = 0; u < NCE_MERGE_BATCH; ++u) {
+                    if (sl + u < send) {
+                        const float ws = wave_readlane(w, sl + u - base);
+                        if (ws > 0.f) acc = fmaf(ws, v[u], acc);
+                    }
+                }
+            }
+        }
+        const float coef = dl * a.inv_T / (float)a.B;
+        a.dq[(int64_t)b * D + lane] = coef * (acc + (expf(pos - lse) - 1.f) * kv);
+    }
+    nce_mean_by_last(a, red, &last);
 }
 
 __global__ __launch_bounds__(kThreads) void nce_combine_kernel(NceDev a)
@@ -377,6 +555,8 @@
     float *ema; int64_t n_ema; float ema_m;
     const gcc_step_scalars *sc;
     double *acc; int32_t *mx; const float *loss, *prob; const int32_t *node_off_q, *edge_off_q, *node_off_k; int32_t B;
+    const double *parts; int32_t nparts;
+    float *q_mem; const float *q_keys; int32_t q_K, q_nkeys, adam_blocks;
 };
 
 __global__ __launch_bounds__(kThreads) void adam_kernel(float *p, float *g, float *m, float *v, int64_t n, float lr,
@@ -385,12 +565,42 @@
                                                         const double *sumsq, float *grad_norm, AdamExtras x)
 {
     TRAIN_STEP_WAVE_PRIORITY();
-    const double ss = sumsq[0];
+    const int nblk = x.q_mem ? x.adam_blocks : (int)gridDim.x;
+    if ((int)blockIdx.x >= nblk) {
+        const int gid = ((int)blockIdx.x - nblk) * kThreads + (int)threadIdx.x;
+        const int i = gid >> 4, c4 = (gid & 15) * 4;
+        if (i >= x.q_nkeys) return;
+        const int row = (x.sc->enqueue_index % x.q_K + i) % x.q_K;
+        st4(x.q_mem + (int64_t)row * D + c4, ld4(x.q_keys + (int64_t)i * D + c4));
+        return;
+    }
+    double ss = 0.0;
+    double pv[4] = {0.0, 0.0, 0.0, 0.0};
+    if (x.parts) {
+#pragma unroll
+        for (int u = 0; u < 4; ++u) {
+            const int idx = (int)threadIdx.x + kThreads * u;
+            pv[u] = x.parts[idx < x.nparts ? idx : x.nparts - 1];
+        }
+    } else {
+        ss = sumsq[0];
+    }
     if (x.sc) { lr = x.sc->lr; bc1 = x.sc->bias_corr1; bc2_sqrt = x.sc->bias_corr2_sqrt; }
-    const int64_t stride = (int64_t)gridDim.x * kThreads, i0 = (int64_t)blockIdx.x * kThreads + threadIdx.x;
+    const int64_t stride = (int64_t)nblk * kThreads, i0 = (int64_t)blockIdx.x * kThreads + threadIdx.x;
     const int64_t ic = i0 < n ? i0 : n - 1;
     float g0 = g[ic], p0 = p[ic], m0 = m[ic], v0 = v[ic];
     const float e0 = x.ema ? x.ema[i0 < x.n_ema ? i0 : x.n_ema - 1] : 0.f;
+    if (x.parts) {
+        __shared__ double red[kThreads / 64];
+        double t = 0.0;
+#pragma unroll
+        for (int u = 0; u < 4; ++u) if ((int)threadIdx.x + kThreads * u < x.nparts) t += pv[u];
+        for (int idx = (int)threadIdx.x + 4 * kThreads; idx < x.nparts; idx += kThreads) t += x.parts[idx];
+        t = wave_sum(t);
+        if ((threadIdx.x & 63) == 0) red[threadIdx.x >> 6] = t;
+        __syncthreads();
+        ss = (red[0] + red[1]) + (red[2] + red[3]);
+    }
     const float norm = grad_scale * (float)sqrt(ss);
     float coef = 1.f;
     if (max_norm > 0.f) {
@@ -531,6 +741,31 @@
     return 0;
 }
 
+int32_t gcc_nce_forward_backward(const gcc_nce_args *a, const float *dloss, float *dq, void *workspace,
+                                 int64_t workspace_bytes, gcc_prof *prof_fwd, gcc_prof *prof_bwd, void *stream)
+{
+    NceDev d;
+    Plan pl;
+    int rc = fill_dev(a, workspace, workspace_bytes, d, pl);
+    if (rc) return rc;
+    if (!a->loss || !a->prob || !dloss || !dq) { snprintf(g_err, kErrLen, "gcc_nce_forward_backward: bad argument"); return -1; }
+    if (a->pos_mode != 0 || a->out_dense || d.bf16) {
+        snprintf(g_err, kErrLen, "gcc_nce_forward_backward: pos_mode 0, f32, no dense output (use gcc_nce_forward + gcc_nce_backward)");
+        return -2;
+    }
+    d.dloss = dloss; d.dq = dq;
+    hipStream_t s = (hipStream_t)stream;
+    prof_mark(prof_fwd, 0, s);
+    hipLaunchKernelGGL(nce_onepass_kernel, dim3(pl.S, pl.QB), dim3(kThreads), 0, s, d);
+    prof_mark(prof_fwd, 1, s);
+    prof_mark(prof_bwd, 0, s);
+    hipLaunchKernelGGL(nce_merge_kernel, dim3((d.B + (kThreads >> 6) - 1) / (kThreads >> 6)), dim3(kThreads), 0, s, d);
+    prof_mark(prof_bwd, 1, s);
+    hipError_t e = hipGetLastError();
+    if (e != hipSuccess) { snprintf(g_err, kErrLen, "gcc_nce_forward_backward: %s", hipGetErrorString(e)); return -10; }
+    return 0;
+}
+
 int32_t gcc_queue_enqueue(float *mem, int32_t K, const float *keys, int32_t nkeys, int32_t index, float *saved,
                           void *stream)
 {
@@ -631,10 +866,16 @@
     return hipGetLastError() == hipSuccess ? 0 : -10;
 }
 
+struct AdamFold {
+    const double *parts; int32_t nparts;
+    float *q_mem; const float *q_keys; int32_t q_K, q_nkeys;
+};
+
 static int32_t adam_ema_launch(const char *who, float *param, float *grad, float *exp_avg, float *exp_avg_sq, int64_t n, float lr,
                                float beta1, float beta2, float eps, float weight_decay, int32_t step, float max_norm,
                                float grad_scale, float *grad_norm, double *scratch, float *ema, int64_t n_ema, float ema_m,
-                               const gcc_step_meters_args *meters, const gcc_step_scalars *scalars, void *stream)
+                               const gcc_step_meters_args *meters, const gcc_step_scalars *scalars, void *stream,
+                               const AdamFold *fold = nullptr)
 {
     if (!param || !grad || !exp_avg || !exp_avg_sq || !grad_norm || !scratch || n < 1 || (!scalars && step < 1) || !(grad_scale > 0.f) ||
         (ema && n_ema < n) ||
@@ -646,7 +887,8 @@
     hipStream_t s = (hipStream_t)stream;
     const float bc1 = scalars ? 1.f : 1.0f - powf(beta1, (float)step);
     const float bc2_sqrt = scalars ? 1.f : sqrtf(1.0f - powf(beta2, (float)step));
-    hipLaunchKernelGGL(gradnorm_kernel, dim3(kNormBlocks), dim3(kThreads), 0, s, (const float *)grad, n, scratch);
+    if (!fold || !fold->parts)
+        hipLaunchKernelGGL(gradnorm_kernel, dim3(kNormBlocks), dim3(kThreads), 0, s, (const float *)grad, n, scratch);
     AdamExtras x = {};
     x.sc = scalars;
     if (ema) { x.ema = ema; x.n_ema = n_ema; x.ema_m = ema_m; }
@@ -658,7 +900,15 @@
     const int64_t nmax = ema ? n_ema : n;
     int blocks = (int)((nmax + kThreads - 1) / kThreads);
     if (blocks > 512) blocks = 512;
-    hipLaunchKernelGGL(adam_kernel, dim3(blocks), dim3(kThreads), 0, s, param, grad, exp_avg, exp_avg_sq, n, lr, beta1,
+    int extra = 0;
+    if (fold) {
+        x.parts = fold->parts; x.nparts = fold->nparts;
+        if (fold->q_mem) {
+            x.q_mem = fold->q_mem; x.q_keys = fold->q_keys; x.q_K = fold->q_K; x.q_nkeys = fold->q_nkeys; x.adam_blocks = blocks;
+            extra = (fold->q_nkeys * 16 + kThreads - 1) / kThreads;
+        }
+    }
+    hipLaunchKernelGGL(adam_kernel, dim3(blocks + extra), dim3(kThreads), 0, s, param, grad, exp_avg, exp_avg_sq, n, lr, beta1,
                        beta2, eps, weight_decay, bc1, bc2_sqrt, max_norm, grad_scale, (const double *)scratch, grad_norm, x);
     return hipGetLastError() == hipSuccess ? 0 : -10;
 }
@@ -680,6 +930,25 @@
     if (!scalars) { snprintf(g_err, kErrLen, "gcc_adam_ema_step_scalars: scalars is NULL"); return -1; }
     return adam_ema_launch("gcc_adam_ema_step_scalars", param, grad, exp_avg, exp_avg_sq, n, 0.f, beta1, beta2, eps, weight_decay,
                            0, max_norm, grad_scale, grad_norm, scratch, ema, n_ema, ema_m, meters, scalars, stream);
+}
+
+int32_t gcc_adam_ema_enqueue_step_scalars(float *param, float *grad, float *exp_avg, float *exp_avg_sq, int64_t n,
+                                          float beta1, float beta2, float eps, float weight_decay, float max_norm,
+                                          float grad_scale, float *grad_norm, double *scratch, float *ema, int64_t n_ema, float ema_m,
+                                          const gcc_step_meters_args *meters, const gcc_step_scalars *scalars,
+                                          const double *sumsq_parts, int32_t nparts, float *queue, int32_t K, const float *keys,
+                                          int32_t nkeys, void *stream)
+{
+    const char *who = "gcc_adam_ema_enqueue_step_scalars";
+    if (!scalars) { snprintf(g_err, kErrLen, "%s: scalars is NULL", who); return -1; }
+    if ((sumsq_parts && nparts < 1) || (!sumsq_parts && nparts != 0) || (queue && (!keys || K < 1 || nkeys < 1 || nkeys > K)) ||
+        (!sumsq_parts && !queue)) {
+        snprintf(g_err, kErrLen, "%s: bad argument (nparts=%d K=%d n=%d)", who, nparts, K, nkeys);
+        return -1;
+    }
+    const AdamFold fold = {sumsq_parts, nparts, queue, keys, K, nkeys};
+    return adam_ema_launch(who, param, grad, exp_avg, exp_avg_sq, n, 0.f, beta1, beta2, eps, weight_decay, 0, max_norm, grad_scale,
+                           grad_norm, scratch, ema, n_ema, ema_m, meters, scalars, stream, &fold);
 }
 
 int32_t gcc_step_meters(double *acc, int32_t *mx, const float *loss, const float *prob, const float *grad_norm,
diff --git a/gcc_amd/encoder.py b/gcc_amd/encoder.py
--- a/gcc_amd/encoder.py
+++ b/gcc_amd/encoder.py
@@ -287,12 +287,18 @@
         key, gen = buf["_slot"]
         return self._gen.get(key) == gen
 
-    def forward(self, passes, stream=None, prof=None):
+    def forward(self, passes, stream=None, prof=None, fetch=None):
         arr = (_cabi.GccGinPass * len(passes))(*passes)
+        if fetch is not None:
+            scalars, ring, ring_len, counter = fetch
+            rc = self.lib.gcc_gin_forward_fetch(arr, len(passes), self.ptr(scalars), ring.data_ptr(), int(ring_len),
+                                                self.ptr(counter), prof.handle if prof is not None else None, stream)
+            if rc != 0:
+                raise RuntimeError(f"gcc_gin_forward_fetch failed ({rc}): {self.lib.gcc_last_error().decode()}")
+            return
         rc = self.lib.gcc_gin_forward(arr, len(passes), prof.handle if prof is not None else None, stream)
         if rc != 0:
             raise RuntimeError(f"gcc_gin_forward failed ({rc}): {self.lib.gcc_last_error().decode()}")
-
 
     def eval_fused(self, passes, mean_out=None, stream=None):
         arr = (_cabi.GccGinPass * len(passes))(*passes)
@@ -300,7 +306,7 @@
         if rc != 0:
             raise RuntimeError(f"gcc_gin_eval_fused failed ({rc}): {self.lib.gcc_last_error().decode()}")
 
-    def backward(self, enc, p, buf, dfeat, targets=None, accumulate=False, stream=None, prof=None):
+    def backward(self, enc, p, buf, dfeat, targets=None, accumulate=False, stream=None, prof=None, sumsq=None):
         ptr = self.ptr
         L = len(enc.gnn.ginlayers)
         g = buf["_keepalive"][0]
@@ -324,6 +330,16 @@
             else:
                 getattr(grads, name)[idx] = ptr(tgt)
         dfeat = dfeat.contiguous()
+        if sumsq is not None:
+            if accumulate:
+                raise ValueError("sumsq: the partial sums are of what ONE backward pass stores (accumulate=False)")
+            nparts = ctypes.c_int32(0)
+            rc = self.lib.gcc_gin_backward_sumsq(ctypes.byref(p), ptr(dfeat), ctypes.byref(grads), ptr(ws), nbytes, node_cap,
+                                                 ptr(sumsq), sumsq.numel(), ctypes.byref(nparts),
+                                                 prof.handle if prof is not None else None, stream)
+            if rc != 0:
+                raise RuntimeError(f"gcc_gin_backward_sumsq failed ({rc}): {self.lib.gcc_last_error().decode()}")
+            return targets, nparts.value
         rc = self.lib.gcc_gin_backward(ctypes.byref(p), ptr(dfeat), ctypes.byref(grads), int(accumulate),
                                        ptr(ws), nbytes, node_cap, prof.handle if prof is not None else None, stream)
         if rc != 0:
diff --git a/gcc_amd/train_step.py b/gcc_amd/train_step.py
--- a/gcc_amd/train_step.py
+++ b/gcc_amd/train_step.py
@@ -261,8 +261,9 @@
         self.steps = 0
         self.grad_norm = torch.zeros(1, dtype=torch.float32, device=param.device)
         self._scratch = torch.zeros(64, dtype=torch.float64, device=param.device)
-
-    def step(self, grad_scale=1.0, ema=None, ema_src=None, ema_m=0.0, meters=None, scalars=None):
+        self.sumsq_parts = torch.zeros(4096, dtype=torch.float64, device=param.device)
+
+    def step(self, grad_scale=1.0, ema=None, ema_src=None, ema_m=0.0, meters=None, scalars=None, sumsq_parts=None, enqueue=None):
         g = self.param_groups[0]
         self.steps += 1
         st = torch.cuda.current_stream(self.param.device).cuda_stream if self.param.is_cuda else None
@@ -273,7 +274,8 @@
         else:
             self.engine.adam_ema(self.param, self.grad, self.exp_avg, self.exp_avg_sq, g["lr"], g["betas"], g["eps"],
                                  g["weight_decay"], self.steps, self.clip_norm, self.grad_norm, self._scratch, stream=st,
-                                 grad_scale=grad_scale, ema=ema, ema_src=ema_src, ema_m=ema_m, meters=meters, scalars=scalars)
+                                 grad_scale=grad_scale, ema=ema, ema_src=ema_src, ema_m=ema_m, meters=meters, scalars=scalars,
+                                 **(dict(sumsq_parts=sumsq_parts, enqueue=enqueue) if sumsq_parts is not None or enqueue is not None else {}))
         return self.grad_norm
 
     def zero_grad(self):
@@ -460,8 +462,10 @@
     def __init__(self, model: GraphEncoder, model_ema: GraphEncoder, contrast: MemoryMoCo, sampler, posemb,
                  learning_rate=0.005, betas=(0.9, 0.999), weight_decay=1e-5, clip_norm=1.0, alpha=0.999,
                  world_size=1, rank=0, prefetch=True, extra_lanes=(), depth=2, lanes=None, chunk=1, reserved_cus=0, cu_layout="interleaved",
-                 collectives=None, ahead=None, graph=None, flat_engine=None):
+                 collectives=None, ahead=None, graph=None, flat_engine=None, fold=None, onepass_head=None):
         self.model, self.ema, self.contrast = model, model_ema, contrast
+        self.fold = (os.environ.get("GCC_STEP_FOLD", "1") != "0") if fold is None else bool(fold)
+        self.onepass_head = (os.environ.get("GCC_STEP_ONEPASS_HEAD", "0") == "1") if onepass_head is None else bool(onepass_head)
         self.sampler, self.posemb = sampler, posemb
         self.clip_norm, self.alpha = clip_norm, alpha
         self.world, self.rank = world_size, rank
@@ -661,22 +665,36 @@
             return self._body_wide(q, k, keep, S, st)
 
         def fwd():
-            self._fetch_scalars(scalars, st)
+            fetch = None
+            if self.fold and scalars is not None:
+                fetch = (scalars, self.ring, self.ring_len, self.ring_counter)
+            else:
+                self._fetch_scalars(scalars, st)
             S["pq"], S["bufq"] = self.gin.make_pass(self.model, q, training=True, keep=keep, slot=("step", 0),
                                                     dropout_seed=(0 if seed is not None else None) if scalars is not None else seed,
                                                     scalars=scalars)
             S["pk"], S["bufk"] = self.gin.make_pass(self.ema, k, training=True, keep=None, slot=("step", 1), backward=False)
-            self.gin.forward([S["pq"], S["pk"]], stream=st, prof=pr.get("gin_fwd"))
+            self.gin.forward([S["pq"], S["pk"]], stream=st, prof=pr.get("gin_fwd"), fetch=fetch)
 
         def gather_begin():
             S["gathering"] = self._all_gather_begin(self.keys_all, S["bufk"]["feat"])
 
         def head_and_backward():
             feat_q, feat_k = S["bufq"]["feat"], S["bufk"]["feat"]
-            S["outs"] = self.nce.forward(feat_q, feat_k, c.kernel_memory(), c.T, 0, stream=st, prof=pr.get("nce_fwd"))
-            dq = self.nce.backward(feat_q, feat_k, c.kernel_memory(), c.T, 0, S["outs"], self.one, stream=st,
-                                   prof=pr.get("nce_bwd"))
-            self.gin.backward(self.model, S["pq"], S["bufq"], dq, targets=self.grad_views, stream=st, prof=pr.get("gin_bwd"))
+            mem = c.kernel_memory()
+            if self.onepass_head:
+                S["outs"], dq = self.nce.forward_backward(feat_q, feat_k, mem, c.T, self.one, stream=st,
+                                                          prof_fwd=pr.get("nce_fwd"), prof_bwd=pr.get("nce_bwd"))
+            else:
+                S["outs"] = self.nce.forward(feat_q, feat_k, mem, c.T, 0, stream=st, prof=pr.get("nce_fwd"))
+                dq = self.nce.backward(feat_q, feat_k, mem, c.T, 0, S["outs"], self.one, stream=st,
+                                       prof=pr.get("nce_bwd"))
+            if self.fold and scalars is not None and not self.collectives:
+                _, n = self.gin.backward(self.model, S["pq"], S["bufq"], dq, targets=self.grad_views, stream=st,
+                                         prof=pr.get("gin_bwd"), sumsq=self.optimizer.sumsq_parts)
+                S["sumsq"] = (self.optimizer.sumsq_parts, n)
+            else:
+                self.gin.backward(self.model, S["pq"], S["bufq"], dq, targets=self.grad_views, stream=st, prof=pr.get("gin_bwd"))
 
         def reduce_and_join():
             self._all_reduce(self.flat_grad)
@@ -684,6 +702,11 @@
 
         def update():
             outs = S["outs"]
+            if "sumsq" in S:
+                S["gnorm"] = self.optimizer.step(ema=self.flat_ema, ema_src=self.flat, ema_m=self.alpha,
+                                                 meters=(self.meter_acc, self.meter_max, outs["loss"], outs["prob"], q, k),
+                                                 scalars=scalars, sumsq_parts=S["sumsq"], enqueue=(c.kernel_memory(), S["bufk"]["feat"]))
+                return
             S["gnorm"] = self.optimizer.step(grad_scale=1.0 / self.world if self.collectives else 1.0,
                                              ema=self.flat_ema, ema_src=self.flat, ema_m=self.alpha,
                                              meters=(self.meter_acc, self.meter_max, outs["loss"], outs["prob"], q, k),
diff --git a/include/gcc_amd.h b/include/gcc_amd.h
--- a/include/gcc_amd.h
+++ b/include/gcc_amd.h
@@ -180,6 +180,9 @@
 } gcc_gin_pass;
 
 int32_t gcc_gin_forward(const gcc_gin_pass *passes, int32_t npass, gcc_prof *prof, void *stream);
+int32_t gcc_gin_forward_fetch(const gcc_gin_pass *passes, int32_t npass, gcc_step_scalars *dev,
+                              const gcc_step_scalars *ring, int32_t ring_len, unsigned long long *counter,
+                              gcc_prof *prof, void *stream);
 
 int32_t gcc_gin_eval_fused(const gcc_gin_pass *passes, int32_t npass, float *mean_out, void *stream);
 void gcc_gin_eval_debug_ticks(long long *device_ticks64);
@@ -199,6 +202,10 @@
 int32_t gcc_gin_backward(const gcc_gin_pass *pass, const float *dfeat, const gcc_gin_grads *grads,
                          int32_t accumulate, void *workspace, int64_t workspace_bytes, int64_t node_cap,
                          gcc_prof *prof, void *stream);
+
+int32_t gcc_gin_backward_sumsq(const gcc_gin_pass *pass, const float *dfeat, const gcc_gin_grads *grads, void *workspace,
+                               int64_t workspace_bytes, int64_t node_cap, double *sumsq_parts, int32_t parts_cap,
+                               int32_t *nparts, gcc_prof *prof, void *stream);
 
 typedef struct gcc_ginx_pass {
     const int32_t *node_off, *row_ptr, *col_idx, *graph_id;
@@ -278,6 +285,8 @@
                         void *stream);
 int32_t gcc_nce_backward(const gcc_nce_args *a, const float *dloss, int32_t by_mem_row, float *dq,
                          void *workspace, int64_t workspace_bytes, gcc_prof *prof, void *stream);
+int32_t gcc_nce_forward_backward(const gcc_nce_args *a, const float *dloss, float *dq, void *workspace,
+                                 int64_t workspace_bytes, gcc_prof *prof_fwd, gcc_prof *prof_bwd, void *stream);
 
 int32_t gcc_queue_enqueue(float *mem, int32_t K, const float *keys, int32_t nkeys, int32_t index, float *saved,
                           void *stream);
@@ -309,6 +318,12 @@
                                   const gcc_step_meters_args *meters, const gcc_step_scalars *scalars, void *stream);
 int32_t gcc_queue_enqueue_scalars(float *mem, int32_t K, const float *keys, int32_t nkeys,
                                   const gcc_step_scalars *scalars, void *stream);
+int32_t gcc_adam_ema_enqueue_step_scalars(float *param, float *grad, float *exp_avg, float *exp_avg_sq, int64_t n,
+                                          float beta1, float beta2, float eps, float weight_decay, float max_norm,
+                                          float grad_scale, float *grad_norm, double *scratch, float *ema, int64_t n_ema, float ema_m,
+                                          const gcc_step_meters_args *meters, const gcc_step_scalars *scalars,
+                                          const double *sumsq_parts, int32_t nparts, float *queue, int32_t K, const float *keys,
+                                          int32_t nkeys, void *stream);
 
 typedef struct gcc_cls_head_args {
     const float *feat;
```

Result: faster. 716,800, median of 6 (+2.2%).
